# chao1224/GeoSSL

Hardware: AMD Instinct MI355X
Metric: molecules/s/GPU SchNet+DDM fwd+bwd (QM9-sized, bs=1024); % HBM roofline (higher is better)
Workload: dtype f32

## Files before the change

### geossl_amd/Geom3D/models/schnet.py

```python
import ctypes as C
import math
import os

import torch
from ...switches import env as _env
from torch.nn import Embedding, Linear, ModuleList, Sequential

from ... import _lib, ops
from ..._lib import call, ptr, stream
from ...layout import get_layout
from ._atomic_mass import atomic_masses

SUPPORTED_F = (32, 64, 128)


class _Ssp(torch.autograd.Function):
    @staticmethod
    def forward(ctx, x):
        x = x.contiguous()
        y = torch.empty_like(x)
        call("geossl_ssp_fwd", ptr(x), x.numel(), ptr(y), stream())
        ctx.save_for_backward(y)
        return y

    @staticmethod
    def backward(ctx, dy):
        (y,) = ctx.saved_tensors
        dx = torch.empty_like(y)
        call("geossl_ssp_bwd", ptr(y), ptr(dy.contiguous()), y.numel(), ptr(dx), stream())
        return dx


class ShiftedSoftplus(torch.nn.Module):

    def __init__(self):
        super().__init__()
        self.shift = torch.log(torch.tensor(2.0)).item()

    def forward(self, x):
        _lib.require_cuda(x)
        if x.dtype != torch.float32:
            raise TypeError("expected float32, got %s" % x.dtype)
        return _Ssp.apply(x)


class GaussianSmearing(torch.nn.Module):

    def __init__(self, start=0.0, stop=5.0, num_gaussians=50):
        super().__init__()
        offset = torch.linspace(start, stop, num_gaussians)
        self.coeff = -0.5 / (offset[1] - offset[0]).item() ** 2
        self.register_buffer("offset", offset)

    def forward(self, dist):
        return ops.gaussian_smearing(dist, self.offset, self.coeff)


class CFConv(torch.nn.Module):

    def __init__(self, in_channels, out_channels, num_filters, nn, cutoff):
        super().__init__()
        self.lin1 = Linear(in_channels, num_filters, bias=False)
        self.lin2 = Linear(num_filters, out_channels)
        self.nn = nn
        self.cutoff = cutoff
        self.reset_parameters()

    def reset_parameters(self):
        torch.nn.init.xavier_uniform_(self.lin1.weight)
        torch.nn.init.xavier_uniform_(self.lin2.weight)
        self.lin2.bias.data.fill_(0)


class InteractionBlock(torch.nn.Module):
    def __init__(self, hidden_channels, num_gaussians, num_filters, cutoff):
        super().__init__()
        self.mlp = Sequential(Linear(num_gaussians, num_filters), ShiftedSoftplus(), Linear(num_filters, num_filters))
        self.conv = CFConv(hidden_channels, hidden_channels, num_filters, self.mlp, cutoff)
        self.act = ShiftedSoftplus()
        self.lin = Linear(hidden_channels, hidden_channels)
        self.reset_parameters()

    def reset_parameters(self):
        torch.nn.init.xavier_uniform_(self.mlp[0].weight)
        self.mlp[0].bias.data.fill_(0)
        torch.nn.init.xavier_uniform_(self.mlp[2].weight)
        self.conv.reset_parameters()
        torch.nn.init.xavier_uniform_(self.lin.weight)
        self.lin.bias.data.fill_(0)


def _core_params(model):
    ps = [model.embedding.weight]
    for blk in model.interactions:
        ps += [blk.mlp[0].weight, blk.mlp[0].bias, blk.mlp[2].weight, blk.mlp[2].bias, blk.conv.lin1.weight,
               blk.conv.lin2.weight, blk.conv.lin2.bias, blk.lin.weight, blk.lin.bias]
    ps += [model.lin1.weight, model.lin1.bias, model.lin2.weight, model.lin2.bias]
    return ps


class _SchNetCore(torch.autograd.Function):

    @staticmethod
    def forward(ctx, z, pos, lay, cfg, *params):
        L, F, G = cfg["L"], cfg["F"], cfg["G"]
        dev = pos.device
        N = pos.size(0)
        want_params = any(ctx.needs_input_grad[4:])
        training = want_params or ctx.needs_input_grad[1]
        ps = [p.detach().contiguous() for p in params]
        emb_w, head = ps[0], ps[1 + 9 * L:]
        layers = [ps[1 + 9 * l: 1 + 9 * (l + 1)] for l in range(L)]
        st = stream()
        h = torch.empty(N, F, dtype=torch.float32, device=dev)
        status = cfg["status"]
        dyn = getattr(lay, "dyn", None)
        dN2, dP2 = (dyn.n_atoms2, dyn.n_pairs2) if dyn is not None else (None, None)
        if dyn is not None and (ctx.needs_input_grad[1] or F != 128 or not cfg["chain"]):
            raise _lib.GeosslHipError("a capacity-bucket layout serves the F = 128 chain path without position gradients")
        call("geossl_embedding_fwd_dyn", ptr(z), z.stride(0) if z.numel() else 1, ptr(emb_w), emb_w.size(0), N, F, ptr(h),
             ptr(status.word), dN2, st)
        if cfg["debug"]:
            status.check()
        sp = None
        if getattr(lay, "sparse", False):
            if dyn is not None:
                raise _lib.GeosslHipError("capacity buckets hold molecules of at most 255 atoms (bucket.MAX_N)")
            sp = ops.sparse_pair_geometry(pos, lay, cfg["cutoff"])
            pair_d, pair_c, pair_flag, dP2 = sp.pair_d, sp.pair_c, sp.pair_flag, sp.dyn_P
            aggregate = lambda x_, W_, out=None, swap=False, mols=None: ops.aggregate_sparse(x_, W_, sp, swap=swap, out=out)
        else:
            pair_d, pair_c, pair_flag = ops.pair_geometry(pos, lay, cfg["cutoff"])
            aggregate = lambda x_, W_, out=None, swap=False, mols=None: ops.aggregate(x_, W_, pair_flag, lay, swap=swap,
                                                                                      out=out, mols=mols)
        P = lay.P
        fw = _lib.FilterWeights()
        for l, lp in enumerate(layers):
            fw.w1[l], fw.b1[l], fw.w2[l], fw.b2[l] = ptr(lp[0]), ptr(lp[1]), ptr(lp[2]), ptr(lp[3])
        Wf = torch.empty(L, P, F, dtype=torch.float32, device=dev)
        keep_T = training and (ctx.needs_input_grad[1] or not _env("GEOSSL_FILTER_RECOMPUTE_T")
                               or bool(_env("GEOSSL_FILTER_BWD_BF16X3"))
                               or bool(_env("GEOSSL_ARITH_24BIT")))
        T = torch.empty(L, P, F, dtype=torch.float32, device=dev) if keep_T else None
        if P > 0:
            call("geossl_cfconv_filter_fwd_dyn", ptr(pair_d), ptr(pair_c), P, C.byref(fw), L, F, G, ptr(cfg["offset"]),
                 cfg["coeff"], ptr(T), ptr(Wf), dP2, st)
        hs, xs, aggs, ts = [], [], [], []
        heads = None
        if cfg["chain"]:
            chain_w = [lp[k] for lp in layers for k in (4, 5, 7)] + [head[0], head[2]]
            if want_params and 2 * len(chain_w) <= _lib.PREPARE_MAX:
                img, img_bwd = ops.prepare_chain(chain_w, both=True)
            else:
                img, img_bwd = ops.prepare_chain(chain_w, transB=True), None
            i_lin1, i_lin2, i_lin = img[0:3 * L:3], img[1:3 * L:3], img[2:3 * L:3]
            full = lambda: torch.empty(N, F, dtype=torch.float32, device=dev)
            hs, xs, aggs, ts = [h] + [full() for _ in range(L)], [full() for _ in range(L)], [full() for _ in range(L)], \
                [full() for _ in range(L)]
            u, hout = full(), full()

            def run_rows(a0, a1, mols, todo=None):
                rows = lambda t_: t_[a0:a1]

                def chain(x_, stages):
                    if todo is not None:
                        todo.append(("chain", x_, stages))
                    else:
                        ops.linear_chain(x_, stages, dyn_rows=dN2)

                chain(rows(hs[0]), [dict(image=i_lin1[0], out=rows(xs[0]))])
                for l, lp in enumerate(layers):
                    if todo is not None:
                        todo.append(("agg", xs[l], Wf[l], aggs[l], False))
                    else:
                        aggregate(xs[l], Wf[l], out=aggs[l], mols=mols)
                    stages = [dict(image=i_lin2[l], bias=lp[6], flags=_lib.EPI_SSP, out=rows(ts[l])),
                              dict(image=i_lin[l], bias=lp[8], res=rows(hs[l]), out=rows(hs[l + 1]))]
                    if l + 1 < L:
                        stages.append(dict(image=i_lin1[l + 1], out=rows(xs[l + 1])))
                    else:
                        stages.append(dict(image=img[3 * L], bias=head[1], flags=_lib.EPI_SSP, out=rows(u)))
                    chain(rows(aggs[l]), stages)
                chain(rows(u), [dict(image=img[3 * L + 1], bias=head[3], out=rows(hout))])

            todo = [] if (cfg["loop"] and P > 0 and sp is None and 2 * L + 2 <= _lib.LOOP_MAX_OPS) else None
            if todo is not None:
                run_rows(0, N, None, todo)
                if not ops.layer_loop(todo, lay, pair_flag, N, F, stagger=cfg["loop_stagger"]):
                    todo = None
            if todo is None:
                run_rows(0, N, None)
            h = hs[L]
            hs = hs[:L]
            if not training:
                hs, xs, aggs, ts = [], [], [], []
        else:
            pw = ops.prepare_linear([lp[k] for lp in layers for k in (4, 5, 7)], transB=True)
            if pw is not None:
                layers = [lp[:4] + [pw[3 * l], pw[3 * l + 1], lp[6], pw[3 * l + 2], lp[8]] for l, lp in enumerate(layers)]
            for l, lp in enumerate(layers):
                x = ops.linear(h, lp[4])
                agg = aggregate(x, Wf[l])
                t = ops.linear(agg, lp[5], bias=lp[6], flags=_lib.EPI_SSP)
                hn = ops.linear(t, lp[7], bias=lp[8], res=h)
                if training:
                    hs.append(h); xs.append(x); aggs.append(agg); ts.append(t)
                h = hn
            u = ops.linear(h, head[0], bias=head[1], flags=_lib.EPI_SSP)
            hout = ops.linear(u, head[2], bias=head[3])
        if training:
            ctx.lay, ctx.cfg = lay, cfg
            ctx.z = z
            ctx.pos = pos
            ctx.want_params = want_params
            ctx.ps = ps
            ctx.params = params
            ctx.saved = dict(pair_d=pair_d, pair_c=pair_c, pair_flag=pair_flag, Wf=Wf, T=T, hs=hs, xs=xs, aggs=aggs,
                             ts=ts, h_last=h, u=u, img_bwd=img_bwd if cfg["chain"] else None, sparse=sp)
        return hout

    @staticmethod
    def backward(ctx, dhout):
        want_pos, want_params = ctx.needs_input_grad[1], ctx.want_params
        if torch.is_grad_enabled():
            from ...higher_order import SchNetGradNode
            if ctx.saved.get("sparse") is not None:
                raise NotImplementedError("second-order gradients (create_graph=True, training on forces) are limited to "
                                          "dense layouts: structures of at most 255 atoms, GEOSSL_SPARSE_PAIRS unset")
            dpos, grads = SchNetGradNode.run(ctx, dhout, want_pos, want_params)
            return (None, dpos, None, None) + tuple(grads)
        dpos, grads = _SchNetCore.fused_backward(ctx, dhout, want_pos, want_params, allow_direct=True)
        return (None, dpos, None, None) + tuple(grads)

    @staticmethod
    def fused_backward(ctx, dhout, want_pos, want_params, allow_direct):
        cfg, lay, sv, ps = ctx.cfg, ctx.lay, ctx.saved, ctx.ps
        L, F, G = cfg["L"], cfg["F"], cfg["G"]
        dev = dhout.device
        N = dhout.size(0)
        st = stream()
        emb_w, head = ps[0], ps[1 + 9 * L:]
        layers = [ps[1 + 9 * l: 1 + 9 * (l + 1)] for l in range(L)]
        direct = want_params and allow_direct and _lib.direct_grads_enabled(ctx.params)
        grads = [p.grad for p in ctx.params] if direct else [torch.empty_like(p) if want_params else None for p in ps]
        accum = 1 if direct else 0
        g_emb, g_head = grads[0], grads[1 + 9 * L:]
        g_layers = [grads[1 + 9 * l: 1 + 9 * (l + 1)] for l in range(L)]
        dh_out = dhout.contiguous()
        dyn = getattr(lay, "dyn", None)
        dN2, dP2 = (dyn.n_atoms2, dyn.n_pairs2) if dyn is not None else (None, None)
        sp = sv.get("sparse")
        if sp is not None:
            dP2, pair_i, pair_j = sp.dyn_P, sp.pair_i, sp.pair_j
            aggregate = lambda x_, W_, out=None, mols=None: ops.aggregate_sparse(x_, W_, sp, swap=True, out=out)
        else:
            pair_i, pair_j = lay.pair_i, lay.pair_j
            aggregate = lambda x_, W_, out=None, mols=None: ops.aggregate(x_, W_, sv["pair_flag"], lay, swap=True,
                                                                          out=out, mols=mols)
        probs = []
        daggs = [None] * L
        if cfg["chain"]:
            img = sv.get("img_bwd")
            if img is None:
                img = ops.prepare_chain([lp[k] for lp in layers for k in (4, 5, 7)] + [head[0], head[2]], transB=False)
            i_lin1, i_lin2, i_lin = img[0:3 * L:3], img[1:3 * L:3], img[2:3 * L:3]
            full = lambda: torch.empty(N, F, dtype=torch.float32, device=dev)
            du = full()
            dhs = [full() for _ in range(L + 1)]
            dys, dxs = [full() for _ in range(L)], [full() for _ in range(L)]
            daggs = [full() for _ in range(L)]

            def run_rows(a0, a1, mols, todo=None):
                rows = lambda t_: t_[a0:a1]

                def chain(x_, stages):
                    if todo is not None:
                        todo.append(("chain", x_, stages))
                    else:
                        ops.linear_chain(x_, stages, dyn_rows=dN2)

                chain(rows(dh_out), [dict(image=img[3 * L + 1], tprev=rows(sv["u"]), out=rows(du)),
                                     dict(image=img[3 * L], out=rows(dhs[L]))])
                chain(rows(dhs[L]), [dict(image=i_lin[L - 1], tprev=rows(sv["ts"][L - 1]), out=rows(dys[L - 1])),
                                     dict(image=i_lin2[L - 1], out=rows(daggs[L - 1]))])
                for l in reversed(range(L)):
                    if todo is not None:
                        todo.append(("agg", daggs[l], sv["Wf"][l], dxs[l], True))
                    else:
                        aggregate(daggs[l], sv["Wf"][l], out=dxs[l], mols=mols)
                    stages = [dict(image=i_lin1[l], res=rows(dhs[l + 1]), out=rows(dhs[l]))]
                    if l > 0:
                        stages += [dict(image=i_lin[l - 1], tprev=rows(sv["ts"][l - 1]), out=rows(dys[l - 1])),
                                   dict(image=i_lin2[l - 1], out=rows(daggs[l - 1]))]
                    chain(rows(dxs[l]), stages)

            todo = [] if (cfg["loop"] and lay.P > 0 and sp is None and 2 * L + 2 <= _lib.LOOP_MAX_OPS) else None
            if todo is not None:
                run_rows(0, N, None, todo)
                if not ops.layer_loop(todo, lay, sv["pair_flag"], N, F, stagger=cfg["loop_stagger"]):
                    todo = None
            if todo is None:
                run_rows(0, N, None)
            probs.append((dh_out, sv["u"], g_head[2], g_head[3]))
            probs.append((du, sv["h_last"], g_head[0], g_head[1]))
            for l in reversed(range(L)):
                gl = g_layers[l]
                probs.append((dhs[l + 1], sv["ts"][l], gl[7], gl[8]))
                probs.append((dys[l], sv["aggs"][l], gl[5], gl[6]))
                probs.append((dxs[l], sv["hs"][l], gl[4], None))
            dh = dhs[0]
        else:
            du = ops.linear(dh_out, head[2], transB=False, tprev=sv["u"])
            dh = ops.linear(du, head[0], transB=False)
            probs.append((dh_out, sv["u"], g_head[2], g_head[3]))
            probs.append((du, sv["h_last"], g_head[0], g_head[1]))
            pw = ops.prepare_linear([lp[k] for lp in layers for k in (4, 5, 7)], transB=False)
            for l in reversed(range(L)):
                lp, gl = layers[l], g_layers[l]
                w_lin1, w_lin2, w_lin = (pw[3 * l], pw[3 * l + 1], pw[3 * l + 2]) if pw is not None else (lp[4], lp[5], lp[7])
                dy = ops.linear(dh, w_lin, transB=False, tprev=sv["ts"][l])
                dagg = ops.linear(dy, w_lin2, transB=False)
                dx = aggregate(dagg, sv["Wf"][l])
                dh_new = ops.linear(dx, w_lin1, transB=False, res=dh)
                probs.append((dh, sv["ts"][l], gl[7], gl[8]))
                probs.append((dy, sv["aggs"][l], gl[5], gl[6]))
                probs.append((dx, sv["hs"][l], gl[4], None))
                daggs[l] = dagg
                dh = dh_new
        P = lay.P
        fw = _lib.FilterWeights()
        gin = _lib.FilterGradIn()
        for l, lp in enumerate(layers):
            fw.w1[l], fw.b1[l], fw.w2[l], fw.b2[l] = ptr(lp[0]), ptr(lp[1]), ptr(lp[2]), ptr(lp[3])
            gin.x[l], gin.dagg[l] = ptr(sv["xs"][l]), ptr(daggs[l])
        if want_params:
            ops.linear_wgrad(probs, N, F, F, accumulate=bool(accum), dyn_rows=dN2)
            nfl = _lib.load().geossl_embedding_bwd_workspace_floats(emb_w.size(0), F)
            ws = torch.empty(nfl, dtype=torch.float32, device=dev)
            z = ctx.z
            call("geossl_embedding_bwd_dyn", ptr(z), z.stride(0) if z.numel() else 1, ptr(dh), emb_w.size(0), N, F,
                 ptr(g_emb), ptr(ws), accum, dN2, st)
            if P > 0:
                gout = _lib.FilterGradOut()
                for l, gl in enumerate(g_layers):
                    gout.dw1[l], gout.db1[l], gout.dw2[l], gout.db2[l] = ptr(gl[0]), ptr(gl[1]), ptr(gl[2]), ptr(gl[3])
                nfl = _lib.load().geossl_cfconv_filter_bwd_workspace_floats(P, L, F, G)
                ws2 = torch.empty(nfl, dtype=torch.float32, device=dev)
                call("geossl_cfconv_filter_bwd_dyn", ptr(sv["pair_d"]), ptr(sv["pair_c"]), ptr(sv["pair_flag"]),
                     ptr(pair_i), ptr(pair_j), P, N, C.byref(fw), C.byref(gin), L, F, G, ptr(cfg["offset"]),
                     cfg["coeff"], ptr(sv["T"]), C.byref(gout), ptr(ws2), accum, dP2, dN2, st)
            elif not direct:
                for gl in g_layers:
                    for k in range(4):
                        gl[k].zero_()
        dpos = None
        if want_pos:
            dpos = torch.zeros(N, 3, dtype=torch.float32, device=dev)
            if P > 0:
                dd = torch.empty(L, P, dtype=torch.float32, device=dev)
                call("geossl_cfconv_filter_dpos", ptr(sv["pair_d"]), ptr(sv["pair_c"]), ptr(sv["pair_flag"]),
                     ptr(pair_i), ptr(pair_j), P, C.byref(fw), C.byref(gin), L, F, G, ptr(cfg["offset"]),
                     cfg["coeff"], cfg["cutoff"], ptr(sv["T"]), ptr(sv["Wf"]), ptr(dd), st)
                if sp is not None:
                    ops.pair_position_grad_sparse(ctx.pos, sp, dd, out=dpos)
                else:
                    call("geossl_pair_position_grad", ptr(ctx.pos), ptr(sv["pair_d"]), ptr(dd), ptr(lay.mol_ptr),
                         ptr(lay.pair_ptr), lay.B, P, L, ptr(dpos), st)
        if direct:
            return dpos, [None] * len(grads)
        return dpos, list(grads)


class _SchNetTapeCore(torch.autograd.Function):

    @staticmethod
    def forward(ctx, z, pos, lay, cfg, *params):
        from ... import tape as tp
        with torch.no_grad():
            x = tp.leaf(pos, bool(ctx.needs_input_grad[1]))
            ps = [tp.leaf(p, bool(n)) for p, n in zip(params, ctx.needs_input_grad[4:])]
            h = tp.schnet_atom_features(z, x, lay, cfg, ps)
        ctx.tape = (h, x, ps)
        ctx.shapes = [tuple(p.shape) for p in params]
        return h.t

    @staticmethod
    def backward(ctx, dh):
        from ... import tape as tp
        if torch.is_grad_enabled():
            raise NotImplementedError("second-order gradients (training on forces) need the fused widths: "
                                      "hidden_channels == num_filters in %s" % (SUPPORTED_F,))
        h, x, ps = ctx.tape
        wrt = [v for v in [x] + ps if v.req]
        with torch.no_grad():
            got = iter(tp.grad([h], [tp.const(dh.contiguous())], wrt))
        vals = [next(got) if v.req else None for v in [x] + ps]
        dpos = None if vals[0] is None else vals[0].t
        grads = [None if g is None else g.t.reshape(shape) for g, shape in zip(vals[1:], ctx.shapes)]
        return (None, dpos, None, None) + tuple(grads)


class _SegmentReduce(torch.autograd.Function):

    @staticmethod
    def forward(ctx, h, lay, reduce):
        ctx.lay, ctx.reduce = lay, reduce
        return ops.segment_reduce(h.contiguous(), lay, reduce)

    @staticmethod
    def backward(ctx, dout):
        return _SegmentExpand.apply(dout, ctx.lay, ctx.reduce), None, None


class _SegmentExpand(torch.autograd.Function):

    @staticmethod
    def forward(ctx, dout, lay, reduce):
        ctx.lay, ctx.reduce = lay, reduce
        dh = torch.empty(lay.N, dout.size(1), dtype=torch.float32, device=dout.device)
        call("geossl_segment_reduce_bwd", ptr(dout.contiguous()), ptr(lay.mol_ptr), lay.B, dout.size(1),
             1 if reduce == "mean" else 0, ptr(dh), 0, stream())
        return dh

    @staticmethod
    def backward(ctx, g):
        return _SegmentReduce.apply(g, ctx.lay, ctx.reduce), None, None


class SchNet(torch.nn.Module):
    def __init__(self, hidden_channels=128, num_filters=128, num_interactions=6, num_gaussians=50, cutoff=10.0,
                 node_class=None, readout="mean", dipole=False, mean=None, std=None, atomref=None):
        super().__init__()
        assert readout in ["add", "sum", "mean"]
        self.hidden_channels = hidden_channels
        self.num_filters = num_filters
        self.num_interactions = num_interactions
        self.num_gaussians = num_gaussians
        self.cutoff = cutoff
        self.readout = readout
        self.dipole = dipole
        self.readout = "add" if self.dipole else self.readout
        self.mean = mean
        self.std = std
        self.scale = None

        self.register_buffer("atomic_mass", atomic_masses())
        self.embedding = Embedding(node_class, hidden_channels)
        self.distance_expansion = GaussianSmearing(0.0, cutoff, num_gaussians)
        self.interactions = ModuleList()
        for _ in range(num_interactions):
            self.interactions.append(InteractionBlock(hidden_channels, num_gaussians, num_filters, cutoff))
        self.lin1 = Linear(hidden_channels, hidden_channels)
        self.act = ShiftedSoftplus()
        self.lin2 = Linear(hidden_channels, hidden_channels)
        self.register_buffer("initial_atomref", atomref)
        self.atomref = None
        if atomref is not None:
            self.atomref = Embedding(100, 1)
            self.atomref.weight.data.copy_(atomref)
        self.reset_parameters()

    def reset_parameters(self):
        self.embedding.reset_parameters()
        for interaction in self.interactions:
            interaction.reset_parameters()
        torch.nn.init.xavier_uniform_(self.lin1.weight)
        self.lin1.bias.data.fill_(0)
        torch.nn.init.xavier_uniform_(self.lin2.weight)
        self.lin2.bias.data.fill_(0)
        if self.atomref is not None:
            self.atomref.weight.data.copy_(self.initial_atomref)

    def _status_word(self, device):
        return _lib.module_status(self, device, "atom type out of range for the embedding table (node_class=%d)"
                                  % self.embedding.num_embeddings)

    def check_status(self):
        st = self.__dict__.get("_geossl_status")
        if st is not None:
            st.check()

    def _check_supported(self):
        if self.dipole:
            raise NotImplementedError("dipole readout (schnet.py:103-107,117-118) is off the GeoSSL path")
        F = self.hidden_channels
        return (self.num_filters == F and F in SUPPORTED_F and self.num_interactions <= _lib.MAX_L
                and self.num_gaussians <= 64)

    def forward(self, z, pos, batch=None, return_latent=False, layout=None, latent_only=False):
        assert z.dim() == 1 and z.dtype == torch.long
        _lib.require_cuda(z, pos, batch)
        fused = self._check_supported()
        batch = torch.zeros_like(z) if batch is None else batch
        lay = layout if layout is not None else get_layout(batch)
        if lay.N != pos.size(0):
            raise ValueError("layout does not match the number of atoms")
        status = self._status_word(pos.device)
        status.poll()
        cfg = dict(L=self.num_interactions, F=self.hidden_channels, G=self.num_gaussians, cutoff=float(self.cutoff),
                   offset=self.distance_expansion.offset, coeff=float(self.distance_expansion.coeff),
                   debug=bool(_env("GEOSSL_DEBUG")), status=status,
                   chain=(self.num_interactions >= 1 and not _env("GEOSSL_NO_CHAIN")
                          and not _env("GEOSSL_ARITH_24BIT")),
                   loop=(_env("GEOSSL_LAYER_LOOP") == "1" or
                         (_env("GEOSSL_LAYER_LOOP") is None and not _env("GEOSSL_NO_LAYER_LOOP")
                          and torch.cuda.is_current_stream_capturing())),
                   loop_stagger=int(_env("GEOSSL_LAYER_LOOP_STAGGER") or 0))
        if pos.dtype != torch.float32:
            raise TypeError("positions must be float32")
        if fused:
            h = _SchNetCore.apply(z, pos.contiguous(), lay, cfg, *_core_params(self))
        else:
            if getattr(lay, "sparse", False):
                raise NotImplementedError("the general-width path (hidden_channels != num_filters, or widths outside %s) "
                                          "is limited to structures of at most 255 atoms; the fused widths take up to "
                                          "1024" % (SUPPORTED_F,))
            if z.numel() and (int(z.min()) < 0 or int(z.max()) >= self.embedding.num_embeddings):
                raise IndexError("atom type out of range for the embedding table (node_class=%d)"
                                 % self.embedding.num_embeddings)
            h = _SchNetTapeCore.apply(z, pos.contiguous(), lay, cfg, *_core_params(self))
        status.arm()
        if not self.dipole and self.mean is not None and self.std is not None:
            h = h * self.std + self.mean
        if not self.dipole and self.atomref is not None:
            h = h + self.atomref(z)
        if latent_only and return_latent:
            return None, h
        out = _SegmentReduce.apply(h, lay, self.readout)
        if self.scale is not None:
            out = self.scale * out
        if return_latent:
            return out, h
        return out

    def __repr__(self):
        return (f"{self.__class__.__name__}(hidden_channels={self.hidden_channels}, "
                f"num_filters={self.num_filters}, num_interactions={self.num_interactions}, "
                f"num_gaussians={self.num_gaussians}, cutoff={self.cutoff})")
```

### geossl_amd/_lib.py

```python
import ctypes as C
import os

import torch

HERE = os.path.dirname(os.path.abspath(__file__))
LIB_PATH = os.path.join(HERE, "lib", "libgeossl_hip.so")

MAX_L = 12
TN_MAX = 32
EPI_BIAS, EPI_SSP, EPI_RESIDUAL, EPI_MUL_DSSP, CHAIN_SAME_INPUT, CHAIN_NEW_INPUT, CHAIN_ADD_PREV = 1, 2, 4, 8, 16, 32, 64
EPI_SILU, EPI_MUL_DSILU = 128, 256

vp = C.c_void_p
i64 = C.c_int64
i32 = C.c_int
f32 = C.c_float
f64 = C.c_double
u64 = C.c_uint64


class FilterWeights(C.Structure):
    _fields_ = [("w1", vp * MAX_L), ("b1", vp * MAX_L), ("w2", vp * MAX_L), ("b2", vp * MAX_L)]


PREPARE_MAX = 64


class PrepareBatch(C.Structure):
    _fields_ = [("W", vp * PREPARE_MAX), ("image", vp * PREPARE_MAX), ("ldw", i32 * PREPARE_MAX), ("tb", i32 * PREPARE_MAX)]


CHAIN_MAX = 5


class ChainStage(C.Structure):
    _fields_ = [("image", vp), ("bias", vp), ("res", vp), ("tprev", vp), ("out", vp), ("ld", i32), ("flags", i32),
                ("xin", vp), ("ldxin", i32), ("pad_", i32), ("out_act", vp)]


class Chain(C.Structure):
    _fields_ = [("nstage", i32), ("st", ChainStage * CHAIN_MAX)]


LOOP_MAX_OPS = 14


class LoopOp(C.Structure):
    _fields_ = [("kind", i32), ("swap", i32), ("X", vp), ("Wf", vp), ("out", vp), ("chain", Chain)]


class FilterGradIn(C.Structure):
    _fields_ = [("x", vp * MAX_L), ("dagg", vp * MAX_L)]


class FilterGradOut(C.Structure):
    _fields_ = [("dw1", vp * MAX_L), ("db1", vp * MAX_L), ("dw2", vp * MAX_L), ("db2", vp * MAX_L)]


class TnBatch(C.Structure):
    _fields_ = [("A", vp * TN_MAX), ("B", vp * TN_MAX), ("dW", vp * TN_MAX), ("db", vp * TN_MAX)]


class NcsnWeights(C.Structure):
    _fields_ = [(k, vp) for k in ("in_w1", "in_b1", "in_w2", "in_b2", "o1_w", "o1_b", "o2_w", "o2_b", "o3_w", "o3_b",
                                  "sigmas")]


class NcsnGrads(C.Structure):
    _fields_ = [(k, vp) for k in ("in_w1", "in_b1", "in_w2", "in_b2", "o1_w", "o1_b", "o2_w", "o2_b", "o3_w", "o3_b")]


class NcsnSaved(C.Structure):
    _fields_ = [(k, vp) for k in ("a1", "a2", "pd", "emb", "gscale")]


class NcsnHeadFwd(C.Structure):
    _fields_ = [("h", vp), ("distance", vp), ("noise_level", vp), ("distance_noise", vp), ("w", NcsnWeights),
                ("saved", NcsnSaved), ("anneal_power", f32), ("pad_", f32), ("loss_e", vp), ("workspace", vp)]


class NcsnHeadBwd(C.Structure):
    _fields_ = [("h", vp), ("w", NcsnWeights), ("saved", NcsnSaved), ("out_scale", f32), ("pad_", f32), ("dfeat", vp),
                ("demb", vp), ("grow", vp), ("grads", NcsnGrads), ("workspace", vp), ("dh", vp)]


COPY_MAX = 8


class CopyBatch(C.Structure):
    _fields_ = [("dst", vp * COPY_MAX), ("src", vp * COPY_MAX), ("bytes", i64 * COPY_MAX)]


class Gather(C.Structure):
    _fields_ = [(k, vp) for k in ("x_src", "pos_src", "src_off", "mol_ptr", "x_dst", "pos_dst", "batch_dst", "se_ptr", "sei0",
                                  "sei1", "pair_ptr2", "pair_i", "pair_j", "inc_ptr", "inc_idx", "e0_src", "e1_src",
                                  "e_src_off", "e_ptr", "e0_dst", "e1_dst", "zero")] + \
               [("zero_count", i64), ("x_cols", i32), ("option", i32)]


class Mask(C.Structure):
    _fields_ = [(k, vp) for k in ("bond_ptr", "bond_dst", "src_n", "mol_id", "keep_in", "keep_out", "e_src_cnt",
                                  "e_count")] + [("seed", u64), ("max_n", i32), ("pad_", i32)]


P = C.POINTER
PROTOTYPES = {
    "geossl_abi_version": (i32, []),
    "geossl_layout_build": (i32, [vp, i64, i64, vp, vp, vp, vp]),
    "geossl_pair_index_fill": (i32, [vp, vp, i64, vp, vp, vp]),
    "geossl_radius_graph_count": (i32, [vp, vp, i64, i32, f32, i32, vp, vp]),
    "geossl_radius_graph_fill": (i32, [vp, vp, i64, i32, f32, i32, vp, vp, vp, vp, vp]),
    "geossl_pair_geometry": (i32, [vp, vp, vp, i64, i32, f32, i32, f32, vp, vp, vp, vp]),
    "geossl_rbf_fwd": (i32, [vp, i64, vp, i32, f32, vp, vp]),
    "geossl_ssp_fwd": (i32, [vp, i64, vp, vp]),
    "geossl_ssp_bwd": (i32, [vp, vp, i64, vp, vp]),
    "geossl_cfconv_filter_fwd": (i32, [vp, vp, i64, P(FilterWeights), i32, i32, i32, vp, f32, vp, vp, vp]),
    "geossl_cfconv_filter_bwd_workspace_floats": (i64, [i64, i32, i32, i32]),
    "geossl_cfconv_filter_bwd": (i32, [vp, vp, vp, vp, vp, i64, i64, P(FilterWeights), P(FilterGradIn), i32, i32, i32, vp,
                                       f32, vp, P(FilterGradOut), vp, i32, vp]),
    "geossl_cfconv_filter_dpos": (i32, [vp, vp, vp, vp, vp, i64, P(FilterWeights), P(FilterGradIn), i32, i32, i32, vp, f32,
                                        f32, vp, vp, vp, vp]),
    "geossl_pair_position_grad": (i32, [vp, vp, vp, vp, vp, i64, i64, i32, vp, vp]),
    "geossl_cfconv_aggregate": (i32, [vp, vp, vp, vp, vp, vp, i64, i32, i32, i32, vp, vp]),
    "geossl_aggregate_parts": (i32, [i32]),
    "geossl_cfconv_aggregate_work": (i32, [vp, vp, vp, vp, vp, vp, i64, i32, i32, i32, vp, vp]),
    "geossl_pair_product": (i32, [vp, vp, vp, vp, vp, i64, i32, i32, vp, vp]),
    "geossl_linear": (i32, [vp, i32, vp, vp, vp, vp, vp, i32, i64, i32, i32, i32, i32, vp]),
    "geossl_tn_plan": (None, [i64, i32, P(i32), P(i32)]),
    "geossl_tn_workspace_floats": (i64, [i64, i32, i32, i32]),
    "geossl_row_normalize_fwd": (i32, [vp, i64, i32, f32, vp, vp, vp]),
    "geossl_row_normalize_bwd": (i32, [vp, vp, vp, i64, i32, f32, vp, vp]),
    "geossl_atom_tuples": (i32, [vp, vp, i64, i32, vp, vp, vp]),
    "geossl_linear_image_words": (i64, [i32, i32]),
    "geossl_linear_prepare": (i32, [P(PrepareBatch), i32, i32, i32, i32, vp]),
    "geossl_linear_prepared": (i32, [vp, i32, vp, vp, vp, vp, vp, i32, i64, i32, i32, i32, vp]),
    "geossl_chain_image_words": (i64, [i32]),
    "geossl_chain_prepare": (i32, [P(PrepareBatch), i32, i32, i32, vp]),
    "geossl_linear_chain": (i32, [vp, i32, P(Chain), i64, i32, vp]),
    "geossl_linear_wgrad": (i32, [P(TnBatch), i32, i64, i32, i32, i32, i32, i32, vp, i32, vp]),
    "geossl_embedding_fwd": (i32, [vp, i64, vp, i32, i64, i32, vp, vp, vp]),
    "geossl_embedding_bwd_workspace_floats": (i64, [i32, i32]),
    "geossl_embedding_bwd": (i32, [vp, i64, vp, i32, i64, i32, vp, vp, i32, vp]),
    "geossl_segment_reduce_fwd": (i32, [vp, vp, i64, i32, i32, vp, vp]),
    "geossl_segment_reduce_bwd": (i32, [vp, vp, i64, i32, i32, vp, i32, vp]),
    "geossl_axpy": (i32, [vp, vp, f32, i64, vp, vp]),
    "geossl_pair_distance": (i32, [vp, vp, vp, i64, vp, vp]),
    "geossl_super_edge_ptr": (i32, [vp, vp, vp, i64, i64, vp, vp, vp]),
    "geossl_incidence_count": (i32, [vp, vp, vp, vp, i64, i32, vp, vp]),
    "geossl_incidence_fill": (i32, [vp, vp, vp, vp, i64, i32, vp, vp, vp]),
    "geossl_ddm_loss_fwd_workspace_floats": (i64, [i32]),
    "geossl_ddm_loss_fwd": (i32, [vp, vp, vp, vp, i64, vp, vp, vp, P(NcsnWeights), i32, f32, vp, P(NcsnSaved), vp, vp]),
    "geossl_schnet_layer_loop": (i32, [vp, i32, vp, i32, vp, vp, vp, i32, i32, i64, i32, i32, vp]),
    "geossl_schnet_layer_loop_ragged": (i32, [vp, i32, vp, vp, vp, i64, i32, i64, i32, vp]),
    "geossl_copy2": (i32, [vp, vp, i64, vp, vp, i64, vp]),
    "geossl_ddm_noise": (i32, [vp, f32, f32, i64, i64, i64, i32, i32, vp, vp, vp, vp, vp, vp]),
    "geossl_ddm_noise_seeded": (i32, [u64, f32, f32, i64, i64, i64, i32, i32, vp, vp, vp, vp, vp, vp]),
    "geossl_ddm_views": (i32, [vp, vp, vp, vp, i64, i64, vp, vp, vp, vp, i64, vp, vp]),
    "geossl_loss_reduce_partials": (i32, [vp, vp, f32, vp, i32, vp]),
    "geossl_ddm_loss_fwd2": (i32, [vp, vp, vp, vp, i64, i32, vp]),
    "geossl_loss_reduce_partials2": (i32, [vp, vp, vp, f32, f32, vp, vp]),
    "geossl_ddm_loss_bwd_fused2": (i32, [vp, vp, vp, i64, i64, i32, vp, vp, vp, vp, i32, vp]),
    "geossl_loss_reduce_workspace_floats": (i64, [i64]),
    "geossl_loss_reduce": (i32, [vp, i64, vp, f32, vp, vp, i32, vp]),
    "geossl_ddm_loss_bwd_rows": (i32, [P(NcsnWeights), P(NcsnSaved), i64, i32, vp, f32, vp, vp, vp, vp, vp, vp]),
    "geossl_ddm_loss_bwd_workspace_floats": (i64, [i64, i32]),
    "geossl_ddm_loss_bwd_weights": (i32, [vp, vp, vp, i64, i32, P(NcsnWeights), P(NcsnSaved), vp, vp, vp, P(NcsnGrads),
                                          vp, i32, vp]),
    "geossl_ddm_loss_bwd_fused_workspace_floats": (i64, [i64, i32]),
    "geossl_ddm_loss_bwd_fused": (i32, [vp, vp, vp, i64, i64, i32, P(NcsnWeights), P(NcsnSaved), vp, f32, vp, vp, vp, vp,
                                        P(NcsnGrads), vp, i32, vp]),
    "geossl_incidence_gather": (i32, [vp, vp, vp, i64, i32, vp, i32, vp]),
    "geossl_painn_edge_geom": (i32, [vp, vp, vp, i64, f32, vp, vp, i32, vp, vp, vp, vp]),
    "geossl_silu_fwd": (i32, [vp, i64, vp, vp]),
    "geossl_silu_bwd": (i32, [vp, vp, i64, vp, vp]),
    "geossl_painn_interaction_fwd": (i32, [vp, vp, vp, vp, vp, vp, vp, vp, vp, vp, vp, i64, i32, i32, vp, vp, vp]),
    "geossl_painn_interaction_bwd_workspace_floats": (i64, [i64, i32, i32]),
    "geossl_painn_interaction_fwd_mol": (i32, [vp, vp, vp, vp, vp, vp, vp, vp, vp, vp, vp, vp, i64, i32, i64, i32, i32, vp,
                                               vp, vp]),
    "geossl_painn_interaction_fwd_mma": (i32, [vp, vp, vp, vp, vp, vp, vp, vp, vp, vp, vp, vp, vp, i64, i32, i64, i32, i32,
                                               vp, vp, vp]),
    "geossl_painn_interaction_bwd_mol_workspace_floats": (i64, [i64, i64, i32, i32]),
    "geossl_painn_interaction_bwd_mol": (i32, [vp, vp, vp, vp, vp, vp, vp, vp, vp, vp, vp, vp, vp, i64, i32, i64, i32, i32,
                                               vp, vp, vp, vp, vp, i32, vp]),
    "geossl_painn_interaction_bwd": (i32, [vp, vp, vp, vp, vp, vp, vp, vp, vp, vp, vp, vp, i64, i32, i32, vp, vp, vp, vp,
                                           vp, i32, vp]),
    "geossl_painn_mix_pre_fwd": (i32, [vp, vp, i64, i32, f32, vp, vp, vp]),
    "geossl_painn_mix_post_fwd": (i32, [vp, vp, vp, vp, vp, i64, i32, vp, vp, vp]),
    "geossl_painn_mix_post_bwd": (i32, [vp, vp, vp, vp, vp, i64, i32, vp, vp, vp]),
    "geossl_painn_mix_pre_bwd": (i32, [vp, vp, vp, vp, i64, i32, vp, vp, vp]),
    "geossl_add": (i32, [vp, vp, i64, vp, vp]),
    "geossl_painn_edge_grads": (i32, [vp] * 11 + [i64, i32, i32, vp, vp, vp, i32, vp]),
    "geossl_painn_edge_geom_bwd": (i32, [vp, vp, vp, i64, f32, vp, vp, i32, vp, vp, vp, vp, vp]),
    "geossl_painn_position_grad": (i32, [vp, vp, vp, vp, vp, i64, vp, vp]),
    "geossl_adam_step": (i32, [vp, vp, vp, vp, i64, f64, f64, f64, f64, f64, i64, f32, vp]),
    "geossl_copy_n": (i32, [P(CopyBatch), i32, vp]),
    "geossl_ddm_views_dyn": (i32, [vp, vp, vp, vp, i64, i64, vp, vp, vp, vp, i64, vp, vp, vp, vp]),
    "geossl_embedding_fwd_dyn": (i32, [vp, i64, vp, i32, i64, i32, vp, vp, vp, vp]),
    "geossl_embedding_bwd_dyn": (i32, [vp, i64, vp, i32, i64, i32, vp, vp, i32, vp, vp]),
    "geossl_cfconv_filter_fwd_dyn": (i32, [vp, vp, i64, P(FilterWeights), i32, i32, i32, vp, f32, vp, vp, vp, vp]),
    "geossl_cfconv_filter_bwd_dyn": (i32, [vp, vp, vp, vp, vp, i64, i64, P(FilterWeights), P(FilterGradIn), i32, i32, i32,
                                           vp, f32, vp, P(FilterGradOut), vp, i32, vp, vp, vp]),
    "geossl_cfconv_aggregate_work_dyn": (i32, [vp, vp, vp, vp, vp, vp, i64, i32, i32, i32, vp, vp, vp]),
    "geossl_cfconv_aggregate_targets_dyn": (i32, [vp, vp, vp, vp, vp, vp, i64, i32, i32, i32, vp, vp, vp]),
    "geossl_linear_chain_dyn": (i32, [vp, i32, P(Chain), i64, i32, vp, vp]),
    "geossl_linear_wgrad_dyn": (i32, [P(TnBatch), i32, i64, i32, i32, i32, i32, i32, vp, i32, vp, vp]),
    "geossl_ddm_loss_fwd2_dyn": (i32, [vp, vp, vp, vp, i64, i32, vp, vp, vp]),
    "geossl_ddm_loss_bwd_fused2_dyn": (i32, [vp, vp, vp, i64, i64, i32, vp, vp, vp, vp, i32, vp, vp, vp]),
    "geossl_painn_group_capacity": (i64, [i64, i64]),
    "geossl_painn_edge_layout": (i32, [vp, vp, i64, vp, i64, i64, i64] + [vp] * 12),
    "geossl_painn_edge_geom_dyn": (i32, [vp, vp, vp, i64, f32, vp, vp, i32, vp, vp, vp, vp, vp]),
    "geossl_painn_interaction_fwd_mma_dyn": (i32, [vp, vp, vp, vp, vp, vp, vp, vp, vp, vp, vp, vp, vp, i64, i32, i64, i32,
                                                   i32, vp, vp, vp, vp]),
    "geossl_tape_unary": (i32, [i32, vp, i64, f32, f32, vp, vp]),
    "geossl_tape_binary": (i32, [i32, vp, i32, vp, i32, i64, i32, f32, vp, vp]),
    "geossl_tape_colsum_workspace_floats": (i64, [i64, i32]),
    "geossl_tape_reduce": (i32, [i32, vp, i64, i32, vp, vp, vp]),
    "geossl_tape_gather_rows": (i32, [vp, vp, i32, i64, i32, vp, vp]),
    "geossl_tape_scatter_rows": (i32, [vp, vp, i32, vp, i64, i32, vp, vp]),
    "geossl_tape_copy2d": (i32, [vp, i64, vp, i64, i64, i32, vp]),
    "geossl_tape_fill": (i32, [vp, i64, f32, vp]),
    "geossl_painn_stage_cap": (i32, [i32, i32, i32]),
    "geossl_painn_interaction_fwd_atoms": (i32, [vp] * 12 + [i64, vp, i32, i32, vp, vp, vp]),
    "geossl_painn_interaction_bwd_atoms": (i32, [vp] * 13 + [i64, vp, i32, i32, vp, vp, vp, vp, vp, i32, vp]),
    "geossl_painn_interaction_bwd_mol_skip": (i32, [vp, vp, vp, vp, vp, vp, vp, vp, vp, vp, vp, vp, vp, i64, i32, i64, i32,
                                                    i32, vp, vp, vp, vp, vp, i32, vp]),
    "geossl_painn_mix_pre_fwd_dyn": (i32, [vp, vp, i64, i32, f32, vp, vp, vp, vp]),
    "geossl_painn_mix_post_fwd_dyn": (i32, [vp, vp, vp, vp, vp, i64, i32, vp, vp, vp, vp]),
    "geossl_painn_mix_post_bwd_dyn": (i32, [vp, vp, vp, vp, vp, i64, i32, vp, vp, vp, vp]),
    "geossl_painn_mix_pre_bwd_dyn": (i32, [vp, vp, vp, vp, i64, i32, vp, vp, vp, vp]),
    "geossl_gather_molecules": (i32, [P(Gather), i64, vp]),
    "geossl_gather_masked_molecules": (i32, [P(Gather), P(Mask), i64, vp]),
    "geossl_infonce_fwd": (i32, [vp, vp, i64, i32, f32, vp, vp, vp, vp, vp]),
    "geossl_infonce_bwd": (i32, [vp, vp, vp, vp, i64, i32, f32, vp, vp, vp, vp]),
    "geossl_ebm_nce_fwd": (i32, [vp, vp, i64, i32, i32, vp, vp, vp, vp, vp, vp]),
    "geossl_ebm_nce_bwd": (i32, [vp, vp, vp, i64, i32, i32, vp, vp, vp, vp]),
    "geossl_distance_head_width_ok": (i32, [i32]),
    "geossl_distance_head_fwd_workspace_floats": (i64, [i64]),
    "geossl_distance_head_bwd_workspace_floats": (i64, [i64, i32]),
    "geossl_distance_head_fwd": (i32, [vp, i64, i32, vp, vp, vp, vp, vp, i64, vp, vp, vp, vp, vp, vp]),
    "geossl_distance_head_fwd_dyn": (i32, [vp, i64, i32, vp, vp, vp, vp, vp, i64, vp, vp, vp, vp, vp, vp, vp, vp]),
    "geossl_distance_head_bwd": (i32, [vp, i64, i32, vp, vp, i64, vp, vp, vp, vp, vp, vp, vp, vp, i32, vp]),
    "geossl_distance_head_bwd_dyn": (i32, [vp, i64, i32, vp, vp, i64, vp, vp, vp, vp, vp, vp, vp, vp, i32, vp, vp, vp]),
    "geossl_charge_mask_count": (i64, [i64, f64]),
    "geossl_charge_mask": (i32, [vp, i32, i64, f64, i32, vp, vp, vp, vp, vp, vp]),
    "geossl_charge_mask_dyn": (i32, [vp, i32, i64, f64, i32, vp, vp, vp, vp, vp, vp, vp]),
    "geossl_charge_head_width_ok": (i32, [i32, i32]),
    "geossl_charge_head_fwd_workspace_floats": (i64, [i64]),
    "geossl_charge_head_bwd_workspace_floats": (i64, [i64, i32, i32]),
    "geossl_charge_head_fwd": (i32, [vp, i64, i32, vp, vp, i32, vp, vp, i64, vp, vp, vp, vp, vp, vp]),
    "geossl_charge_head_fwd_dyn": (i32, [vp, i64, i32, vp, vp, i32, vp, vp, i64, vp, vp, vp, vp, vp, vp, vp]),
    "geossl_charge_head_bwd": (i32, [vp, i64, i32, vp, i32, vp, vp, i64, vp, vp, vp, vp, vp, vp, vp, i32, vp]),
    "geossl_charge_head_bwd_dyn": (i32, [vp, i64, i32, vp, i32, vp, vp, i64, vp, vp, vp, vp, vp, vp, vp, i32, vp, vp]),
    "geossl_infograph_width_ok": (i32, [i32]),
    "geossl_infograph_fwd_workspace_floats": (i64, [i64]),
    "geossl_infograph_fwd": (i32, [vp, i64, i32, vp, vp, i64, i32, vp, vp, vp, vp, vp, vp, vp, vp]),
    "geossl_infograph_fwd_dyn": (i32, [vp, i64, i32, vp, vp, i64, i32, vp, vp, vp, vp, vp, vp, vp, vp, vp]),
    "geossl_infograph_bwd": (i32, [vp, i64, i32, vp, vp, i64, i32, vp, vp, vp, vp, vp, vp, vp, vp]),
    "geossl_infograph_bwd_dyn": (i32, [vp, i64, i32, vp, vp, i64, i32, vp, vp, vp, vp, vp, vp, vp, vp, vp]),
    "geossl_property_width_ok": (i32, [i32]),
    "geossl_property_workspace_floats": (i64, [i64]),
    "geossl_property_fwd": (i32, [vp, i64, i32, vp, i64, i32, i32, vp, vp, vp, vp, vp, i64, vp, i32, vp, vp, vp, vp, vp,
                                  vp]),
    "geossl_property_fwd_dyn": (i32, [vp, i64, i32, vp, i64, i32, i32, vp, vp, vp, vp, vp, i64, vp, i32, vp, vp, vp, vp,
                                      vp, vp, vp]),
    "geossl_property_predict": (i32, [vp, i64, i32, vp, i64, i32, i32, vp, vp, vp, vp, vp, vp, vp]),
    "geossl_property_predict_dyn": (i32, [vp, i64, i32, vp, i64, i32, i32, vp, vp, vp, vp, vp, vp, vp, vp]),
    "geossl_property_bwd": (i32, [i64, i32, vp, i64, i32, i32, vp, vp, vp, vp, vp, vp, i64, vp, i32, vp, vp, vp, vp, vp,
                                  vp, i32, vp]),
    "geossl_property_bwd_dyn": (i32, [i64, i32, vp, i64, i32, i32, vp, vp, vp, vp, vp, vp, i64, vp, i32, vp, vp, vp, vp,
                                      vp, vp, i32, vp, vp]),
    "geossl_property_targets": (i32, [vp, i64, i32, i32, vp, vp, i64, vp, vp]),
    "geossl_torsion_head_width_ok": (i32, [i32]),
    "geossl_torsion_head_fwd_workspace_floats": (i64, [i64]),
    "geossl_torsion_head_bwd_workspace_floats": (i64, [i64, i32]),
    "geossl_torsion_head_fwd": (i32, [vp, i64, i32, vp, vp, vp, vp, vp, vp, i64, vp, vp, vp, vp, vp, vp]),
    "geossl_torsion_head_fwd_dyn": (i32, [vp, i64, i32, vp, vp, vp, vp, vp, vp, i64, vp, vp, vp, vp, vp, vp, vp, vp]),
    "geossl_torsion_head_bwd": (i32, [vp, i64, i32, vp, vp, vp, vp, i64, vp, vp, i64, vp, vp, vp, vp, vp, i32, vp]),
    "geossl_torsion_head_bwd_dyn": (i32, [vp, i64, i32, vp, vp, vp, vp, i64, vp, vp, i64, vp, vp, vp, vp, vp, i32, vp, vp,
                                          vp]),
    "geossl_triple_angles": (i32, [vp, i64, vp, vp, vp, i64, vp, vp]),
    "geossl_gather_triples": (i32, [vp, i64, vp, vp, vp, vp, i64, vp, vp, vp, vp, vp]),
    "geossl_sparse_pairs_build": (i32, [vp, vp, i64, i64, i32, f32, i32, f32, i64] + [vp] * 13),
    "geossl_cfconv_aggregate_sparse": (i32, [vp, vp, vp, vp, vp, i64, i32, i32, vp, vp]),
    "geossl_pair_position_grad_sparse": (i32, [vp, vp, vp, vp, vp, vp, i64, i64, i32, vp, vp]),
}

_lib = None


class GeosslHipError(RuntimeError):
    pass


def load():
    global _lib
    if _lib is not None:
        return _lib
    path = os.environ.get("GEOSSL_HIP_LIB", LIB_PATH)
    if not os.path.exists(path):
        raise GeosslHipError(
            "libgeossl_hip.so is not built (%s). Run `python -m geossl_amd.build` (needs hipcc); "
            "there is no CPU fallback." % path)
    lib = C.CDLL(path)
    for name, (res, args) in PROTOTYPES.items():
        fn = getattr(lib, name)
        fn.restype = res
        fn.argtypes = args
    if lib.geossl_abi_version() != 1:
        raise GeosslHipError("ABI version mismatch")
    _lib = lib
    return lib


def check(rc, what):
    if rc != 0:
        raise GeosslHipError("%s failed with hipError %d" % (what, rc))


def ptr(t):
    if t is None:
        return None
    return t.data_ptr()


def stream():
    return torch._C._cuda_getCurrentRawStream(torch._C._cuda_getDevice())


def require_cuda(*tensors):
    for t in tensors:
        if t is not None and not t.is_cuda:
            raise GeosslHipError(
                "geossl_amd runs on MI355X only: got a %s tensor. The HIP path has no CPU fallback." % t.device.type)



_DIRECT = {"depth": 0}


class direct_grads:
    def __enter__(self):
        _DIRECT["depth"] += 1
        return self

    def __exit__(self, *exc):
        _DIRECT["depth"] -= 1
        return False


def direct_grads_enabled(params):
    return _DIRECT["depth"] > 0 and all(
        p.grad is not None and p.grad.is_contiguous() and p.grad.dtype == torch.float32 and p.grad.is_cuda
        for p in params)


class StatusWord:

    def __init__(self, device, message):
        self.word = torch.zeros(1, dtype=torch.int32, device=device)
        self.host = torch.zeros(1, dtype=torch.int32).pin_memory()
        self.event = None
        self.message = message

    def __deepcopy__(self, memo):
        return None

    def __reduce__(self):
        return (type(None), ())

    def poll(self):
        if self.event is None or torch.cuda.is_current_stream_capturing():
            return
        if self.event.query():
            self.event = None
            if int(self.host[0]):
                raise IndexError(self.message)

    def arm(self, every=1):
        self.calls = getattr(self, "calls", 0) + 1
        if every > 1 and self.calls % every != 1:
            return
        if self.event is None and not torch.cuda.is_current_stream_capturing():
            self.host.copy_(self.word, non_blocking=True)
            self.event = torch.cuda.Event()
            self.event.record()

    def check(self):
        if int(self.word.item()):
            raise IndexError(self.message)


def module_status(module, device, message):
    st = module.__dict__.get("_geossl_status")
    if st is None or st.word.device != device:
        st = StatusWord(device, message)
        module.__dict__["_geossl_status"] = st
    return st


TIMERS = None
CALLS = None


def call(name, *args):
    global CALLS
    lib = load()
    if CALLS is not None:
        CALLS += 1
    timers = TIMERS
    key = name[:-4] if name.endswith("_dyn") else name
    if timers is not None and key in timers:
        e0, e1 = torch.cuda.Event(enable_timing=True), torch.cuda.Event(enable_timing=True)
        e0.record()
        rc = getattr(lib, name)(*args)
        e1.record()
        timers[key].append((e0, e1))
    else:
        rc = getattr(lib, name)(*args)
    check(rc, name)


def fill_ptrs(arr, tensors):
    for i, t in enumerate(tensors):
        arr[i] = ptr(t)
```

### geossl_amd/csrc/filter_fwd.hip

```cpp
#include "common.h"
#include "geossl_hip.h"
#include "split.h"

using namespace geossl;

namespace {

#ifdef FF_TIMING
__device__ long long ff_dbg[2 * 64 * 8 + 2 * 64];
#define FF_MARK(slot)                                                                                     \
  do {                                                                                                    \
    __builtin_amdgcn_sched_barrier(0);                                                                    \
    if (blockIdx.x == 3 && blockIdx.y == 0 && lane == 0 && (wave == 0 || wave == 4) && ff_t < 64)        \
      ff_dbg[((wave == 0 ? 0 : 1) * 64 + ff_t) * 8 + (slot)] = clock64();                                 \
    __builtin_amdgcn_sched_barrier(0);                                                                    \
  } while (0)
#else
#define FF_MARK(slot) do {} while (0)
#endif

template <int NMB, int K1S>
__global__ __launch_bounds__(512) void k_filter_fwd(const float* __restrict__ pair_d,
                                                    const float* __restrict__ pair_c, int P,
                                                    GeosslFilterWeights w, int G,
                                                    const float* __restrict__ offset, float coeff,
                                                    float* __restrict__ Tout, float* __restrict__ Wf,
                                                    const int32_t* __restrict__ dyn_P) {
  constexpr int F = 32 * NMB, K2S = F / 16;
  extern __shared__ __attribute__((aligned(16))) uint8_t smem_raw[];
  u32x4* W2f = reinterpret_cast<u32x4*>(smem_raw);
  u32x4* W1f = W2f + NMB * K2S * 3 * 64;
  float* b1s = reinterpret_cast<float*>(W1f + NMB * K1S * 3 * 64);
  float* b2s = b1s + F;
  float* offs = b2s + F;
  const int tid = threadIdx.x, lane = tid & 63, wave = tid >> 6, j = lane & 31, kh = lane >> 5;
  const int l = blockIdx.y;
  {
    const float* __restrict__ w2 = w.w2[l];
    for (int i = tid; i < NMB * K2S * 64; i += 512) {
      const int ln = i & 63, ks = (i >> 6) % K2S, mb = i / (64 * K2S);
      const float* row = w2 + (size_t)(32 * mb + (ln & 31)) * F + 16 * ks + 4 * (ln >> 5);
      const float4 lo = *reinterpret_cast<const float4*>(row), hi = *reinterpret_cast<const float4*>(row + 8);
      const float v[8] = {lo.x, lo.y, lo.z, lo.w, hi.x, hi.y, hi.z, hi.w};
      const Frag3 f = split8(v);
      u32x4* dst = W2f + ((size_t)(mb * K2S + ks) * 3) * 64 + ln;
      dst[0] = f.h;
      dst[64] = f.m;
      dst[128] = f.l;
    }
    const float* __restrict__ w1 = w.w1[l];
    for (int i = tid; i < NMB * K1S * 64; i += 512) {
      const int ln = i & 63, ks = (i >> 6) % K1S, mb = i / (64 * K1S);
      const float* row = w1 + (size_t)(32 * mb + (ln & 31)) * G;
      float v[8];
#pragma unroll
      for (int e = 0; e < 8; ++e) {
        const int g = 16 * ks + 8 * (ln >> 5) + e;
        v[e] = g < G ? row[g] : 0.0f;
      }
      const Frag3 f = split8(v);
      u32x4* dst = W1f + ((size_t)(mb * K1S + ks) * 3) * 64 + ln;
      dst[0] = f.h;
      dst[64] = f.m;
      dst[128] = f.l;
    }
    for (int i = tid; i < F; i += 512) {
      b1s[i] = w.b1[l][i];
      b2s[i] = w.b2[l][i];
    }
    for (int i = tid; i < 16 * K1S; i += 512) offs[i] = i < G ? offset[i] : 0.0f;
  }
  __syncthreads();
  const size_t lbase = (size_t)l * P;
  P = dyn_count(P, dyn_P);
  if (P <= 0) return;
  const int nrb = (P + 31) / 32;
#ifdef FF_TIMING
  int ff_t = -1;
#endif
  for (int rb = blockIdx.x + gridDim.x * wave; rb < nrb; rb += gridDim.x * 8) {
#ifdef FF_TIMING
    ++ff_t;
#endif
    FF_MARK(0);
#ifdef FF_TIMING
    if (blockIdx.x == 3 && blockIdx.y == 0 && lane == 0 && (wave == 0 || wave == 4) && ff_t < 64)
      ff_dbg[2 * 64 * 8 + (wave == 0 ? 0 : 64) + ff_t] = wall_clock64();
#endif
    const int row = 32 * rb + j;
    const bool live = row < P;
    const float d = live ? pair_d[row] : 0.0f;
    const float cw = live ? pair_c[row] : 0.0f;
    f32x16 acc1[NMB];
#pragma unroll
    for (int mb = 0; mb < NMB; ++mb)
#pragma unroll
      for (int q = 0; q < 4; ++q) {
        const float4 b = *reinterpret_cast<const float4*>(b1s + 32 * mb + 8 * q + 4 * kh);
        acc1[mb][4 * q] = b.x;
        acc1[mb][4 * q + 1] = b.y;
        acc1[mb][4 * q + 2] = b.z;
        acc1[mb][4 * q + 3] = b.w;
      }
    Frag3 bfr[K1S];
#pragma unroll
    for (int ks = 0; ks < K1S; ++ks) {
      float v[8];
      const float4 o0 = *reinterpret_cast<const float4*>(offs + 16 * ks + 8 * kh);
      const float4 o1 = *reinterpret_cast<const float4*>(offs + 16 * ks + 8 * kh + 4);
      const float o[8] = {o0.x, o0.y, o0.z, o0.w, o1.x, o1.y, o1.z, o1.w};
#pragma unroll
      for (int e = 0; e < 8; ++e) {
        const float diff = d - o[e];
        v[e] = exp_neg(coeff * (diff * diff));
      }
      bfr[ks] = split8(v);
    }
    FF_MARK(1);
    Frag3 tb[K2S];
    float* trow = Tout != nullptr ? Tout + (lbase + row) * F + 4 * kh : nullptr;
    auto finish_block = [&](int mb) {
#pragma unroll
      for (int half = 0; half < 2; ++half) {
        float v[8];
#pragma unroll
        for (int e = 0; e < 8; ++e) v[e] = ssp(acc1[mb][8 * half + e]);
        if (trow != nullptr && live) {
          *reinterpret_cast<float4*>(trow + 32 * mb + 16 * half) = make_float4(v[0], v[1], v[2], v[3]);
          *reinterpret_cast<float4*>(trow + 32 * mb + 16 * half + 8) = make_float4(v[4], v[5], v[6], v[7]);
        }
        tb[2 * mb + half] = split8(v);
      }
    };
#pragma unroll
    for (int mb = 0; mb < NMB; ++mb) {
#pragma unroll
      for (int ks = 0; ks < K1S; ++ks) {
        Frag3 af;
        const u32x4* src = W1f + ((size_t)(mb * K1S + ks) * 3) * 64 + lane;
        af.h = src[0];
        af.m = src[64];
        af.l = src[128];
        mma6(acc1[mb], af, bfr[ks]);
      }
      if (mb > 0) {
        finish_block(mb - 1);
#pragma unroll
        for (int i = 0; i < 6 * K1S; ++i) {
          __builtin_amdgcn_sched_group_barrier(0x008, 1, 0);
          __builtin_amdgcn_sched_group_barrier(0x002, 16, 0);
        }
      }
      __builtin_amdgcn_sched_barrier(0);
    }
    FF_MARK(2);
    finish_block(NMB - 1);
    __builtin_amdgcn_sched_barrier(0);
    FF_MARK(3);
    constexpr int MP = NMB >= 2 ? 2 : 1;
    float* orow = Wf + (lbase + row) * F + 4 * kh;
#pragma unroll
    for (int mb0 = 0; mb0 < NMB; mb0 += MP) {
      f32x16 acc2[MP];
#pragma unroll
      for (int u = 0; u < MP; ++u)
#pragma unroll
        for (int q = 0; q < 4; ++q) {
          const float4 b = *reinterpret_cast<const float4*>(b2s + 32 * (mb0 + u) + 8 * q + 4 * kh);
          acc2[u][4 * q] = b.x;
          acc2[u][4 * q + 1] = b.y;
          acc2[u][4 * q + 2] = b.z;
          acc2[u][4 * q + 3] = b.w;
        }
      Frag3 af[MP], an[MP];
#pragma unroll
      for (int u = 0; u < MP; ++u) {
        const u32x4* src = W2f + ((size_t)((mb0 + u) * K2S) * 3) * 64 + lane;
        af[u].h = src[0];
        af[u].m = src[64];
        af[u].l = src[128];
      }
#pragma unroll
      for (int ks = 0; ks < K2S; ++ks) {
        if (ks + 1 < K2S) {
#pragma unroll
          for (int u = 0; u < MP; ++u) {
            const u32x4* src = W2f + ((size_t)((mb0 + u) * K2S + ks + 1) * 3) * 64 + lane;
            an[u].h = src[0];
            an[u].m = src[64];
            an[u].l = src[128];
          }
        }
        __builtin_amdgcn_sched_barrier(0);
#pragma unroll
        for (int u = 0; u < MP; ++u) acc2[u] = mfma_bf16(af[u].l, tb[ks].h, acc2[u]);
#pragma unroll
        for (int u = 0; u < MP; ++u) acc2[u] = mfma_bf16(af[u].h, tb[ks].l, acc2[u]);
#pragma unroll
        for (int u = 0; u < MP; ++u) acc2[u] = mfma_bf16(af[u].m, tb[ks].m, acc2[u]);
#pragma unroll
        for (int u = 0; u < MP; ++u) acc2[u] = mfma_bf16(af[u].m, tb[ks].h, acc2[u]);
#pragma unroll
        for (int u = 0; u < MP; ++u) acc2[u] = mfma_bf16(af[u].h, tb[ks].m, acc2[u]);
#pragma unroll
        for (int u = 0; u < MP; ++u) acc2[u] = mfma_bf16(af[u].h, tb[ks].h, acc2[u]);
        __builtin_amdgcn_sched_barrier(0);
        if (ks + 1 < K2S) {
#pragma unroll
          for (int u = 0; u < MP; ++u) af[u] = an[u];
        }
      }
      if (mb0 == 0) FF_MARK(4);
      else FF_MARK(6);
      if (live) {
#pragma unroll
        for (int u = 0; u < MP; ++u)
#pragma unroll
          for (int q = 0; q < 4; ++q)
            *reinterpret_cast<float4*>(orow + 32 * (mb0 + u) + 8 * q) =
                make_float4(acc2[u][4 * q] * cw, acc2[u][4 * q + 1] * cw, acc2[u][4 * q + 2] * cw,
                            acc2[u][4 * q + 3] * cw);
      }
      if (mb0 == 0) FF_MARK(5);
      else FF_MARK(7);
    }
  }
}



#ifndef FFH_THREADS
#define FFH_THREADS 512
#endif
template <int NMB, int K1S>
__global__ __launch_bounds__(FFH_THREADS) void k_filter_fwd_h(const float* __restrict__ pair_d,
                                                      const float* __restrict__ pair_c, int P,
                                                      GeosslFilterWeights w, int G,
                                                      const float* __restrict__ offset, float coeff,
                                                      float* __restrict__ Tout, float* __restrict__ Wf,
                                                    const int32_t* __restrict__ dyn_P) {
  constexpr int F = 32 * NMB, K2S = F / 16;
  extern __shared__ __attribute__((aligned(16))) uint8_t smem_raw[];
  u32x4* W2f = reinterpret_cast<u32x4*>(smem_raw);
  u32x4* W1f = W2f + NMB * K2S * 2 * 64;
  float* b1s = reinterpret_cast<float*>(W1f + NMB * K1S * 2 * 64);
  float* b2s = b1s + F;
  float* offs = b2s + F;
  float* red = offs + 16 * K1S;
  const int tid = threadIdx.x, lane = tid & 63, wave = tid >> 6, j = lane & 31, kh = lane >> 5;
  const int l = blockIdx.y;
  float s1, s2;
  {
    const float* __restrict__ w2 = w.w2[l];
    const float* __restrict__ w1 = w.w1[l];
    float m1 = 0.0f, m2 = 0.0f;
    for (int i = tid; i < F * G; i += FFH_THREADS) m1 = fmaxf(m1, fabsf(w1[i]));
    for (int i = tid; i < F * F; i += FFH_THREADS) m2 = fmaxf(m2, fabsf(w2[i]));
#pragma unroll
    for (int o = 32; o >= 1; o >>= 1) {
      m1 = fmaxf(m1, __shfl_xor(m1, o));
      m2 = fmaxf(m2, __shfl_xor(m2, o));
    }
    if (lane == 0) {
      red[wave] = m1;
      red[16 + wave] = m2;
    }
    __syncthreads();
#pragma unroll
    for (int i = 0; i < FFH_THREADS / 64; ++i) {
      m1 = fmaxf(m1, red[i]);
      m2 = fmaxf(m2, red[16 + i]);
    }
    int e1, e2;
    s1 = pow2_scale_to_2p14(m1, e1);
    s2 = pow2_scale_to_2p14(m2, e2);
    for (int i = tid; i < NMB * K2S * 64; i += FFH_THREADS) {
      const int ln = i & 63, ks = (i >> 6) % K2S, mb = i / (64 * K2S);
      const float* row = w2 + (size_t)(32 * mb + (ln & 31)) * F + 16 * ks + 4 * (ln >> 5);
      const float4 lo = *reinterpret_cast<const float4*>(row), hi = *reinterpret_cast<const float4*>(row + 8);
      const float v[8] = {lo.x * s2, lo.y * s2, lo.z * s2, lo.w * s2, hi.x * s2, hi.y * s2, hi.z * s2, hi.w * s2};
      const Frag2 f = split8h(v);
      u32x4* dst = W2f + ((size_t)(mb * K2S + ks) * 2) * 64 + ln;
      dst[0] = f.h;
      dst[64] = f.l;
    }
    for (int i = tid; i < NMB * K1S * 64; i += FFH_THREADS) {
      const int ln = i & 63, ks = (i >> 6) % K1S, mb = i / (64 * K1S);
      const float* row = w1 + (size_t)(32 * mb + (ln & 31)) * G;
      float v[8];
#pragma unroll
      for (int e = 0; e < 8; ++e) {
        const int g = 16 * ks + 8 * (ln >> 5) + e;
        v[e] = g < G ? row[g] * s1 : 0.0f;
      }
      const Frag2 f = split8h(v);
      u32x4* dst = W1f + ((size_t)(mb * K1S + ks) * 2) * 64 + ln;
      dst[0] = f.h;
      dst[64] = f.l;
    }
    for (int i = tid; i < F; i += FFH_THREADS) {
      b1s[i] = w.b1[l][i];
      b2s[i] = w.b2[l][i];
    }
    for (int i = tid; i < 16 * K1S; i += FFH_THREADS) offs[i] = i < G ? offset[i] : 0.0f;
  }
  int* next_rb = reinterpret_cast<int*>(red + 32);
  if (tid == 0) *next_rb = 0;
  __syncthreads();
  const float inv1 = 1.0f / (s1 * 16384.0f), inv2 = 1.0f / s2;
  const size_t lbase = (size_t)l * P;
  P = dyn_count(P, dyn_P);
  if (P <= 0) return;
  const int nrb = (P + 31) / 32;
  auto take = [&]() {
    int t = 0;
    if (lane == 0) t = atomicAdd(next_rb, 1);
    return (int)blockIdx.x + (int)gridDim.x * __builtin_amdgcn_readfirstlane(t);
  };
  int rb = take();
  float d_n = pair_d[min(32 * rb + j, P - 1)], cw_n = pair_c[min(32 * rb + j, P - 1)];
  while (rb < nrb) {
    const int row = 32 * rb + j;
    const bool live = row < P;
    const float d = d_n;
    const float cw = live ? cw_n : 0.0f;
    const int rb_next = take();
    d_n = pair_d[min(32 * rb_next + j, P - 1)];
    cw_n = pair_c[min(32 * rb_next + j, P - 1)];
    int z = 0;
    asm volatile("" : "+v"(z));
    const int lz = lane + z, khz = 4 * kh + z;
    Frag2 bfr[K1S];
#pragma unroll
    for (int ks = 0; ks < K1S; ++ks) {
      float v[8];
      const float4 o0 = *reinterpret_cast<const float4*>(offs + 16 * ks + 2 * khz);
      const float4 o1 = *reinterpret_cast<const float4*>(offs + 16 * ks + 2 * khz + 4);
      const float o[8] = {o0.x, o0.y, o0.z, o0.w, o1.x, o1.y, o1.z, o1.w};
#pragma unroll
      for (int e = 0; e < 8; ++e) {
        const float diff = d - o[e];
        v[e] = exp_neg(coeff * (diff * diff));
      }
      bfr[ks] = split8h_scaled(v, 16384.0f);
    }
    f32x16 acc1[NMB];
#pragma unroll
    for (int mb = 0; mb < NMB; ++mb) {
#pragma unroll
      for (int e = 0; e < 16; ++e) acc1[mb][e] = 0.0f;
#pragma unroll
      for (int ks = 0; ks < K1S; ++ks) {
        const u32x4* src = W1f + ((size_t)(mb * K1S + ks) * 2) * 64 + lz;
        const u32x4 ah = src[0], al = src[64];
        acc1[mb] = mfma_f16(al, bfr[ks].h, acc1[mb]);
        acc1[mb] = mfma_f16(ah, bfr[ks].l, acc1[mb]);
        acc1[mb] = mfma_f16(ah, bfr[ks].h, acc1[mb]);
      }
    }
    float* trow = Tout != nullptr ? Tout + (lbase + row) * F + 4 * kh : nullptr;
    float tmax = 0.0f;
#pragma unroll
    for (int mb = 0; mb < NMB; ++mb)
#pragma unroll
      for (int q = 0; q < 4; ++q) {
        const float4 b = *reinterpret_cast<const float4*>(b1s + 32 * mb + 8 * q + khz);
        const float bb[4] = {b.x, b.y, b.z, b.w};
#pragma unroll
        for (int e = 0; e < 4; ++e) {
          const float t = ssp(fmaf(acc1[mb][4 * q + e], inv1, bb[e]));
          acc1[mb][4 * q + e] = t;
          tmax = fmaxf(tmax, fabsf(t));
        }
        if (trow != nullptr && live)
          *reinterpret_cast<float4*>(trow + 32 * mb + 8 * q) =
              make_float4(acc1[mb][4 * q], acc1[mb][4 * q + 1], acc1[mb][4 * q + 2], acc1[mb][4 * q + 3]);
      }
    tmax = fmaxf(tmax, __shfl_xor(tmax, 32));
    int et;
    const float st = pow2_scale_to_2p14(tmax, et);
    const float k2 = inv2 * __builtin_amdgcn_ldexpf(1.0f, et - 14);
    Frag2 tb[K2S];
#pragma unroll
    for (int ks = 0; ks < K2S; ++ks) {
      float v[8];
#pragma unroll
      for (int e = 0; e < 8; ++e) v[e] = acc1[ks >> 1][8 * (ks & 1) + e];
      tb[ks] = split8h_scaled(v, st);
    }
    constexpr int MP = NMB >= 2 ? 2 : 1;
    float* orow = Wf + (lbase + row) * F + 4 * kh;
#pragma unroll
    for (int mb0 = 0; mb0 < NMB; mb0 += MP) {
      f32x16 acc2[MP];
#pragma unroll
      for (int u = 0; u < MP; ++u)
#pragma unroll
        for (int e = 0; e < 16; ++e) acc2[u][e] = 0.0f;
#pragma unroll
      for (int ks = 0; ks < K2S; ++ks) {
        u32x4 ah[MP], al[MP];
#pragma unroll
        for (int u = 0; u < MP; ++u) {
          const u32x4* src = W2f + ((size_t)((mb0 + u) * K2S + ks) * 2) * 64 + lz;
          ah[u] = src[0];
          al[u] = src[64];
        }
#pragma unroll
        for (int u = 0; u < MP; ++u) acc2[u] = mfma_f16(al[u], tb[ks].h, acc2[u]);
#pragma unroll
        for (int u = 0; u < MP; ++u) acc2[u] = mfma_f16(ah[u], tb[ks].l, acc2[u]);
#pragma unroll
        for (int u = 0; u < MP; ++u) acc2[u] = mfma_f16(ah[u], tb[ks].h, acc2[u]);
      }
#pragma unroll
      for (int u = 0; u < MP; ++u)
#pragma unroll
        for (int q = 0; q < 4; ++q) {
          const float4 b = *reinterpret_cast<const float4*>(b2s + 32 * (mb0 + u) + 8 * q + khz);
          const float4 o = make_float4(fmaf(acc2[u][4 * q], k2, b.x) * cw, fmaf(acc2[u][4 * q + 1], k2, b.y) * cw,
                                       fmaf(acc2[u][4 * q + 2], k2, b.z) * cw, fmaf(acc2[u][4 * q + 3], k2, b.w) * cw);
          if (live) *reinterpret_cast<float4*>(orow + 32 * (mb0 + u) + 8 * q) = o;
        }
    }
    rb = rb_next;
  }
}

#ifdef FF_TIMING
}
extern "C" int geossl_filter_fwd_debug_read(long long* host) {
  return (int)hipMemcpyFromSymbol(host, HIP_SYMBOL(ff_dbg), sizeof(long long) * (2 * 64 * 8 + 2 * 64));
}
namespace {
#endif

}

extern "C" int geossl_cfconv_filter_fwd(const float* pair_d, const float* pair_c, int64_t P,
                                        const GeosslFilterWeights* w, int L, int F, int G, const float* offset,
                                        float coeff, float* T, float* Wf, hipStream_t stream) {
  return geossl_cfconv_filter_fwd_dyn(pair_d, pair_c, P, w, L, F, G, offset, coeff, T, Wf, nullptr, stream);
}

extern "C" int geossl_cfconv_filter_fwd_dyn(const float* pair_d, const float* pair_c, int64_t P,
                                            const GeosslFilterWeights* w, int L, int F, int G, const float* offset,
                                            float coeff, float* T, float* Wf, const int32_t* dyn_P,
                                            hipStream_t stream) {
  if (P <= 0 || L <= 0) return 0;
  if (L > GEOSSL_MAX_L || (F != 32 && F != 64 && F != 128) || G > 64 || G < 1) return (int)hipErrorInvalidValue;
  const int nrb = (int)((P + 31) / 32);
  int per_layer = 256 / L;
  if (per_layer < 1) per_layer = 1;
  if (per_layer > (nrb + 7) / 8) per_layer = (nrb + 7) / 8;
  dim3 grid(per_layer, L);
#define LAUNCH(NMB, K1S)                                                                                        \
  do {                                                                                                          \
    const size_t lds = (size_t)(NMB * (2 * NMB) + NMB * K1S) * 3 * 1024 + (2 * 32 * NMB + 16 * K1S) * 4;        \
    allow_big_lds(&k_filter_fwd<NMB, K1S>);                                                                     \
    hipLaunchKernelGGL((k_filter_fwd<NMB, K1S>), grid, dim3(512), lds, stream, pair_d, pair_c, (int)P, *w, G,   \
                       offset, coeff, T, Wf, dyn_P);                                                            \
  } while (0)
#define LAUNCH_F(NMB)                   \
  do {                                  \
    if (G <= 16) LAUNCH(NMB, 1);        \
    else if (G <= 32) LAUNCH(NMB, 2);   \
    else if (G <= 48) LAUNCH(NMB, 3);   \
    else LAUNCH(NMB, 4);                \
  } while (0)
  const bool bf16x3 = getenv("GEOSSL_FILTER_FWD_BF16X3") != nullptr || getenv("GEOSSL_ARITH_24BIT") != nullptr;
#define LAUNCH_H(NMB, K1S)                                                                                      \
  do {                                                                                                          \
    const size_t lds = (size_t)(NMB * (2 * NMB) + NMB * K1S) * 2 * 1024 + (2 * 32 * NMB + 16 * K1S + 36) * 4;   \
    allow_big_lds(&k_filter_fwd_h<NMB, K1S>);                                                                   \
    hipLaunchKernelGGL((k_filter_fwd_h<NMB, K1S>), grid, dim3(FFH_THREADS), lds, stream, pair_d, pair_c, (int)P, *w, G, \
                       offset, coeff, T, Wf, dyn_P);                                                            \
  } while (0)
#define LAUNCH_HF(NMB)                    \
  do {                                    \
    if (G <= 16) LAUNCH_H(NMB, 1);        \
    else if (G <= 32) LAUNCH_H(NMB, 2);   \
    else if (G <= 48) LAUNCH_H(NMB, 3);   \
    else LAUNCH_H(NMB, 4);                \
  } while (0)
  if (!bf16x3) {
    if (F == 128) LAUNCH_HF(4); else if (F == 64) LAUNCH_HF(2); else LAUNCH_HF(1);
  } else {
    if (F == 128) LAUNCH_F(4); else if (F == 64) LAUNCH_F(2); else LAUNCH_F(1);
  }
#undef LAUNCH_HF
#undef LAUNCH_H
#undef LAUNCH_F
#undef LAUNCH
  GEOSSL_CHECK_LAUNCH();
  return 0;
}
```

### geossl_amd/csrc/graph.hip

```cpp
#include "common.h"
#include "radius_adj.h"
#include "geossl_hip.h"

using namespace geossl;

namespace {

__global__ __launch_bounds__(1024) void k_layout_build(const int64_t* __restrict__ batch, int N, int B,
                                                       int32_t* __restrict__ mol_ptr, int32_t* __restrict__ pair_ptr,
                                                       int64_t* __restrict__ stats) {
  __shared__ int s_scan[1024];
  __shared__ int s_carry, s_bad, s_maxn;
  const int tid = threadIdx.x;
  if (tid == 0) {
    s_carry = 0;
    s_bad = 0;
    s_maxn = 0;
  }
  __syncthreads();
  int bad = 0;
  for (int a = tid; a < N; a += 1024) {
    const int64_t g = batch[a];
    if (g < 0 || g >= B || (a > 0 && batch[a - 1] > g)) bad = 1;
  }
  if (bad) atomicOr(&s_bad, 1);
  for (int g = tid; g <= B; g += 1024) {
    int lo = 0, hi = N;
    while (lo < hi) {
      const int mid = (lo + hi) >> 1;
      if (batch[mid] < g) lo = mid + 1; else hi = mid;
    }
    mol_ptr[g] = lo;
  }
  __syncthreads();
  __threadfence_block();
  int maxn = 0;
  for (int base = 0; base < B; base += 1024) {
    const int g = base + tid;
    int n = 0;
    if (g < B) n = mol_ptr[g + 1] - mol_ptr[g];
    maxn = max(maxn, n);
    const int v = n * (n - 1) / 2;
    s_scan[tid] = v;
    __syncthreads();
    for (int o = 1; o < 1024; o <<= 1) {
      const int add = tid >= o ? s_scan[tid - o] : 0;
      __syncthreads();
      s_scan[tid] += add;
      __syncthreads();
    }
    const int carry = s_carry;
    if (g < B) pair_ptr[g] = carry + s_scan[tid] - v;
    __syncthreads();
    if (tid == 1023) s_carry = carry + s_scan[1023];
    __syncthreads();
  }
  atomicMax(&s_maxn, maxn);
  __syncthreads();
  if (tid == 0) {
    pair_ptr[B] = s_carry;
    stats[0] = s_maxn;
    stats[1] = s_carry;
    stats[2] = s_bad;
    stats[3] = 0;
  }
}

__global__ void k_pair_index_fill(const int32_t* __restrict__ mol_ptr, const int32_t* __restrict__ pair_ptr, int B,
                                  int32_t* __restrict__ pair_i, int32_t* __restrict__ pair_j) {
  const int m = blockIdx.x;
  if (m >= B) return;
  const int a0 = mol_ptr[m], n = mol_ptr[m + 1] - a0, base = pair_ptr[m];
  for (int a = 0; a + 1 < n; ++a) {
    const int row = base + a * n - a * (a + 1) / 2 - a - 1;
    for (int b = a + 1 + threadIdx.x; b < n; b += blockDim.x) {
      pair_i[row + b] = a0 + a;
      pair_j[row + b] = a0 + b;
    }
  }
}

__global__ void k_atom_tuples(const int32_t* __restrict__ mol_ptr, const int64_t* __restrict__ tuple_ptr, int B,
                              int option, int64_t* __restrict__ out0, int64_t* __restrict__ out1) {
  const int m = blockIdx.x;
  if (m >= B) return;
  const int a0 = mol_ptr[m], n = mol_ptr[m + 1] - a0;
  const int64_t base = tuple_ptr[m];
  if (option == 0) {
    for (int a = 0; a + 1 < n; ++a) {
      const int64_t row = base + a * n - a * (a + 1) / 2 - a - 1;
      for (int b = a + 1 + threadIdx.x; b < n; b += blockDim.x) {
        out0[row + b] = a0 + a;
        out1[row + b] = a0 + b;
      }
    }
  } else {
    for (int a = 0; a < n; ++a) {
      const int64_t row = base + (int64_t)a * (n - 1);
      for (int b = threadIdx.x; b < n; b += blockDim.x) {
        if (b == a) continue;
        const int64_t c = row + (b < a ? b : b - 1);
        out0[c] = a0 + a;
        out1[c] = a0 + b;
      }
    }
  }
}

template <int MODE>
__global__ __launch_bounds__(64) void k_radius(const float* __restrict__ pos, const int32_t* __restrict__ mol_ptr,
                                               const int32_t* __restrict__ pair_ptr, int B, int max_n, float r2, int cap,
                                               int32_t* __restrict__ deg, const int64_t* __restrict__ edge_ptr,
                                               int64_t* __restrict__ edge_src, int64_t* __restrict__ edge_dst,
                                               float* __restrict__ edge_weight, float* __restrict__ pair_d,
                                               uint8_t* __restrict__ pair_flag, float cutoff,
                                               float* __restrict__ pair_c) {
  extern __shared__ __attribute__((aligned(16))) unsigned char smem_raw[];
  const int m = blockIdx.x;
  if (m >= B) return;
  const int lane = threadIdx.x;
  const int a0 = mol_ptr[m], n = mol_ptr[m + 1] - a0;
  const int words = (max_n + 63) / 64;
  unsigned long long* adj = reinterpret_cast<unsigned long long*>(smem_raw);
  float* sp = reinterpret_cast<float*>(adj + (size_t)max_n * words);
  for (int i = lane; i < 3 * n; i += 64) sp[i] = pos[(size_t)a0 * 3 + i];
  __syncthreads();
  const unsigned long long lt = (lane == 0) ? 0ull : (~0ull >> (64 - lane));
  for (int i = 0; i < n; ++i) {
    int64_t ebase = 0;
    if (MODE == 1) ebase = edge_ptr[a0 + i];
    const int d_all = radius_scan_target(sp, n, i, lane, r2, cap,
                                         [&](int c, int jn, float d2, bool keep, unsigned long long kept, int d_in) {
      if (MODE == 2 && lane == 0) adj[(size_t)i * words + c] = kept;
      if (MODE == 1 && keep) {
        const int64_t e = ebase + d_in + __popcll(kept & lt);
        edge_src[e] = a0 + jn;
        edge_dst[e] = a0 + i;
        edge_weight[e] = sqrtf(d2);
      }
    });
    if (MODE == 0 && lane == 0) deg[a0 + i] = d_all;
  }
  if (MODE == 2) {
    __syncthreads();
    const int base = pair_ptr[m];
    for (int a = 0; a + 1 < n; ++a) {
      const int row = base + a * n - a * (a + 1) / 2 - a - 1;
      for (int b = a + 1 + lane; b < n; b += 64) {
        const float d2 = dist2_nofma(sp + 3 * a, sp + 3 * b);
        const unsigned f0 = (adj[(size_t)a * words + (b >> 6)] >> (b & 63)) & 1ull;
        const unsigned f1 = (adj[(size_t)b * words + (a >> 6)] >> (a & 63)) & 1ull;
        const float d = sqrtf(d2);
        pair_d[row + b] = d;
        pair_c[row + b] = pair_envelope(d, cutoff);
        pair_flag[row + b] = (uint8_t)(f0 | (f1 << 1));
      }
    }
  }
}

__global__ __launch_bounds__(64) void k_pair_geometry_flat(const float* __restrict__ pos, const int32_t* __restrict__ mol_ptr,
                                                           const int32_t* __restrict__ pair_ptr, int B, float r2,
                                                           float cutoff, float* __restrict__ pair_d,
                                                           float* __restrict__ pair_c, uint8_t* __restrict__ pair_flag) {
  __shared__ float sp[3 * 64];
  const int m = blockIdx.x, lane = threadIdx.x;
  if (m >= B) return;
  const int a0 = mol_ptr[m], n = mol_ptr[m + 1] - a0;
  const int base = pair_ptr[m], np = n * (n - 1) / 2;
  for (int i = lane; i < 3 * n; i += 64) sp[i] = pos[(size_t)a0 * 3 + i];
  __syncthreads();
  const float tn = (float)(2 * n - 1);
  for (int q = lane; q < np; q += 64) {
    int a = (int)((tn - sqrtf(fmaxf(tn * tn - 8.0f * (float)q, 0.0f))) * 0.5f);
    a = min(max(a, 0), n - 2);
    if (a * n - a * (a + 1) / 2 > q) --a;
    else if ((a + 1) * n - (a + 1) * (a + 2) / 2 <= q) ++a;
    const int b = q - (a * n - a * (a + 1) / 2) + a + 1;
    const float d2 = dist2_nofma(sp + 3 * a, sp + 3 * b);
    const float d = sqrtf(d2);
    pair_d[base + q] = d;
    pair_c[base + q] = pair_envelope(d, cutoff);
    pair_flag[base + q] = d2 < r2 ? (uint8_t)3 : (uint8_t)0;
  }
}

__global__ void k_super_edge_ptr(const int64_t* __restrict__ batch, const int64_t* __restrict__ sei0,
                                 const int64_t* __restrict__ sei1, int S, int B, int32_t* __restrict__ se_ptr,
                                 int64_t* __restrict__ stats) {
  const int tid = blockIdx.x * blockDim.x + threadIdx.x, nth = gridDim.x * blockDim.x;
  if (tid == 0) stats[0] = S > 0 ? batch[sei0[S - 1]] + 1 : 0;
  for (int s = tid; s < S; s += nth) {
    const int64_t g = batch[sei0[s]];
    if (batch[sei1[s]] != g || (s > 0 && batch[sei0[s - 1]] > g)) stats[1] = 1;
  }
  for (int g = tid; g <= B; g += nth) {
    int lo = 0, hi = S;
    while (lo < hi) {
      const int mid = (lo + hi) >> 1;
      if (batch[sei0[mid]] < g) lo = mid + 1; else hi = mid;
    }
    se_ptr[g] = lo;
  }
}

template <int FILL>
__global__ __launch_bounds__(256) void k_incidence(const int64_t* __restrict__ batch, const int64_t* __restrict__ sei0,
                                                   const int64_t* __restrict__ sei1, const int32_t* __restrict__ se_ptr,
                                                   int N, int sides, int32_t* __restrict__ inc_cnt,
                                                   const int64_t* __restrict__ inc_ptr, int32_t* __restrict__ inc_idx) {
  const int a = blockIdx.x * 4 + (threadIdx.x >> 6), lane = threadIdx.x & 63;
  if (a >= N) return;
  const int g = (int)batch[a];
  const int s0 = se_ptr[g], s1 = se_ptr[g + 1];
  const unsigned long long lt = (lane == 0) ? 0ull : (~0ull >> (64 - lane));
  int count = 0;
  const int64_t base = FILL ? inc_ptr[a] : 0;
  for (int s = s0 + lane; s - lane < s1; s += 64) {
    bool mu = false, mv = false;
    if (s < s1) {
      mu = (sides & 1) && sei0[s] == a;
      mv = (sides & 2) && sei1[s] == a;
    }
    const unsigned long long bu = __ballot(mu), bv = __ballot(mv);
    if (FILL) {
      const int before = count + __popcll(bu & lt) + __popcll(bv & lt);
      if (mu) inc_idx[base + before] = s;
      if (mv) inc_idx[base + before + (mu ? 1 : 0)] = s;
    }
    count += __popcll(bu) + __popcll(bv);
  }
  if (!FILL && lane == 0) inc_cnt[a] = count;
}

__global__ void k_pair_distance(const float* __restrict__ pos, const int64_t* __restrict__ sei0,
                                const int64_t* __restrict__ sei1, int S, float* __restrict__ out) {
  for (int s = blockIdx.x * blockDim.x + threadIdx.x; s < S; s += gridDim.x * blockDim.x) {
    const int64_t u = sei0[s], v = sei1[s];
    out[s] = sqrtf(norm2_rn(pos[3 * u] - pos[3 * v], pos[3 * u + 1] - pos[3 * v + 1], pos[3 * u + 2] - pos[3 * v + 2]));
  }
}

__global__ void k_ddm_views(const float* __restrict__ pos, const float* __restrict__ noise,
                            const int64_t* __restrict__ sei0, const int64_t* __restrict__ sei1, int64_t n3, int S,
                            float* __restrict__ pos2, float* __restrict__ d01, float* __restrict__ d02,
                            const int64_t* __restrict__ z, int64_t zs, int64_t* __restrict__ z2,
                            const int32_t* __restrict__ dyn_N, const int32_t* __restrict__ dyn_S) {
  n3 = 3 * (int64_t)dyn_count((int)(n3 / 3), dyn_N);
  S = dyn_count(S, dyn_S);
  const int64_t t = (int64_t)blockIdx.x * blockDim.x + threadIdx.x, nt = (int64_t)gridDim.x * blockDim.x;
  if (z2 != nullptr)
    for (int64_t i = t; i < n3 / 3; i += nt) {
      const int64_t v = z[i * zs];
      z2[i] = v;
      z2[n3 / 3 + i] = v;
    }
  for (int64_t i = t; i < n3; i += nt) {
    const float a = pos[i];
    pos2[i] = a;
    pos2[n3 + i] = add_rn(a, noise[i]);
  }
  for (int64_t s = t; s < S; s += nt) {
    const int64_t u = sei0[s], v = sei1[s];
    const float ux = pos[3 * u], uy = pos[3 * u + 1], uz = pos[3 * u + 2];
    const float vx = pos[3 * v], vy = pos[3 * v + 1], vz = pos[3 * v + 2];
    d01[s] = sqrtf(norm2_rn(ux - vx, uy - vy, uz - vz));
    const float px = add_rn(ux, noise[3 * u]), py = add_rn(uy, noise[3 * u + 1]), pz = add_rn(uz, noise[3 * u + 2]);
    const float qx = add_rn(vx, noise[3 * v]), qy = add_rn(vy, noise[3 * v + 1]), qz = add_rn(vz, noise[3 * v + 2]);
    d02[s] = sqrtf(norm2_rn(px - qx, py - qy, pz - qz));
  }
}

__global__ void k_copy2(uint32_t* __restrict__ d0, const uint32_t* __restrict__ s0, int64_t n0,
                        uint32_t* __restrict__ d1, const uint32_t* __restrict__ s1, int64_t n1) {
  const int64_t t = (int64_t)blockIdx.x * blockDim.x + threadIdx.x, nt = (int64_t)gridDim.x * blockDim.x;
  for (int64_t i = t; i < n0; i += nt) d0[i] = s0[i];
  for (int64_t i = t; i < n1; i += nt) d1[i] = s1[i];
}

__device__ __forceinline__ uint4 philox4x32_10(uint4 c, uint2 k) {
#pragma unroll
  for (int r = 0; r < 10; ++r) {
    const uint32_t hi0 = __umulhi(0xD2511F53u, c.x), lo0 = 0xD2511F53u * c.x;
    const uint32_t hi1 = __umulhi(0xCD9E8D57u, c.z), lo1 = 0xCD9E8D57u * c.z;
    c = make_uint4(hi1 ^ c.y ^ k.x, lo1, hi0 ^ c.w ^ k.y, lo0);
    k.x += 0x9E3779B9u;
    k.y += 0xBB67AE85u;
  }
  return c;
}
__device__ __forceinline__ void normal4(uint4 r, float (&z)[4]) {
  const float u0 = ((float)(r.x >> 8) + 1.0f) * (1.0f / 16777216.0f), u1 = (float)(r.y >> 8) * (1.0f / 16777216.0f);
  const float u2 = ((float)(r.z >> 8) + 1.0f) * (1.0f / 16777216.0f), u3 = (float)(r.w >> 8) * (1.0f / 16777216.0f);
  const float ra = sqrtf(-2.0f * logf(u0)), rb = sqrtf(-2.0f * logf(u2));
  float sa, ca, sb, cb;
  sincosf(6.283185307179586f * u1, &sa, &ca);
  sincosf(6.283185307179586f * u3, &sb, &cb);
  z[0] = ra * ca; z[1] = ra * sa; z[2] = rb * cb; z[3] = rb * sb;
}
__global__ void k_ddm_noise(const int64_t* __restrict__ seed, uint64_t seed_value, float mu, float sigma, int64_t n_pos,
                            int64_t S, int64_t B, int K1, int K2, float* __restrict__ pos_noise,
                            int64_t* __restrict__ nl1, float* __restrict__ dn1, int64_t* __restrict__ nl2,
                            float* __restrict__ dn2) {
  const uint64_t sd = seed != nullptr ? (uint64_t)seed[0] : seed_value;
  const uint2 key = make_uint2((uint32_t)sd, (uint32_t)(sd >> 32));
  const int64_t g_pos = (n_pos + 3) / 4, g_s = (S + 3) / 4, g_b = (B + 3) / 4;
  const int64_t total = g_pos + 2 * g_s + 2 * g_b;
  for (int64_t t = (int64_t)blockIdx.x * blockDim.x + threadIdx.x; t < total; t += (int64_t)gridDim.x * blockDim.x) {
    int seg;
    int64_t g = t;
    if (g < g_pos) seg = 0;
    else if ((g -= g_pos) < g_s) seg = 1;
    else if ((g -= g_s) < g_s) seg = 2;
    else if ((g -= g_s) < g_b) seg = 3;
    else { g -= g_b; seg = 4; }
    const uint4 r = philox4x32_10(make_uint4((uint32_t)g, (uint32_t)(g >> 32), (uint32_t)seg, 0u), key);
    if (seg <= 2) {
      float z[4];
      normal4(r, z);
      float* dst = seg == 0 ? pos_noise : (seg == 1 ? dn1 : dn2);
      const int64_t n = seg == 0 ? n_pos : S;
      const float m = seg == 0 ? mu : 0.0f, sg = seg == 0 ? sigma : 1.0f;
#pragma unroll
      for (int e = 0; e < 4; ++e)
        if (4 * g + e < n) dst[4 * g + e] = add_rn(mul_rn(z[e], sg), m);
    } else {
      int64_t* dst = seg == 3 ? nl1 : nl2;
      const uint32_t K = (uint32_t)(seg == 3 ? K1 : K2);
      const uint32_t v[4] = {r.x, r.y, r.z, r.w};
#pragma unroll
      for (int e = 0; e < 4; ++e)
        if (4 * g + e < B) dst[4 * g + e] = (int64_t)(v[e] % K);
    }
  }
}

__global__ void k_axpy(const float* __restrict__ a, const float* __restrict__ b, float alpha, int64_t n,
                       float* __restrict__ out) {
  for (int64_t i = (int64_t)blockIdx.x * blockDim.x + threadIdx.x; i < n; i += (int64_t)gridDim.x * blockDim.x)
    out[i] = a[i] + alpha * b[i];
}

inline int grid1d(int64_t n, int block, int cap = 2048) {
  int64_t g = (n + block - 1) / block;
  return (int)(g < 1 ? 1 : (g > cap ? cap : g));
}

}

extern "C" int geossl_layout_build(const int64_t* batch, int64_t N, int64_t B, int32_t* mol_ptr, int32_t* pair_ptr,
                                   int64_t* stats, hipStream_t stream) {
  hipLaunchKernelGGL(k_layout_build, dim3(1), dim3(1024), 0, stream, batch, (int)N, (int)B, mol_ptr, pair_ptr, stats);
  GEOSSL_CHECK_LAUNCH();
  return 0;
}

extern "C" int geossl_pair_index_fill(const int32_t* mol_ptr, const int32_t* pair_ptr, int64_t B, int32_t* pair_i,
                                      int32_t* pair_j, hipStream_t stream) {
  if (B <= 0) return 0;
  hipLaunchKernelGGL(k_pair_index_fill, dim3((unsigned)B), dim3(64), 0, stream, mol_ptr, pair_ptr, (int)B, pair_i,
                     pair_j);
  GEOSSL_CHECK_LAUNCH();
  return 0;
}

extern "C" int geossl_atom_tuples(const int32_t* mol_ptr, const int64_t* tuple_ptr, int64_t B, int option,
                                  int64_t* out0, int64_t* out1, hipStream_t stream) {
  if (B <= 0) return 0;
  if (option != 0 && option != 1) return (int)hipErrorInvalidValue;
  hipLaunchKernelGGL(k_atom_tuples, dim3((unsigned)B), dim3(64), 0, stream, mol_ptr, tuple_ptr, (int)B, option, out0,
                     out1);
  GEOSSL_CHECK_LAUNCH();
  return 0;
}

extern "C" int geossl_radius_graph_count(const float* pos, const int32_t* mol_ptr, int64_t B, int max_n, float r2,
                                         int cap, int32_t* deg, hipStream_t stream) {
  if (B <= 0) return 0;
  if (max_n < 1 || max_n > GEOSSL_RADIUS_MAX_N) return (int)hipErrorInvalidValue;
  allow_big_lds(&k_radius<0>);
  hipLaunchKernelGGL((k_radius<0>), dim3((unsigned)B), dim3(64), radius_lds(max_n), stream, pos, mol_ptr, nullptr,
                     (int)B, max_n, r2, cap, deg, nullptr, nullptr, nullptr, nullptr, nullptr, nullptr, 1.0f, nullptr);
  GEOSSL_CHECK_LAUNCH();
  return 0;
}

extern "C" int geossl_radius_graph_fill(const float* pos, const int32_t* mol_ptr, int64_t B, int max_n, float r2,
                                        int cap, const int64_t* edge_ptr, int64_t* edge_src, int64_t* edge_dst,
                                        float* edge_weight, hipStream_t stream) {
  if (B <= 0) return 0;
  if (max_n < 1 || max_n > GEOSSL_RADIUS_MAX_N) return (int)hipErrorInvalidValue;
  allow_big_lds(&k_radius<1>);
  hipLaunchKernelGGL((k_radius<1>), dim3((unsigned)B), dim3(64), radius_lds(max_n), stream, pos, mol_ptr, nullptr,
                     (int)B, max_n, r2, cap, nullptr, edge_ptr, edge_src, edge_dst, edge_weight, nullptr, nullptr, 1.0f,
                     nullptr);
  GEOSSL_CHECK_LAUNCH();
  return 0;
}

extern "C" int geossl_pair_geometry(const float* pos, const int32_t* mol_ptr, const int32_t* pair_ptr, int64_t B,
                                    int max_n, float r2, int cap, float cutoff, float* pair_d, float* pair_c,
                                    uint8_t* pair_flag, hipStream_t stream) {
  if (B <= 0) return 0;
  if (max_n <= cap && max_n <= 64) {
    hipLaunchKernelGGL(k_pair_geometry_flat, dim3((unsigned)B), dim3(64), 0, stream, pos, mol_ptr, pair_ptr, (int)B, r2,
                       cutoff, pair_d, pair_c, pair_flag);
    GEOSSL_CHECK_LAUNCH();
    return 0;
  }
  if (max_n < 1 || max_n > GEOSSL_RADIUS_MAX_N) return (int)hipErrorInvalidValue;
  allow_big_lds(&k_radius<2>);
  hipLaunchKernelGGL((k_radius<2>), dim3((unsigned)B), dim3(64), radius_lds(max_n), stream, pos, mol_ptr, pair_ptr,
                     (int)B, max_n, r2, cap, nullptr, nullptr, nullptr, nullptr, nullptr, pair_d, pair_flag, cutoff, pair_c);
  GEOSSL_CHECK_LAUNCH();
  return 0;
}

extern "C" int geossl_super_edge_ptr(const int64_t* batch, const int64_t* sei0, const int64_t* sei1, int64_t S,
                                     int64_t B, int32_t* se_ptr, int64_t* stats, hipStream_t stream) {
  hipLaunchKernelGGL(k_super_edge_ptr, dim3(grid1d(S > B ? S : B + 1, 256)), dim3(256), 0, stream, batch, sei0, sei1,
                     (int)S, (int)B, se_ptr, stats);
  GEOSSL_CHECK_LAUNCH();
  return 0;
}

extern "C" int geossl_incidence_count(const int64_t* batch, const int64_t* sei0, const int64_t* sei1,
                                      const int32_t* se_ptr, int64_t N, int sides, int32_t* inc_cnt,
                                      hipStream_t stream) {
  if (N <= 0) return 0;
  hipLaunchKernelGGL((k_incidence<0>), dim3((unsigned)((N + 3) / 4)), dim3(256), 0, stream, batch, sei0, sei1, se_ptr,
                     (int)N, sides, inc_cnt, nullptr, nullptr);
  GEOSSL_CHECK_LAUNCH();
  return 0;
}

extern "C" int geossl_incidence_fill(const int64_t* batch, const int64_t* sei0, const int64_t* sei1,
                                     const int32_t* se_ptr, int64_t N, int sides, const int64_t* inc_ptr,
                                     int32_t* inc_idx, hipStream_t stream) {
  if (N <= 0) return 0;
  hipLaunchKernelGGL((k_incidence<1>), dim3((unsigned)((N + 3) / 4)), dim3(256), 0, stream, batch, sei0, sei1, se_ptr,
                     (int)N, sides, nullptr, inc_ptr, inc_idx);
  GEOSSL_CHECK_LAUNCH();
  return 0;
}

extern "C" int geossl_pair_distance(const float* pos, const int64_t* sei0, const int64_t* sei1, int64_t S, float* out,
                                    hipStream_t stream) {
  if (S <= 0) return 0;
  hipLaunchKernelGGL(k_pair_distance, dim3(grid1d(S, 256)), dim3(256), 0, stream, pos, sei0, sei1, (int)S, out);
  GEOSSL_CHECK_LAUNCH();
  return 0;
}

extern "C" int geossl_ddm_views_dyn(const float* pos, const float* noise, const int64_t* sei0, const int64_t* sei1,
                                    int64_t N, int64_t S, float* pos2, float* d01, float* d02, const int64_t* z,
                                    int64_t z_stride, int64_t* z2, const int32_t* dyn_N, const int32_t* dyn_S,
                                    hipStream_t stream) {
  if (N <= 0) return 0;
  const int64_t work = 3 * N > S ? 3 * N : S;
  hipLaunchKernelGGL(k_ddm_views, dim3(grid1d(work, 256)), dim3(256), 0, stream, pos, noise, sei0, sei1, 3 * N, (int)S,
                     pos2, d01, d02, z, z_stride, z2, dyn_N, dyn_S);
  GEOSSL_CHECK_LAUNCH();
  return 0;
}

extern "C" int geossl_ddm_views(const float* pos, const float* noise, const int64_t* sei0, const int64_t* sei1, int64_t N,
                                int64_t S, float* pos2, float* d01, float* d02, const int64_t* z, int64_t z_stride,
                                int64_t* z2, hipStream_t stream) {
  return geossl_ddm_views_dyn(pos, noise, sei0, sei1, N, S, pos2, d01, d02, z, z_stride, z2, nullptr, nullptr, stream);
}

extern "C" int geossl_copy2(void* dst0, const void* src0, int64_t bytes0, void* dst1, const void* src1, int64_t bytes1,
                            hipStream_t stream) {
  if ((bytes0 | bytes1) & 3) return (int)hipErrorInvalidValue;
  if (((uintptr_t)dst0 | (uintptr_t)src0 | (uintptr_t)dst1 | (uintptr_t)src1) & 3) return (int)hipErrorInvalidValue;
  const int64_t n0 = bytes0 / 4, n1 = bytes1 / 4, work = n0 > n1 ? n0 : n1;
  if (work <= 0) return 0;
  hipLaunchKernelGGL(k_copy2, dim3(grid1d(work, 256)), dim3(256), 0, stream, (uint32_t*)dst0, (const uint32_t*)src0, n0,
                     (uint32_t*)dst1, (const uint32_t*)src1, n1);
  GEOSSL_CHECK_LAUNCH();
  return 0;
}

namespace {
__global__ void k_copy_n(GeosslCopyBatch b) {
  const uint32_t* __restrict__ s = reinterpret_cast<const uint32_t*>(b.src[blockIdx.y]);
  uint32_t* __restrict__ d = reinterpret_cast<uint32_t*>(b.dst[blockIdx.y]);
  const int64_t n = b.bytes[blockIdx.y] / 4;
  const int64_t t0 = (int64_t)blockIdx.x * blockDim.x + threadIdx.x, nt = (int64_t)gridDim.x * blockDim.x;
  if (s == nullptr) {
    for (int64_t i = t0; i < n; i += nt) d[i] = 0u;
    return;
  }
  for (int64_t i = t0; i < n; i += nt) d[i] = s[i];
}
}

extern "C" int geossl_copy_n(const GeosslCopyBatch* batch, int n, hipStream_t stream) {
  if (batch == nullptr || n < 0 || n > GEOSSL_COPY_MAX) return (int)hipErrorInvalidValue;
  int64_t work = 0;
  for (int i = 0; i < n; ++i) {
    if ((batch->bytes[i] & 3) || (((uintptr_t)batch->dst[i] | (uintptr_t)batch->src[i]) & 3) || batch->bytes[i] < 0 ||
        (batch->dst[i] == nullptr && batch->bytes[i] > 0))
      return (int)hipErrorInvalidValue;
    if (batch->bytes[i] / 4 > work) work = batch->bytes[i] / 4;
  }
  if (n == 0 || work <= 0) return 0;
  hipLaunchKernelGGL(k_copy_n, dim3(grid1d(work, 256, 512), n), dim3(256), 0, stream, *batch);
  GEOSSL_CHECK_LAUNCH();
  return 0;
}

static int ddm_noise_launch(const int64_t* seed, uint64_t seed_value, float mu, float sigma, int64_t n_pos, int64_t S,
                            int64_t B, int K1, int K2, float* pos_noise, int64_t* noise_level_1,
                            float* distance_noise_1, int64_t* noise_level_2, float* distance_noise_2,
                            hipStream_t stream) {
  if (K1 < 1 || K2 < 1) return (int)hipErrorInvalidValue;
  const int64_t total = (n_pos + 3) / 4 + 2 * ((S + 3) / 4) + 2 * ((B + 3) / 4);
  if (total <= 0) return 0;
  hipLaunchKernelGGL(k_ddm_noise, dim3(grid1d(total, 256)), dim3(256), 0, stream, seed, seed_value, mu, sigma, n_pos, S, B,
                     K1, K2, pos_noise, noise_level_1, distance_noise_1, noise_level_2, distance_noise_2);
  GEOSSL_CHECK_LAUNCH();
  return 0;
}

extern "C" int geossl_ddm_noise(const int64_t* seed, float mu, float sigma, int64_t n_pos, int64_t S, int64_t B, int K1,
                                int K2, float* pos_noise, int64_t* noise_level_1, float* distance_noise_1,
                                int64_t* noise_level_2, float* distance_noise_2, hipStream_t stream) {
  if (seed == nullptr) return (int)hipErrorInvalidValue;
  return ddm_noise_launch(seed, 0, mu, sigma, n_pos, S, B, K1, K2, pos_noise, noise_level_1, distance_noise_1,
                          noise_level_2, distance_noise_2, stream);
}

extern "C" int geossl_ddm_noise_seeded(uint64_t seed, float mu, float sigma, int64_t n_pos, int64_t S, int64_t B, int K1,
                                       int K2, float* pos_noise, int64_t* noise_level_1, float* distance_noise_1,
                                       int64_t* noise_level_2, float* distance_noise_2, hipStream_t stream) {
  return ddm_noise_launch(nullptr, seed, mu, sigma, n_pos, S, B, K1, K2, pos_noise, noise_level_1, distance_noise_1,
                          noise_level_2, distance_noise_2, stream);
}

extern "C" int geossl_axpy(const float* a, const float* b, float alpha, int64_t n, float* out, hipStream_t stream) {
  if (n <= 0) return 0;
  hipLaunchKernelGGL(k_axpy, dim3(grid1d(n, 256)), dim3(256), 0, stream, a, b, alpha, n, out);
  GEOSSL_CHECK_LAUNCH();
  return 0;
}
```

### geossl_amd/csrc/sparse_pairs.hip

```cpp
#include "common.h"
#include "radius_adj.h"
#include "geossl_hip.h"

using namespace geossl;

namespace {

constexpr int SP_THREADS = 256, SP_WAVES = SP_THREADS / 64;
constexpr unsigned SP_FWD = 1u << 30, SP_BWD = 1u << 31, SP_ATOM = SP_FWD - 1u;

__host__ __device__ inline int sp_stride(int max_n) { return ((max_n + 63) / 64) | 1; }

struct SpLds {
  unsigned long long* adj;
  float* sp;
  int* up;
  int* inc;
  int* s_a;
  int* s_b;
  int* s_wcnt;
};
inline size_t sp_lds_bytes(int max_n) {
  return (size_t)max_n * sp_stride(max_n) * 8 + (size_t)max_n * 12 + 2 * (size_t)(max_n + 1) * 4 +
         (2 * SP_THREADS + 2 * 4 * SP_WAVES) * 4;
}
__device__ __forceinline__ SpLds sp_carve(unsigned char* raw, int max_n) {
  SpLds L;
  L.adj = reinterpret_cast<unsigned long long*>(raw);
  L.sp = reinterpret_cast<float*>(L.adj + (size_t)max_n * sp_stride(max_n));
  L.up = reinterpret_cast<int*>(L.sp + 3 * (size_t)max_n);
  L.inc = L.up + max_n + 1;
  L.s_a = L.inc + max_n + 1;
  L.s_b = L.s_a + SP_THREADS;
  L.s_wcnt = L.s_b + SP_THREADS;
  return L;
}

__device__ __forceinline__ void sp_adjacency(const float* __restrict__ pos, int a0, int n, int ws, float r2, int cap,
                                             const SpLds& L) {
  const int tid = threadIdx.x, lane = tid & 63, wave = tid >> 6;
  for (int i = tid; i < 3 * n; i += SP_THREADS) L.sp[i] = pos[(size_t)a0 * 3 + i];
  __syncthreads();
  for (int i = wave; i < n; i += SP_WAVES)
    radius_scan_target(L.sp, n, i, lane, r2, cap, [&](int c, int, float, bool, unsigned long long kept, int) {
      if (lane == 0) L.adj[(size_t)i * ws + c] = kept;
    });
  __syncthreads();
}

__global__ __launch_bounds__(SP_THREADS) void k_sparse_count(const float* __restrict__ pos,
                                                             const int32_t* __restrict__ mol_ptr, int B, int max_n,
                                                             float r2, int cap, int32_t* __restrict__ mol_cnt,
                                                             int32_t* __restrict__ up_cnt, int32_t* __restrict__ lo_cnt) {
  extern __shared__ __attribute__((aligned(16))) unsigned char smem_raw[];
  const int m = blockIdx.x;
  if (m >= B) return;
  const int tid = threadIdx.x, lane = tid & 63, wave = tid >> 6;
  const int a0 = mol_ptr[m], n = mol_ptr[m + 1] - a0, ws = sp_stride(max_n);
  const SpLds L = sp_carve(smem_raw, max_n);
  int* s_tot = L.s_a;
  sp_adjacency(pos, a0, n, ws, r2, cap, L);
  int tot = 0;
  for (int a = wave; a < n; a += SP_WAVES) {
    const int wa = a >> 6, ba = a & 63;
    int up = 0, lo = 0;
    for (int c = 0; c * 64 < n; ++c) {
      const int b = c * 64 + lane;
      const unsigned long long row = L.adj[(size_t)a * ws + c];
      bool on = false;
      if (b < n && b != a) on = (((row >> lane) | (L.adj[(size_t)b * ws + wa] >> ba)) & 1ull) != 0ull;
      const unsigned long long mk = __ballot(on);
      if (c < wa) lo += __popcll(mk);
      else if (c > wa) up += __popcll(mk);
      else {
        lo += __popcll(mk & ((1ull << ba) - 1ull));
        up += __popcll((mk >> ba) >> 1);
      }
    }
    if (lane == 0) {
      up_cnt[a0 + a] = up;
      lo_cnt[a0 + a] = lo;
    }
    tot += up;
  }
  if (lane == 0) s_tot[wave] = tot;
  __syncthreads();
  if (tid == 0) {
    int t = 0;
    for (int w = 0; w < SP_WAVES; ++w) t += s_tot[w];
    mol_cnt[m] = t;
  }
}

__global__ __launch_bounds__(SP_THREADS) void k_sparse_fill(
    const float* __restrict__ pos, const int32_t* __restrict__ mol_ptr, int B, int N, int max_n, float r2, int cap,
    float cutoff, const int32_t* __restrict__ mol_cnt, const int32_t* __restrict__ up_cnt,
    const int32_t* __restrict__ lo_cnt, int Pcap, int32_t* __restrict__ pair_i, int32_t* __restrict__ pair_j,
    float* __restrict__ pair_d, float* __restrict__ pair_c, uint8_t* __restrict__ pair_flag,
    int32_t* __restrict__ inc_ptr, int32_t* __restrict__ inc_pair, uint32_t* __restrict__ inc_src,
    int32_t* __restrict__ n_pairs) {
  extern __shared__ __attribute__((aligned(16))) unsigned char smem_raw[];
  const int m = blockIdx.x;
  if (m >= B) return;
  const int tid = threadIdx.x, lane = tid & 63, wave = tid >> 6;
  const int a0 = mol_ptr[m], n = mol_ptr[m + 1] - a0, ws = sp_stride(max_n);
  const SpLds L = sp_carve(smem_raw, max_n);
  int* s_a = L.s_a;
  int* s_b = L.s_b;
  int(*s_wcnt)[4][SP_WAVES] = reinterpret_cast<int(*)[4][SP_WAVES]>(L.s_wcnt);
  {
    int before = 0, all = 0;
    for (int k = tid; k < B; k += SP_THREADS) {
      const int v = mol_cnt[k];
      all += v;
      if (k < m) before += v;
    }
    s_a[tid] = before;
    s_b[tid] = all;
    __syncthreads();
    for (int o = SP_THREADS / 2; o > 0; o >>= 1) {
      if (tid < o) {
        s_a[tid] += s_a[tid + o];
        s_b[tid] += s_b[tid + o];
      }
      __syncthreads();
    }
  }
  const int base = s_a[0], total = min(s_b[0], Pcap);
  __syncthreads();
  if (m == 0 && tid == 0) n_pairs[0] = total;
  if (m == B - 1 && tid == 0) inc_ptr[N] = 2 * total;
  for (int p = total + m * SP_THREADS + tid; p < Pcap; p += B * SP_THREADS) {
    pair_i[p] = 0;
    pair_j[p] = 0;
    pair_d[p] = cutoff;
    pair_c[p] = 0.0f;
    pair_flag[p] = 0;
  }
  sp_adjacency(pos, a0, n, ws, r2, cap, L);
  {
    int va[4], vb[4], ta = 0, tb = 0;
#pragma unroll
    for (int q = 0; q < 4; ++q) {
      const int a = 4 * tid + q;
      va[q] = a < n ? up_cnt[a0 + a] : 0;
      vb[q] = a < n ? va[q] + lo_cnt[a0 + a] : 0;
      ta += va[q];
      tb += vb[q];
    }
    s_a[tid] = ta;
    s_b[tid] = tb;
    __syncthreads();
    for (int o = 1; o < SP_THREADS; o <<= 1) {
      const int xa = tid >= o ? s_a[tid - o] : 0, xb = tid >= o ? s_b[tid - o] : 0;
      __syncthreads();
      s_a[tid] += xa;
      s_b[tid] += xb;
      __syncthreads();
    }
    int ea = s_a[tid] - ta, eb = s_b[tid] - tb;
#pragma unroll
    for (int q = 0; q < 4; ++q) {
      const int a = 4 * tid + q;
      if (a < n) {
        L.up[a] = ea;
        L.inc[a] = eb;
        inc_ptr[a0 + a] = 2 * base + eb;
      }
      ea += va[q];
      eb += vb[q];
    }
    if (tid == 0) {
      L.up[n] = s_a[SP_THREADS - 1];
      L.inc[n] = s_b[SP_THREADS - 1];
    }
    __syncthreads();
  }
  const unsigned long long lt = (lane == 0) ? 0ull : (~0ull >> (64 - lane));
  const int nS = (n + SP_THREADS - 1) / SP_THREADS;
  int colcnt[4] = {0, 0, 0, 0};
  for (int a = 0; a + 1 < n; ++a) {
    const int par = a & 1, wa = a >> 6, ba = a & 63;
    unsigned fl[4];
    unsigned long long msk[4];
#pragma unroll
    for (int s = 0; s < 4; ++s) {
      fl[s] = 0u;
      msk[s] = 0ull;
      if (s < nS && SP_THREADS * s + SP_THREADS - 1 > a) {
        const int b = SP_THREADS * s + tid;
        if (b < n && b > a) {
          const unsigned f0 = (unsigned)((L.adj[(size_t)a * ws + (b >> 6)] >> lane) & 1ull);
          const unsigned f1 = (unsigned)((L.adj[(size_t)b * ws + wa] >> ba) & 1ull);
          fl[s] = f0 | (f1 << 1);
        }
        msk[s] = __ballot(fl[s] != 0u);
      }
      if (lane == 0) s_wcnt[par][s][wave] = __popcll(msk[s]);
    }
    __syncthreads();
    const int up0 = L.up[a];
    const int lo_a = (L.inc[a + 1] - L.inc[a]) - (L.up[a + 1] - up0);
    const int inc_a = 2 * base + L.inc[a] + lo_a;
    int run = 0;
#pragma unroll
    for (int s = 0; s < 4; ++s) {
      int mine = 0;
#pragma unroll
      for (int w = 0; w < SP_WAVES; ++w) {
        if (w == wave) mine = run;
        run += s_wcnt[par][s][w];
      }
      if (fl[s] != 0u) {
        const int b = SP_THREADS * s + tid;
        const int rank = mine + __popcll(msk[s] & lt);
        const int p = base + up0 + rank;
        if (p < Pcap) {
          const unsigned f0 = fl[s] & 1u, f1 = fl[s] >> 1;
          const float d = sqrtf(dist2_nofma(L.sp + 3 * a, L.sp + 3 * b));
          pair_i[p] = a0 + a;
          pair_j[p] = a0 + b;
          pair_d[p] = d;
          pair_c[p] = pair_envelope(d, cutoff);
          pair_flag[p] = (uint8_t)fl[s];
          const int ku = min(inc_a + rank, 2 * Pcap - 1), kl = min(2 * base + L.inc[b] + colcnt[s], 2 * Pcap - 1);
          inc_pair[ku] = p;
          inc_src[ku] = (unsigned)(a0 + b) | (f0 ? SP_FWD : 0u) | (f1 ? SP_BWD : 0u);
          inc_pair[kl] = p;
          inc_src[kl] = (unsigned)(a0 + a) | (f1 ? SP_FWD : 0u) | (f0 ? SP_BWD : 0u);
        }
        colcnt[s] += 1;
      }
    }
  }
}

template <int VW>
__global__ __launch_bounds__(SP_THREADS) void k_aggregate_sparse(const float* __restrict__ x,
                                                                 const float* __restrict__ Wf,
                                                                 const int32_t* __restrict__ inc_ptr,
                                                                 const int32_t* __restrict__ inc_pair,
                                                                 const uint32_t* __restrict__ inc_src, int N, int F,
                                                                 int swap, float* __restrict__ out) {
#pragma clang fp contract(off)
  typedef float V __attribute__((ext_vector_type(VW)));
  const int per = gridDim.x / 8;
  const int blk = (blockIdx.x & 7) * per + (blockIdx.x >> 3);
  const int t = blk * SP_WAVES + (threadIdx.x >> 6), lane = threadIdx.x & 63;
  if (t >= N) return;
  const bool col = VW * lane < F;
  const int f = col ? VW * lane : 0;
  const int k0 = inc_ptr[t], k1 = inc_ptr[t + 1];
  const unsigned dir = swap ? SP_BWD : SP_FWD;
  V acc = V(0.0f);
  for (int kb = k0; kb < k1; kb += 64) {
    const int k = min(kb + lane, k1 - 1);
    const unsigned src = inc_src[k];
    const int row = inc_pair[k];
    unsigned long long mk = __ballot(kb + lane < k1 && (src & dir) != 0u);
    while (mk != 0ull) {
      V xv[4], wv[4];
      bool live[4];
#pragma unroll
      for (int q = 0; q < 4; ++q) {
        live[q] = mk != 0ull;
        const int u = live[q] ? __builtin_ctzll(mk) : 0;
        mk &= mk - 1ull;
        const unsigned s_u = (unsigned)__builtin_amdgcn_readlane((int)src, u) & SP_ATOM;
        const int r_u = __builtin_amdgcn_readlane(row, u);
        xv[q] = *reinterpret_cast<const V*>(x + (size_t)s_u * F + f);
        wv[q] = *reinterpret_cast<const V*>(Wf + (size_t)r_u * F + f);
      }
#pragma unroll
      for (int q = 0; q < 4; ++q) {
        const V tq = xv[q] * wv[q];
        const V sq = acc + tq;
        acc = live[q] ? sq : acc;
      }
    }
  }
  if (col) *reinterpret_cast<V*>(out + (size_t)t * F + f) = acc;
}

__global__ __launch_bounds__(64) void k_pair_position_grad_sparse(const float* __restrict__ pos,
                                                                  const float* __restrict__ pair_d,
                                                                  const float* __restrict__ dd,
                                                                  const int32_t* __restrict__ inc_ptr,
                                                                  const int32_t* __restrict__ inc_pair,
                                                                  const uint32_t* __restrict__ inc_src, int N, int64_t P,
                                                                  int L, float* __restrict__ dpos) {
  const int t = blockIdx.x * 64 + threadIdx.x;
  if (t >= N) return;
  const float px = pos[3 * (size_t)t], py = pos[3 * (size_t)t + 1], pz = pos[3 * (size_t)t + 2];
  float gx = 0.0f, gy = 0.0f, gz = 0.0f;
  const int k1 = inc_ptr[t + 1];
  for (int k = inc_ptr[t]; k < k1; ++k) {
    const int row = inc_pair[k];
    const size_t b = inc_src[k] & SP_ATOM;
    float s = 0.0f;
    for (int l = 0; l < L; ++l) s += dd[(size_t)l * P + row];
    const float dist = pair_d[row];
    if (s != 0.0f && dist > 0.0f) {
      const float k_ = s / dist;
      gx += k_ * (px - pos[3 * b]);
      gy += k_ * (py - pos[3 * b + 1]);
      gz += k_ * (pz - pos[3 * b + 2]);
    }
  }
  dpos[3 * (size_t)t] = gx;
  dpos[3 * (size_t)t + 1] = gy;
  dpos[3 * (size_t)t + 2] = gz;
}

}

extern "C" int geossl_sparse_pairs_build(const float* pos, const int32_t* mol_ptr, int64_t B, int64_t N, int max_n,
                                         float r2, int cap, float cutoff, int64_t capacity, int32_t* mol_cnt,
                                         int32_t* up_cnt, int32_t* lo_cnt, int32_t* pair_i, int32_t* pair_j,
                                         float* pair_d, float* pair_c, uint8_t* pair_flag, int32_t* inc_ptr,
                                         int32_t* inc_pair, uint32_t* inc_src, int32_t* n_pairs, hipStream_t stream) {
  if (max_n < 1 || max_n > GEOSSL_RADIUS_MAX_N || B <= 0 || N <= 0 || capacity < 0 || capacity > (1ll << 29))
    return (int)hipErrorInvalidValue;
  const size_t lds = sp_lds_bytes(max_n);
  allow_big_lds(&k_sparse_count);
  allow_big_lds(&k_sparse_fill);
  hipLaunchKernelGGL(k_sparse_count, dim3((unsigned)B), dim3(SP_THREADS), lds, stream, pos, mol_ptr, (int)B, max_n, r2, cap,
                     mol_cnt, up_cnt, lo_cnt);
  GEOSSL_CHECK_LAUNCH();
  hipLaunchKernelGGL(k_sparse_fill, dim3((unsigned)B), dim3(SP_THREADS), lds, stream, pos, mol_ptr, (int)B, (int)N, max_n,
                     r2, cap, cutoff, mol_cnt, up_cnt, lo_cnt, (int)capacity, pair_i, pair_j, pair_d, pair_c, pair_flag,
                     inc_ptr, inc_pair, inc_src, n_pairs);
  GEOSSL_CHECK_LAUNCH();
  return 0;
}

extern "C" int geossl_cfconv_aggregate_sparse(const float* x, const float* Wf, const int32_t* inc_ptr,
                                              const int32_t* inc_pair, const uint32_t* inc_src, int64_t N, int F,
                                              int swap, float* out, hipStream_t stream) {
  if (N <= 0) return 0;
  if (F != 32 && F != 64 && F != 128) return (int)hipErrorInvalidValue;
  const unsigned blocks = (unsigned)((N + SP_WAVES - 1) / SP_WAVES), grid = 8 * ((blocks + 7) / 8);
  if (F == 128)
    hipLaunchKernelGGL(k_aggregate_sparse<2>, dim3(grid), dim3(SP_THREADS), 0, stream, x, Wf, inc_ptr, inc_pair, inc_src,
                       (int)N, F, swap, out);
  else
    hipLaunchKernelGGL(k_aggregate_sparse<1>, dim3(grid), dim3(SP_THREADS), 0, stream, x, Wf, inc_ptr, inc_pair, inc_src,
                       (int)N, F, swap, out);
  GEOSSL_CHECK_LAUNCH();
  return 0;
}

extern "C" int geossl_pair_position_grad_sparse(const float* pos, const float* pair_d, const float* dd,
                                                const int32_t* inc_ptr, const int32_t* inc_pair,
                                                const uint32_t* inc_src, int64_t N, int64_t P, int L, float* dpos,
                                                hipStream_t stream) {
  if (N <= 0) return 0;
  hipLaunchKernelGGL(k_pair_position_grad_sparse, dim3((unsigned)((N + 63) / 64)), dim3(64), 0, stream, pos, pair_d, dd,
                     inc_ptr, inc_pair, inc_src, (int)N, P, L, dpos);
  GEOSSL_CHECK_LAUNCH();
  return 0;
}
```

### geossl_amd/ops.py

```python
import ctypes as C
import math
import os

import numpy as np
import torch
from .switches import env as _env

from . import _lib
from ._lib import call, ptr, stream
from .layout import MolLayout, SPARSE_MAX_N, get_layout

PI_F32 = float(torch.tensor(math.pi, dtype=torch.float32))
RAGGED_LOOP_MAX_MOLS = int(_env("GEOSSL_RAGGED_LOOP_MAX", 256))


def _f32(t):
    if t.dtype != torch.float32:
        raise TypeError("expected float32, got %s" % t.dtype)
    return t.contiguous()


def radius_cap(max_num_neighbors, loop=False):
    return max_num_neighbors if loop else max_num_neighbors + 1


def _check_graph_size(layout):
    if layout.max_n > SPARSE_MAX_N:
        raise ValueError("the radius graph takes structures of at most %d atoms (the largest here has %d)"
                         % (SPARSE_MAX_N, layout.max_n))


def radius_graph(pos, r, batch=None, loop=False, max_num_neighbors=32, layout=None, return_weight=False):
    _lib.require_cuda(pos)
    if loop:
        raise NotImplementedError("loop=True is not on the GeoSSL path")
    pos = _f32(pos)
    N = pos.size(0)
    if batch is None:
        batch = torch.zeros(N, dtype=torch.long, device=pos.device)
    lay = layout or get_layout(batch)
    _check_graph_size(lay)
    r2 = float(torch.tensor(float(r) * float(r), dtype=torch.float32))
    cap = radius_cap(max_num_neighbors)
    deg = torch.zeros(N, dtype=torch.int32, device=pos.device)
    call("geossl_radius_graph_count", ptr(pos), ptr(lay.mol_ptr), lay.B, lay.max_n, r2, cap, ptr(deg), stream())
    edge_ptr = torch.zeros(N + 1, dtype=torch.int64, device=pos.device)
    edge_ptr[1:] = torch.cumsum(deg, 0, dtype=torch.int64)
    E = int(edge_ptr[-1].item())
    edge_index = torch.empty(2, E, dtype=torch.int64, device=pos.device)
    weight = torch.empty(E, dtype=torch.float32, device=pos.device)
    if E > 0:
        call("geossl_radius_graph_fill", ptr(pos), ptr(lay.mol_ptr), lay.B, lay.max_n, r2, cap, ptr(edge_ptr),
             ptr(edge_index[0]), ptr(edge_index[1]), ptr(weight), stream())
    return (edge_index, weight) if return_weight else edge_index


def pair_geometry(pos, layout, cutoff, max_num_neighbors=32):
    if getattr(layout, "sparse", False):
        raise _lib.GeosslHipError("a sparse layout (a structure above 255 atoms, or GEOSSL_SPARSE_PAIRS=1) has no dense "
                                  "pair slots: ops.sparse_pair_geometry builds its pair list")
    _check_graph_size(layout)
    pos = _f32(pos)
    dev = pos.device
    P = layout.P
    pair_d = torch.empty(P, dtype=torch.float32, device=dev)
    pair_c = torch.empty(P, dtype=torch.float32, device=dev)
    pair_flag = torch.empty(P, dtype=torch.uint8, device=dev)
    r2 = float(torch.tensor(float(cutoff) * float(cutoff), dtype=torch.float32))
    if P > 0:
        call("geossl_pair_geometry", ptr(pos), ptr(layout.mol_ptr), ptr(layout.pair_ptr), layout.B, layout.max_n, r2,
             radius_cap(max_num_neighbors), float(cutoff), ptr(pair_d), ptr(pair_c), ptr(pair_flag), stream())
    return pair_d, pair_c, pair_flag


class SparsePairs:

    __slots__ = ("P", "N", "pair_i", "pair_j", "pair_d", "pair_c", "pair_flag", "inc_ptr", "inc_pair", "inc_src",
                 "n_pairs")

    @property
    def dyn_P(self):
        return self.n_pairs.data_ptr()


def sparse_pair_geometry(pos, layout, cutoff, max_num_neighbors=32):
    if not getattr(layout, "sparse", False):
        raise _lib.GeosslHipError("sparse_pair_geometry needs a sparse layout (GEOSSL_SPARSE_PAIRS=1 makes any layout one)")
    _check_graph_size(layout)
    if radius_cap(max_num_neighbors) > 33:
        raise ValueError("the capacity of the sparse pair list is sized for max_num_neighbors <= 32")
    pos = _f32(pos)
    dev, N, P = pos.device, layout.N, layout.P
    i32 = dict(dtype=torch.int32, device=dev)
    sp = SparsePairs()
    sp.P, sp.N = P, N
    sp.pair_i, sp.pair_j = torch.empty(max(P, 1), **i32), torch.empty(max(P, 1), **i32)
    sp.pair_d = torch.empty(max(P, 1), dtype=torch.float32, device=dev)
    sp.pair_c = torch.empty(max(P, 1), dtype=torch.float32, device=dev)
    sp.pair_flag = torch.empty(max(P, 1), dtype=torch.uint8, device=dev)
    sp.inc_ptr = torch.empty(N + 1, **i32)
    sp.inc_pair, sp.inc_src = torch.empty(max(2 * P, 1), **i32), torch.empty(max(2 * P, 1), **i32)
    sp.n_pairs = torch.empty(1, **i32)
    work = torch.empty(layout.B + 2 * N, **i32)
    r2 = float(torch.tensor(float(cutoff) * float(cutoff), dtype=torch.float32))
    call("geossl_sparse_pairs_build", ptr(pos), ptr(layout.mol_ptr), layout.B, N, layout.max_n, r2,
         radius_cap(max_num_neighbors), float(cutoff), P, ptr(work), ptr(work[layout.B:]), ptr(work[layout.B + N:]),
         ptr(sp.pair_i), ptr(sp.pair_j), ptr(sp.pair_d), ptr(sp.pair_c), ptr(sp.pair_flag), ptr(sp.inc_ptr),
         ptr(sp.inc_pair), ptr(sp.inc_src), ptr(sp.n_pairs), stream())
    return sp


def aggregate_sparse(x, Wf_l, pairs, swap=False, out=None):
    N, F = x.shape
    if out is None:
        out = torch.empty_like(x)
    call("geossl_cfconv_aggregate_sparse", ptr(x), ptr(Wf_l), ptr(pairs.inc_ptr), ptr(pairs.inc_pair), ptr(pairs.inc_src),
         N, F, 1 if swap else 0, ptr(out), stream())
    return out


def pair_position_grad_sparse(pos, pairs, dd, out=None):
    N = pos.size(0)
    if out is None:
        out = torch.empty(N, 3, dtype=torch.float32, device=pos.device)
    call("geossl_pair_position_grad_sparse", ptr(pos), ptr(pairs.pair_d), ptr(dd), ptr(pairs.inc_ptr), ptr(pairs.inc_pair),
         ptr(pairs.inc_src), N, pairs.P, dd.size(0), ptr(out), stream())
    return out


def gaussian_smearing(dist, offset, coeff):
    _lib.require_cuda(dist)
    d = _f32(dist).view(-1)
    out = torch.empty(d.numel(), offset.numel(), dtype=torch.float32, device=d.device)
    call("geossl_rbf_fwd", ptr(d), d.numel(), ptr(offset), offset.numel(), float(coeff), ptr(out), stream())
    return out


class PreparedWeight:
    __slots__ = ("image", "K", "NO")

    def __init__(self, image, K, NO):
        self.image, self.K, self.NO = image, K, NO


def prepare_linear(weights, transB=True):
    w0 = weights[0]
    NO, K = (w0.size(0), w0.size(1)) if transB else (w0.size(1), w0.size(0))
    words = int(_lib.load().geossl_linear_image_words(K, NO))
    if words == 0:
        return None
    out = []
    for lo in range(0, len(weights), _lib.TN_MAX):
        chunk = weights[lo:lo + _lib.TN_MAX]
        images = torch.empty(len(chunk), words, dtype=torch.int32, device=w0.device)
        pb = _lib.PrepareBatch()
        for i, w in enumerate(chunk):
            assert w.shape == w0.shape and w.stride(1) == 1
            pb.W[i], pb.image[i] = ptr(w), ptr(images[i])
            pb.ldw[i] = 0 if w.is_contiguous() else w.stride(0)
        call("geossl_linear_prepare", C.byref(pb), len(chunk), K, NO, 1 if transB else 0, stream())
        out += [PreparedWeight(images[i], K, NO) for i in range(len(chunk))]
    return out


def linear(x, w, bias=None, res=None, tprev=None, transB=True, flags=0, out=None, K=None, NO=None):
    R = x.size(0)
    prepared = isinstance(w, PreparedWeight)
    if prepared:
        K, NO = w.K, w.NO
    K = x.size(1) if K is None else K
    NO = (w.size(0) if transB else w.size(1)) if NO is None else NO
    if out is None:
        out = torch.empty(R, NO, dtype=torch.float32, device=x.device)
    if bias is not None:
        flags |= _lib.EPI_BIAS
    if res is not None:
        flags |= _lib.EPI_RESIDUAL
    if tprev is not None:
        flags |= _lib.EPI_MUL_DSSP
    assert x.stride(1) == 1 and out.stride(1) == 1
    for aux in (res, tprev):
        assert aux is None or (aux.stride(0) == out.stride(0) and aux.stride(1) == 1)
    if prepared:
        call("geossl_linear_prepared", ptr(x), x.stride(0), ptr(w.image), ptr(bias), ptr(res), ptr(tprev), ptr(out),
             out.stride(0), R, K, NO, flags, stream())
    else:
        call("geossl_linear", ptr(x), x.stride(0), ptr(w), ptr(bias), ptr(res), ptr(tprev), ptr(out), out.stride(0), R,
             K, NO, 1 if transB else 0, flags, stream())
    return out


def prepare_chain(weights, transB=True, both=False):
    w0 = weights[0]
    F = w0.size(0)
    words = int(_lib.load().geossl_chain_image_words(F)) if w0.size(1) == F else 0
    if words == 0:
        return (None, None) if both else None
    jobs = [(w, 1) for w in weights] + [(w, 2) for w in weights] if both else [(w, 0) for w in weights]
    out = []
    for lo in range(0, len(jobs), _lib.PREPARE_MAX):
        chunk = jobs[lo:lo + _lib.PREPARE_MAX]
        images = torch.empty(len(chunk), words, dtype=torch.int32, device=w0.device)
        pb = _lib.PrepareBatch()
        for i, (w, tb) in enumerate(chunk):
            assert w.shape == w0.shape and w.stride(1) == 1
            pb.W[i], pb.image[i] = ptr(w), ptr(images[i])
            pb.ldw[i] = 0 if w.is_contiguous() else w.stride(0)
            pb.tb[i] = tb
        call("geossl_chain_prepare", C.byref(pb), len(chunk), F, 1 if transB else 0, stream())
        out += [images[i] for i in range(len(chunk))]
    return (out[:len(weights)], out[len(weights):]) if both else out


def _dyn(layout_or_dyn, field):
    d = getattr(layout_or_dyn, "dyn", layout_or_dyn)
    return None if d is None else getattr(d, field)


def linear_chain(x, stages, dyn_rows=None):
    R, F = x.shape
    assert x.stride(1) == 1 and 1 <= len(stages) <= _lib.CHAIN_MAX
    ch = _lib.Chain()
    ch.nstage = len(stages)
    outs = []
    for s, sd in enumerate(stages):
        st = ch.st[s]
        o = sd.get("out")
        if o is None and sd.get("store", True):
            o = torch.empty(R, F, dtype=torch.float32, device=x.device)
        rows_ = [a for a in (o, sd.get("res"), sd.get("tprev"), sd.get("out_act")) if a is not None]
        ld = rows_[0].stride(0) if rows_ else F
        for a in rows_:
            assert a.stride(0) == ld and a.stride(1) == 1 and a.size(0) == R and a.size(1) == F
        st.image, st.bias, st.res, st.tprev, st.out = (ptr(sd["image"]), ptr(sd.get("bias")), ptr(sd.get("res")),
                                                       ptr(sd.get("tprev")), ptr(o))
        st.out_act = ptr(sd.get("out_act"))
        st.ld, st.flags = ld, int(sd.get("flags", 0)) | (_lib.CHAIN_SAME_INPUT if sd.get("same_input") else 0)
        xin = sd.get("x")
        if xin is not None:
            assert s > 0 and xin.stride(1) == 1 and xin.size(0) == R and xin.size(1) == F
            st.xin, st.ldxin = ptr(xin), xin.stride(0)
            st.flags |= _lib.CHAIN_NEW_INPUT | (_lib.CHAIN_ADD_PREV if sd.get("add_prev") else 0)
        else:
            st.xin, st.ldxin = None, 0
        outs.append(o)
    call("geossl_linear_chain_dyn", ptr(x), x.stride(0), C.byref(ch), R, F, dyn_rows, stream())
    return outs


_LOOP_WORDS, _LOOP_STAGE0, _LOOP_STAGE_WORDS = 50, 5, 9
assert C.sizeof(_lib.LoopOp) == 8 * _LOOP_WORDS and _lib.LoopOp.chain.offset == 32 and _lib.Chain.st.offset == 8 \
    and C.sizeof(_lib.ChainStage) == 8 * _LOOP_STAGE_WORDS and _lib.ChainStage.ld.offset == 40 \
    and _lib.ChainStage.out_act.offset == 64


def layer_loop(ops_list, layout, pair_flag, N, F, stagger=0):
    plan, nblk = layout.loop_plan()
    ragged = (plan is None and F == 128 and 1 < layout.max_n <= 33 and layout.B <= RAGGED_LOOP_MAX_MOLS
              and not _env("GEOSSL_NO_RAGGED_LOOP") and len(ops_list) <= _lib.LOOP_MAX_OPS)
    if not ragged and (plan is None or F != 128 or not layout.uniform or layout.max_n > 20
                       or len(ops_list) > _lib.LOOP_MAX_OPS):
        return False
    words = [0] * (_LOOP_WORDS * len(ops_list))
    dp = lambda t_: 0 if t_ is None else t_.data_ptr()
    for i, op in enumerate(ops_list):
        b = _LOOP_WORDS * i
        if op[0] == "chain":
            _, x, stages = op
            assert x.shape == (N, F) and x.is_contiguous() and len(stages) <= 3
            words[b + 1], words[b + 4] = x.data_ptr(), len(stages)
            for s, sd in enumerate(stages):
                w = b + _LOOP_STAGE0 + _LOOP_STAGE_WORDS * s
                o, r, tp = sd.get("out"), sd.get("res"), sd.get("tprev")
                for a in (o, r, tp):
                    assert a is None or (a.shape == (N, F) and a.is_contiguous())
                words[w], words[w + 1], words[w + 2], words[w + 3], words[w + 4] = (
                    sd["image"].data_ptr(), dp(sd.get("bias")), dp(r), dp(tp), dp(o))
                words[w + 5] = F | (int(sd.get("flags", 0)) << 32)
        else:
            _, x, Wf_l, out, swap = op
            words[b], words[b + 1], words[b + 2], words[b + 3] = 1 | ((1 if swap else 0) << 32), x.data_ptr(), \
                Wf_l.data_ptr(), out.data_ptr()
    arr = np.array(words, dtype=np.uint64)
    if ragged:
        call("geossl_schnet_layer_loop_ragged", arr.ctypes.data, len(ops_list), ptr(layout.mol_ptr), ptr(layout.pair_ptr),
             ptr(pair_flag), layout.B, 1 if layout.B <= 512 else 2, N, F, stream())
        return True
    call("geossl_schnet_layer_loop", arr.ctypes.data, len(ops_list), ptr(plan), nblk, ptr(layout.mol_ptr),
         ptr(layout.pair_ptr), ptr(pair_flag), layout.max_n, 1 if layout.uniform else 0, N, F, int(stagger), stream())
    return True


def linear_wgrad(problems, R, M, N, accumulate=False, lda=None, ldb=None, ldw=None, dyn_rows=None):
    dev = problems[0][0].device
    lda, ldb, ldw = lda or M, ldb or N, ldw or N
    for lo in range(0, len(problems), _lib.TN_MAX):
        chunk = problems[lo:lo + _lib.TN_MAX]
        tb = _lib.TnBatch()
        for i, (A, Bm, dW, db) in enumerate(chunk):
            tb.A[i], tb.B[i], tb.dW[i], tb.db[i] = ptr(A), ptr(Bm), ptr(dW), ptr(db)
        nfl = _lib.load().geossl_tn_workspace_floats(R, M, N, len(chunk))
        ws = torch.empty(nfl, dtype=torch.float32, device=dev)
        call("geossl_linear_wgrad_dyn", C.byref(tb), len(chunk), R, M, N, lda, ldb, ldw, ptr(ws), 1 if accumulate else 0,
             dyn_rows, stream())


def aggregate(x, Wf_l, pair_flag, layout, swap=False, out=None, mols=None):
    N, F = x.shape
    if out is None:
        out = torch.empty_like(x)
    work = getattr(layout, "agg_work", None)
    if mols is None and work is not None and 32 < F <= 128:
        call("geossl_cfconv_aggregate_targets_dyn" if getattr(layout, "agg_targets", False)
             else "geossl_cfconv_aggregate_work_dyn", ptr(x), ptr(Wf_l), ptr(pair_flag), ptr(layout.mol_ptr),
             ptr(layout.pair_ptr), ptr(work), work.numel(), layout.max_n, F, 1 if swap else 0, ptr(out),
             _dyn(layout, "n_work"), stream())
        return out
    if getattr(layout, "dyn", None) is not None:
        raise _lib.GeosslHipError("a capacity-bucket layout needs the work-list aggregation (64 or 128 features)")
    if mols is None:
        mp, pp, order, B = ptr(layout.mol_ptr), ptr(layout.pair_ptr), layout.order, layout.B
    else:
        m0, m1, order = mols
        B = m1 - m0
        if order is not None:
            mp, pp = ptr(layout.mol_ptr), ptr(layout.pair_ptr)
        else:
            mp, pp = ptr(layout.mol_ptr) + 4 * m0, ptr(layout.pair_ptr) + 4 * m0
    call("geossl_cfconv_aggregate", ptr(x), ptr(Wf_l), ptr(pair_flag), mp, pp, ptr(order), B, layout.max_n, F,
         1 if swap else 0, ptr(out), stream())
    return out


def pair_product(a, b, layout, pair_flag, swap=False):
    N, F = a.shape
    out = torch.empty(layout.P, F, dtype=torch.float32, device=a.device)
    call("geossl_pair_product", ptr(a), ptr(b), ptr(layout.pair_i), ptr(layout.pair_j), ptr(pair_flag), layout.P, F,
         1 if swap else 0, ptr(out), stream())
    return out


def segment_reduce(h, layout, reduce):
    out = torch.empty(layout.B, h.size(1), dtype=torch.float32, device=h.device)
    call("geossl_segment_reduce_fwd", ptr(h), ptr(layout.mol_ptr), layout.B, h.size(1), 1 if reduce == "mean" else 0,
         ptr(out), stream())
    return out


def pair_distance(pos, sei0, sei1):
    pos = _f32(pos)
    S = sei0.numel()
    out = torch.empty(S, 1, dtype=torch.float32, device=pos.device)
    call("geossl_pair_distance", ptr(pos), ptr(sei0), ptr(sei1), S, ptr(out), stream())
    return out


def ddm_views(pos, noise, sei0, sei1, z=None, dyn=None):
    pos, noise = _f32(pos), _f32(noise)
    N, S = pos.size(0), sei0.numel()
    pos2 = torch.empty(2 * N, 3, dtype=torch.float32, device=pos.device)
    d01 = torch.empty(S, 1, dtype=torch.float32, device=pos.device)
    d02 = torch.empty(S, 1, dtype=torch.float32, device=pos.device)
    z2 = None
    if z is not None:
        assert z.dim() == 1 and z.dtype == torch.long and z.numel() == N
        z2 = torch.empty(2 * N, dtype=torch.long, device=pos.device)
    call("geossl_ddm_views_dyn", ptr(pos), ptr(noise), ptr(sei0), ptr(sei1), N, S, ptr(pos2), ptr(d01), ptr(d02), ptr(z),
         z.stride(0) if z is not None and N > 0 else 1, ptr(z2), _dyn(dyn, "n_atoms"), _dyn(dyn, "n_super"), stream())
    return (pos2, d01, d02) if z is None else (pos2, d01, d02, z2)


def add_scaled(a, b, alpha=1.0):
    a, b = _f32(a), _f32(b)
    out = torch.empty_like(a)
    call("geossl_axpy", ptr(a), ptr(b), float(alpha), a.numel(), ptr(out), stream())
# ... 615 lines not shown
```

### include/geossl_hip.h

```cpp
#ifndef GEOSSL_HIP_H
#define GEOSSL_HIP_H
#include <stdint.h>
#ifdef __HIPCC__
#include <hip/hip_runtime.h>
#else
typedef struct ihipStream_t* hipStream_t;
#endif

#ifdef __cplusplus
extern "C" {
#endif

#define GEOSSL_ABI_VERSION 1
#define GEOSSL_MAX_L 12
#define GEOSSL_TN_MAX 32
#define GEOSSL_LOSS_PARTIALS 256

#define GEOSSL_EPI_BIAS 1
#define GEOSSL_EPI_SSP 2
#define GEOSSL_EPI_RESIDUAL 4
#define GEOSSL_EPI_MUL_DSSP 8
#define GEOSSL_CHAIN_NEW_INPUT 32
#define GEOSSL_CHAIN_ADD_PREV 64
#define GEOSSL_EPI_SILU 128
// ... 270 lines not shown
int geossl_painn_interaction_fwd_mma(const float* q, const float* mu, const float* xc, const int64_t* idx_j,
                                     const int32_t* row_edge, const int32_t* grp_atom, const int32_t* mol_grp,
                                     const float* phi, const float* fcut, const float* dir, const float* Wf,
                                     const float* bf, const int32_t* mol_ptr, int64_t B, int max_n, int64_t N, int F, int R,
                                     float* q_out, float* mu_out, hipStream_t stream);
int geossl_painn_interaction_fwd_mol(const float* q, const float* mu, const float* xc, const int64_t* idx_j,
                                     const int64_t* inc_ptr, const int32_t* inc_idx, const float* phi, const float* fcut,
                                     const float* dir, const float* Wf, const float* bf, const int32_t* mol_ptr,
                                     int64_t B, int max_n, int64_t N, int F, int R, float* q_out, float* mu_out,
                                     hipStream_t stream);
int64_t geossl_painn_interaction_bwd_mol_workspace_floats(int64_t N, int64_t B, int F, int R);
int geossl_painn_interaction_bwd_mol(const float* dq_out, const float* dmu_out, const float* mu, const float* xc,
                                     const int64_t* idx_i, const int64_t* inc_ptr, const int32_t* inc_idx,
                                     const float* phi, const float* fcut, const float* dir, const float* Wf,
                                     const float* bf, const int32_t* mol_ptr, int64_t B, int max_n, int64_t N, int F,
                                     int R, float* dxc, float* dmu_in, float* dWf, float* dbf, float* workspace,
                                     int accumulate, hipStream_t stream);
int geossl_painn_mix_pre_fwd(const float* q, const float* mm, int64_t N, int F, float eps, float* ctx, float* dot,
                             hipStream_t stream);
int geossl_painn_mix_post_fwd(const float* q, const float* mu, const float* mm, const float* xx, const float* dot,
                              int64_t N, int F, float* q_out, float* mu_out, hipStream_t stream);
int geossl_painn_mix_post_bwd(const float* dq_new, const float* dmu_new, const float* mm, const float* xx,
                              const float* dot, int64_t N, int F, float* dxx, float* dmm, hipStream_t stream);
int geossl_painn_mix_pre_bwd(const float* dq_new, const float* dctx, const float* ctx, const float* mm, int64_t N, int F,
                             float* dq_in, float* dmm, hipStream_t stream);
int geossl_add(const float* a, const float* b, int64_t n, float* out, hipStream_t stream);

int geossl_painn_edge_grads(const float* dq_out, const float* dmu_out, const float* mu, const float* xc,
                            const int64_t* idx_i, const int64_t* idx_j, const float* phi, const float* fcut,
                            const float* dir, const float* Wf, const float* bf, int64_t E, int F, int R, float* dphi,
                            float* dfcut, float* ddir, int accumulate, hipStream_t stream);
int geossl_painn_edge_geom_bwd(const float* pos, const int64_t* idx_i, const int64_t* idx_j, int64_t E, float cutoff,
                               const float* offsets, const float* widths, int R, const float* dphi, const float* dfcut,
                               const float* ddir, float* dr, hipStream_t stream);
int geossl_painn_position_grad(const float* dr, const int64_t* inc_i_ptr, const int32_t* inc_i_idx,
                               const int64_t* inc_j_ptr, const int32_t* inc_j_idx, int64_t N, float* dpos,
                               hipStream_t stream);

int geossl_adam_step(float* param, const float* grad, float* exp_avg, float* exp_avg_sq, int64_t n, double lr,
                     double beta1, double beta2, double eps, double weight_decay, int64_t step_count, float grad_scale,
                     hipStream_t stream);

#define GEOSSL_COPY_MAX 8
typedef struct GeosslCopyBatch {
  void* dst[GEOSSL_COPY_MAX];
  const void* src[GEOSSL_COPY_MAX];
  int64_t bytes[GEOSSL_COPY_MAX];
} GeosslCopyBatch;
int geossl_copy_n(const GeosslCopyBatch* batch, int n, hipStream_t stream);
int geossl_ddm_views_dyn(const float* pos, const float* noise, const int64_t* sei0, const int64_t* sei1, int64_t N,
                         int64_t S, float* pos2, float* d01, float* d02, const int64_t* z, int64_t z_stride, int64_t* z2,
                         const int32_t* dyn_N, const int32_t* dyn_S, hipStream_t stream);
int geossl_embedding_fwd_dyn(const int64_t* z, int64_t z_stride, const float* table, int num_classes, int64_t N, int F,
                             float* out, int32_t* status, const int32_t* dyn_N, hipStream_t stream);
int geossl_embedding_bwd_dyn(const int64_t* z, int64_t z_stride, const float* dh, int num_classes, int64_t N, int F,
                             float* dtable, float* workspace, int accumulate, const int32_t* dyn_N, hipStream_t stream);
int geossl_cfconv_filter_fwd_dyn(const float* pair_d, const float* pair_c, int64_t P, const GeosslFilterWeights* w, int L,
                                 int F, int G, const float* offset, float coeff, float* T, float* Wf,
                                 const int32_t* dyn_P, hipStream_t stream);
int geossl_cfconv_filter_bwd_dyn(const float* pair_d, const float* pair_c, const uint8_t* pair_flag,
                                 const int32_t* pair_i, const int32_t* pair_j, int64_t P, int64_t N,
                                 const GeosslFilterWeights* w, const GeosslFilterGradIn* g, int L, int F, int G,
                                 const float* offset, float coeff, const float* T, const GeosslFilterGradOut* out,
                                 float* workspace, int accumulate, const int32_t* dyn_P, const int32_t* dyn_N,
                                 hipStream_t stream);
int geossl_cfconv_aggregate_work_dyn(const float* x, const float* Wf, const uint8_t* pair_flag, const int32_t* mol_ptr,
                                     const int32_t* pair_ptr, const int32_t* work, int64_t nwork, int max_n, int F,
                                     int swap, float* out, const int32_t* dyn_nwork, hipStream_t stream);
int geossl_linear_chain_dyn(const float* X, int ldx, const GeosslChain* chain, int64_t R, int F, const int32_t* dyn_R,
                            hipStream_t stream);
int geossl_linear_wgrad_dyn(const GeosslTnBatch* batch, int nprob, int64_t R, int M, int N, int lda, int ldb, int ldw,
                            float* workspace, int accumulate, const int32_t* dyn_R, hipStream_t stream);
int geossl_ddm_loss_fwd2_dyn(const GeosslNcsnHeadFwd* heads, const int64_t* batch, const int64_t* sei0,
                             const int64_t* sei1, int64_t S, int F, const int32_t* dyn_S, const int32_t* dyn_view,
                             hipStream_t stream);
int geossl_ddm_loss_bwd_fused2_dyn(const GeosslNcsnHeadBwd* heads, const int64_t* sei0, const int64_t* sei1, int64_t S,
                                   int64_t N, int F, const int64_t* stats_divisor, const float* gout,
                                   const int64_t* inc_ptr, const int32_t* inc_idx, int accumulate, const int32_t* dyn_S,
                                   const int32_t* dyn_view, hipStream_t stream);

int64_t geossl_painn_group_capacity(int64_t E2, int64_t N2);
int geossl_painn_edge_layout(const int64_t* src_i, const int64_t* src_j, int64_t E, const int32_t* mol_ptr, int64_t N,
                             int64_t B, int64_t N2cap, int64_t* idx_i2, int64_t* idx_j2, int64_t* iptr_i,
                             int32_t* ilist_i, int64_t* iptr_j, int32_t* ilist_j, int32_t* row_edge, int32_t* grp_atom,
                             int32_t* mol_grp, int32_t* mol_grp_end, int32_t* status, hipStream_t stream);
int geossl_painn_edge_geom_dyn(const float* pos, const int64_t* idx_i, const int64_t* idx_j, int64_t E, float cutoff,
                               const float* offsets, const float* widths, int R, float* dir, float* fcut, float* phi,
                               const int32_t* dyn_E, hipStream_t stream);
int geossl_painn_interaction_fwd_mma_dyn(const float* q, const float* mu, const float* xc, const int64_t* idx_j,
                                         const int32_t* row_edge, const int32_t* grp_atom, const int32_t* mol_grp,
                                         const float* phi, const float* fcut, const float* dir, const float* Wf,
                                         const float* bf, const int32_t* mol_ptr, int64_t B, int max_n, int64_t N, int F,
                                         int R, float* q_out, float* mu_out, const int32_t* mol_grp_end,
                                         hipStream_t stream);
int geossl_painn_stage_cap(int kind, int F, int R);
int geossl_painn_interaction_fwd_atoms(const float* q, const float* mu, const float* xc, const int64_t* idx_j,
                                       const int64_t* inc_ptr, const int32_t* inc_idx, const float* phi,
                                       const float* fcut, const float* dir, const float* Wf, const float* bf,
                                       const int32_t* atom_list, int64_t nlist, const int32_t* dyn_nlist, int F, int R,
                                       float* q_out, float* mu_out, hipStream_t stream);
int geossl_painn_interaction_bwd_atoms(const float* dq_out, const float* dmu_out, const float* mu, const float* xc,
                                       const int64_t* idx_i, const int64_t* inc_ptr, const int32_t* inc_idx,
                                       const float* phi, const float* fcut, const float* dir, const float* Wf,
                                       const float* bf, const int32_t* atom_list, int64_t nlist,
                                       const int32_t* dyn_nlist, int F, int R, float* dxc, float* dmu_in, float* dWf,
                                       float* dbf, float* workspace, int accumulate, hipStream_t stream);
int geossl_painn_interaction_bwd_mol_skip(const float* dq_out, const float* dmu_out, const float* mu, const float* xc,
                                          const int64_t* idx_i, const int64_t* inc_ptr, const int32_t* inc_idx,
                                          const float* phi, const float* fcut, const float* dir, const float* Wf,
                                          const float* bf, const int32_t* mol_ptr, int64_t B, int max_n, int64_t N, int F,
                                          int R, float* dxc, float* dmu_in, float* dWf, float* dbf, float* workspace,
                                          int accumulate, hipStream_t stream);
int geossl_painn_mix_pre_fwd_dyn(const float* q, const float* mm, int64_t N, int F, float eps, float* ctx, float* dot,
                                 const int32_t* dyn_N, hipStream_t stream);
int geossl_painn_mix_post_fwd_dyn(const float* q, const float* mu, const float* mm, const float* xx, const float* dot,
                                  int64_t N, int F, float* q_out, float* mu_out, const int32_t* dyn_N,
                                  hipStream_t stream);
int geossl_painn_mix_post_bwd_dyn(const float* dq_new, const float* dmu_new, const float* mm, const float* xx,
                                  const float* dot, int64_t N, int F, float* dxx, float* dmm, const int32_t* dyn_N,
                                  hipStream_t stream);
int geossl_painn_mix_pre_bwd_dyn(const float* dq_new, const float* dctx, const float* ctx, const float* mm, int64_t N,
                                 int F, float* dq_in, float* dmm, const int32_t* dyn_N, hipStream_t stream);

int geossl_tape_unary(int kind, const float* x, int64_t n, float alpha, float beta, float* y, hipStream_t stream);
int geossl_tape_binary(int op, const float* a, int amode, const float* b, int bmode, int64_t R, int D, float scale,
                       float* y, hipStream_t stream);
int64_t geossl_tape_colsum_workspace_floats(int64_t R, int D);
int geossl_tape_reduce(int kind, const float* x, int64_t R, int D, float* y, float* workspace, hipStream_t stream);
int geossl_tape_gather_rows(const float* src, const void* idx, int idx64, int64_t E, int D, float* out,
                            hipStream_t stream);
int geossl_tape_scatter_rows(const float* src, const void* ptr, int ptr64, const int32_t* perm, int64_t N, int D,
                             float* out, hipStream_t stream);
int geossl_tape_copy2d(const float* src, int64_t ld_src, float* dst, int64_t ld_dst, int64_t R, int C,
                       hipStream_t stream);
int geossl_tape_fill(float* dst, int64_t n, float value, hipStream_t stream);

typedef struct GeosslGather {
  const int64_t* x_src;
  const float* pos_src;
  const int32_t* src_off;
  const int32_t* mol_ptr;
  int64_t* x_dst;
  float* pos_dst;
  int64_t* batch_dst;
  const int32_t* se_ptr;
  int64_t* sei0;
  int64_t* sei1;
  const int32_t* pair_ptr2;
  int32_t* pair_i;
  int32_t* pair_j;
  const int64_t* inc_ptr;
  int32_t* inc_idx;
  const int64_t* e0_src;
  const int64_t* e1_src;
  const int32_t* e_src_off;
  const int32_t* e_ptr;
  int64_t* e0_dst;
  int64_t* e1_dst;
  float* zero;
  int64_t zero_count;
  int32_t x_cols;
  int32_t option;
} GeosslGather;
int geossl_gather_molecules(const GeosslGather* g, int64_t B, hipStream_t stream);

typedef struct GeosslMask {
  const int32_t* bond_ptr;
  const int32_t* bond_dst;
  const int32_t* src_n;
  const int64_t* mol_id;
  const int32_t* keep_in;
  int32_t* keep_out;
  const int32_t* e_src_cnt;
  int32_t* e_count;
  uint64_t seed;
  int32_t max_n;
  int32_t pad_;
} GeosslMask;
int geossl_gather_masked_molecules(const GeosslGather* g, const GeosslMask* mask, int64_t B, hipStream_t stream);

int geossl_infonce_fwd(const float* X, const float* Y, int64_t B, int F, float inv_t, float* stats, int32_t* amax,
                       float* loss, int32_t* counts, hipStream_t stream);
int geossl_infonce_bwd(const float* X, const float* Y, const float* stats, const int32_t* amax, int64_t B, int F,
                       float inv_t, const float* gout, float* dX, float* dY, hipStream_t stream);
int geossl_ebm_nce_fwd(const float* X, const float* Y, int64_t B, int F, int num_neg, float* pred, double* terms,
                       int32_t* hits, double* loss, int32_t* counts, hipStream_t stream);
int geossl_ebm_nce_bwd(const float* X, const float* Y, const float* pred, int64_t B, int F, int num_neg,
                       const double* gout, float* dX, float* dY, hipStream_t stream);

int geossl_distance_head_width_ok(int F);
int64_t geossl_distance_head_fwd_workspace_floats(int64_t S);
int64_t geossl_distance_head_bwd_workspace_floats(int64_t N, int F);
int geossl_distance_head_fwd(const float* h, int64_t N, int F, const float* W, const float* bias, const float* pos,
                             const int64_t* sei0, const int64_t* sei1, int64_t S, float* proj, float* pred, float* sgn,
                             float* workspace, float* loss, hipStream_t stream);
int geossl_distance_head_fwd_dyn(const float* h, int64_t N, int F, const float* W, const float* bias, const float* pos,
                                 const int64_t* sei0, const int64_t* sei1, int64_t S, float* proj, float* pred,
                                 float* sgn, float* workspace, float* loss, const int32_t* dyn_N, const int32_t* dyn_S,
                                 hipStream_t stream);
int geossl_distance_head_bwd(const float* h, int64_t N, int F, const float* W, const int64_t* sei0, int64_t S,
                             const float* sgn, const int64_t* inc_ptr, const int32_t* inc_idx, const float* gout,
                             float* dh, float* dW, float* db, float* workspace, int accumulate, hipStream_t stream);
int geossl_distance_head_bwd_dyn(const float* h, int64_t N, int F, const float* W, const int64_t* sei0, int64_t S,
                                 const float* sgn, const int64_t* inc_ptr, const int32_t* inc_idx, const float* gout,
                                 float* dh, float* dW, float* db, float* workspace, int accumulate,
                                 const int32_t* dyn_N, const int32_t* dyn_S, hipStream_t stream);

int64_t geossl_charge_mask_count(int64_t N, double ratio);
int geossl_charge_mask(int64_t* x, int x_cols, int64_t N, double ratio, int C, int64_t* seed, const int64_t* given,
                       int64_t* idx, int64_t* labels, int32_t* k, hipStream_t stream);
int geossl_charge_mask_dyn(int64_t* x, int x_cols, int64_t N, double ratio, int C, int64_t* seed, const int64_t* given,
                           int64_t* idx, int64_t* labels, int32_t* k, const int32_t* dyn_N, hipStream_t stream);
int geossl_charge_head_width_ok(int F, int C);
int64_t geossl_charge_head_fwd_workspace_floats(int64_t K);
int64_t geossl_charge_head_bwd_workspace_floats(int64_t K, int F, int C);
int geossl_charge_head_fwd(const float* h, int64_t N, int F, const float* W, const float* bias, int C,
                           const int64_t* idx, const int64_t* labels, int64_t K, const int32_t* k_dev, float* prob,
                           float* workspace, float* loss, int32_t* status, hipStream_t stream);
int geossl_charge_head_fwd_dyn(const float* h, int64_t N, int F, const float* W, const float* bias, int C,
                               const int64_t* idx, const int64_t* labels, int64_t K, const int32_t* k_dev, float* prob,
                               float* workspace, float* loss, int32_t* status, const int32_t* dyn_N,
                               hipStream_t stream);
int geossl_charge_head_bwd(const float* h, int64_t N, int F, const float* W, int C, const int64_t* idx,
                           const int64_t* labels, int64_t K, const int32_t* k_dev, const float* prob, const float* gout,
                           float* dh, float* dW, float* db, float* workspace, int accumulate, hipStream_t stream);
int geossl_charge_head_bwd_dyn(const float* h, int64_t N, int F, const float* W, int C, const int64_t* idx,
                               const int64_t* labels, int64_t K, const int32_t* k_dev, const float* prob,
                               const float* gout, float* dh, float* dW, float* db, float* workspace, int accumulate,
                               const int32_t* dyn_N, hipStream_t stream);

int geossl_infograph_width_ok(int F);
int64_t geossl_infograph_fwd_workspace_floats(int64_t B);
int geossl_infograph_fwd(const float* x, int64_t N, int F, const float* W, const int32_t* mol_ptr, int64_t B,
                         int readout, const float* m_in, float* s, float* h, float* scores, float* workspace,
                         float* loss, int32_t* counts, hipStream_t stream);
int geossl_infograph_fwd_dyn(const float* x, int64_t N, int F, const float* W, const int32_t* mol_ptr, int64_t B,
                             int readout, const float* m_in, float* s, float* h, float* scores, float* workspace,
                             float* loss, int32_t* counts, const int32_t* dyn_N, hipStream_t stream);
int geossl_infograph_bwd(const float* x, int64_t N, int F, const float* W, const int32_t* mol_ptr, int64_t B,
                         int readout, const float* s, const float* h, const float* scores, const float* gout,
                         float* dx, float* dm, float* dh, hipStream_t stream);
int geossl_infograph_bwd_dyn(const float* x, int64_t N, int F, const float* W, const int32_t* mol_ptr, int64_t B,
                             int readout, const float* s, const float* h, const float* scores, const float* gout,
                             float* dx, float* dm, float* dh, const int32_t* dyn_N, hipStream_t stream);

int geossl_property_width_ok(int F);
int64_t geossl_property_workspace_floats(int64_t B);
int geossl_property_fwd(const float* h, int64_t N, int F, const int32_t* mol_ptr, int64_t B, int readout, int head,
                        const float* W1, const float* b1, const float* W2, const float* b2, const float* y,
                        int64_t y_stride, const float* stats, int loss_kind, float* m, float* z, float* pred,
                        float* workspace, float* loss, hipStream_t stream);
int geossl_property_fwd_dyn(const float* h, int64_t N, int F, const int32_t* mol_ptr, int64_t B, int readout, int head,
                            const float* W1, const float* b1, const float* W2, const float* b2, const float* y,
                            int64_t y_stride, const float* stats, int loss_kind, float* m, float* z, float* pred,
                            float* workspace, float* loss, const int32_t* dyn_N, hipStream_t stream);
int geossl_property_predict(const float* h, int64_t N, int F, const int32_t* mol_ptr, int64_t B, int readout, int head,
                            const float* W1, const float* b1, const float* W2, const float* b2, const float* stats,
                            float* pred, hipStream_t stream);
int geossl_property_predict_dyn(const float* h, int64_t N, int F, const int32_t* mol_ptr, int64_t B, int readout,
                                int head, const float* W1, const float* b1, const float* W2, const float* b2,
                                const float* stats, float* pred, const int32_t* dyn_N, hipStream_t stream);
int geossl_property_bwd(int64_t N, int F, const int32_t* mol_ptr, int64_t B, int readout, int head, const float* W1,
                        const float* W2, const float* m, const float* z, const float* pred, const float* y,
                        int64_t y_stride, const float* stats, int loss_kind, const float* gout, float* dh, float* dz,
                        float* dw, float* db, float* workspace, int accumulate, hipStream_t stream);
int geossl_property_bwd_dyn(int64_t N, int F, const int32_t* mol_ptr, int64_t B, int readout, int head, const float* W1,
                            const float* W2, const float* m, const float* z, const float* pred, const float* y,
                            int64_t y_stride, const float* stats, int loss_kind, const float* gout, float* dh, float* dz,
                            float* dw, float* db, float* workspace, int accumulate, const int32_t* dyn_N,
                            hipStream_t stream);
int geossl_property_targets(const float* y, int64_t M, int T, int task_id, const int64_t* mol_off,
                            const int32_t* src_off, int64_t B, float* out, hipStream_t stream);

int geossl_torsion_head_width_ok(int F);
int64_t geossl_torsion_head_fwd_workspace_floats(int64_t T);
int64_t geossl_torsion_head_bwd_workspace_floats(int64_t N, int F);
int geossl_torsion_head_fwd(const float* h, int64_t N, int F, const float* W, const float* bias, const int64_t* tri0,
                            const int64_t* tri1, const int64_t* tri2, const float* angle, int64_t T, float* proj,
                            float* pred, float* res, float* workspace, float* loss, hipStream_t stream);
int geossl_torsion_head_fwd_dyn(const float* h, int64_t N, int F, const float* W, const float* bias, const int64_t* tri0,
                                const int64_t* tri1, const int64_t* tri2, const float* angle, int64_t T, float* proj,
                                float* pred, float* res, float* workspace, float* loss, const int32_t* dyn_N,
                                const int32_t* dyn_T, hipStream_t stream);
int geossl_torsion_head_bwd(const float* h, int64_t N, int F, const float* W, const int64_t* tri0, const int64_t* tri1,
                            const int64_t* tri2, int64_t T, const float* res, const int32_t* mol_ptr, int64_t B,
                            const float* gout, float* dh, float* dW, float* db, float* workspace, int accumulate,
                            hipStream_t stream);
int geossl_torsion_head_bwd_dyn(const float* h, int64_t N, int F, const float* W, const int64_t* tri0,
                                const int64_t* tri1, const int64_t* tri2, int64_t T, const float* res,
                                const int32_t* mol_ptr, int64_t B, const float* gout, float* dh, float* dW, float* db,
                                float* workspace, int accumulate, const int32_t* dyn_N, const int32_t* dyn_T,
                                hipStream_t stream);
int geossl_triple_angles(const float* pos, int64_t N, const int64_t* tri0, const int64_t* tri1, const int64_t* tri2,
                         int64_t T, float* angle, hipStream_t stream);
int geossl_gather_triples(const int32_t* tri_src, int64_t stride, const float* angle_src, const int32_t* t_src_off,
                          const int32_t* t_ptr, const int32_t* mol_ptr, int64_t B, int64_t* tri0, int64_t* tri1,
                          int64_t* tri2, float* angle_dst, hipStream_t stream);

int geossl_sparse_pairs_build(const float* pos, const int32_t* mol_ptr, int64_t B, int64_t N, int max_n, float r2,
                              int cap, float cutoff, int64_t capacity, int32_t* mol_cnt, int32_t* up_cnt,
                              int32_t* lo_cnt, int32_t* pair_i, int32_t* pair_j, float* pair_d, float* pair_c,
                              uint8_t* pair_flag, int32_t* inc_ptr, int32_t* inc_pair, uint32_t* inc_src,
                              int32_t* n_pairs, hipStream_t stream);
int geossl_cfconv_aggregate_sparse(const float* x, const float* Wf, const int32_t* inc_ptr, const int32_t* inc_pair,
                                   const uint32_t* inc_src, int64_t N, int F, int swap, float* out,
                                   hipStream_t stream);
int geossl_pair_position_grad_sparse(const float* pos, const float* pair_d, const float* dd, const int32_t* inc_ptr,
                                     const int32_t* inc_pair, const uint32_t* inc_src, int64_t N, int64_t P, int L,
                                     float* dpos, hipStream_t stream);

#ifdef __cplusplus
}
#endif
#endif
```

Before: 391,900.

## Compact live pairs so filter MLP runs only on in-cutoff pairs

Adds a live-pair compaction pass in the dense layout. The pair geometry kernel now counts live pairs per molecule, and a build kernel packs the pairs inside the cutoff (distance, cosine, flag, indices, original slot) into a dense list with a device-side count. The filter forward runs over this compacted list and scatters Wf back to the original slots through row_slot, and the filter backward also iterates only over live pairs, gathering saved T rows when needed. This is meant to skip the filter MLP work on padded or out-of-cutoff pair slots, at the cost of extra compaction and gather kernels and additional buffers.

```diff
diff --git a/geossl_amd/Geom3D/models/schnet.py b/geossl_amd/Geom3D/models/schnet.py
--- a/geossl_amd/Geom3D/models/schnet.py
+++ b/geossl_amd/Geom3D/models/schnet.py
@@ -122,7 +122,7 @@
              ptr(status.word), dN2, st)
         if cfg["debug"]:
             status.check()
-        sp = None
+        sp = live = None
         if getattr(lay, "sparse", False):
             if dyn is not None:
                 raise _lib.GeosslHipError("capacity buckets hold molecules of at most 255 atoms (bucket.MAX_N)")
@@ -130,7 +130,12 @@
             pair_d, pair_c, pair_flag, dP2 = sp.pair_d, sp.pair_c, sp.pair_flag, sp.dyn_P
             aggregate = lambda x_, W_, out=None, swap=False, mols=None: ops.aggregate_sparse(x_, W_, sp, swap=swap, out=out)
         else:
-            pair_d, pair_c, pair_flag = ops.pair_geometry(pos, lay, cfg["cutoff"])
+            use_live = (lay.P > 0 and ops.live_pairs_enabled() and (want_params or not ctx.needs_input_grad[1]))
+            live_fwd = use_live and not ctx.needs_input_grad[1]
+            mol_live = torch.empty(lay.B, dtype=torch.int32, device=dev) if use_live else None
+            pair_d, pair_c, pair_flag = ops.pair_geometry(pos, lay, cfg["cutoff"], mol_live=mol_live)
+            if use_live:
+                live = ops.live_pairs(pair_d, pair_c, pair_flag, lay, mol_live, cfg["cutoff"])
             aggregate = lambda x_, W_, out=None, swap=False, mols=None: ops.aggregate(x_, W_, pair_flag, lay, swap=swap,
                                                                                       out=out, mols=mols)
         P = lay.P
@@ -142,7 +147,10 @@
                                or bool(_env("GEOSSL_FILTER_BWD_BF16X3"))
                                or bool(_env("GEOSSL_ARITH_24BIT")))
         T = torch.empty(L, P, F, dtype=torch.float32, device=dev) if keep_T else None
-        if P > 0:
+        if live is not None and live_fwd:
+            call("geossl_cfconv_filter_fwd_rows", ptr(live.pair_d), ptr(live.pair_c), P, C.byref(fw), L, F, G,
+                 ptr(cfg["offset"]), cfg["coeff"], ptr(T), ptr(Wf), live.dyn_P, ptr(live.row_slot), st)
+        elif P > 0:
             call("geossl_cfconv_filter_fwd_dyn", ptr(pair_d), ptr(pair_c), P, C.byref(fw), L, F, G, ptr(cfg["offset"]),
                  cfg["coeff"], ptr(T), ptr(Wf), dP2, st)
         hs, xs, aggs, ts = [], [], [], []
@@ -216,7 +224,8 @@
             ctx.ps = ps
             ctx.params = params
             ctx.saved = dict(pair_d=pair_d, pair_c=pair_c, pair_flag=pair_flag, Wf=Wf, T=T, hs=hs, xs=xs, aggs=aggs,
-                             ts=ts, h_last=h, u=u, img_bwd=img_bwd if cfg["chain"] else None, sparse=sp)
+                             ts=ts, h_last=h, u=u, img_bwd=img_bwd if cfg["chain"] else None, sparse=sp, live=live,
+                             live_T=live is not None and live_fwd)
         return hout
 
     @staticmethod
@@ -346,9 +355,21 @@
                     gout.dw1[l], gout.db1[l], gout.dw2[l], gout.db2[l] = ptr(gl[0]), ptr(gl[1]), ptr(gl[2]), ptr(gl[3])
                 nfl = _lib.load().geossl_cfconv_filter_bwd_workspace_floats(P, L, F, G)
                 ws2 = torch.empty(nfl, dtype=torch.float32, device=dev)
-                call("geossl_cfconv_filter_bwd_dyn", ptr(sv["pair_d"]), ptr(sv["pair_c"]), ptr(sv["pair_flag"]),
-                     ptr(pair_i), ptr(pair_j), P, N, C.byref(fw), C.byref(gin), L, F, G, ptr(cfg["offset"]),
-                     cfg["coeff"], ptr(sv["T"]), C.byref(gout), ptr(ws2), accum, dP2, dN2, st)
+                live = sv.get("live")
+                if live is not None:
+                    T_rows = sv["T"]
+                    if T_rows is not None and not sv["live_T"]:
+                        T_rows = torch.empty_like(T_rows)
+                        call("geossl_gather_live_rows", ptr(sv["T"]), ptr(live.row_slot), ptr(live.n_live), P, L, F,
+                             ptr(T_rows), st)
+                    call("geossl_cfconv_filter_bwd_dyn", ptr(live.pair_d), ptr(live.pair_c), ptr(live.pair_flag),
+                         ptr(live.pair_i), ptr(live.pair_j), P, N, C.byref(fw), C.byref(gin), L, F, G,
+                         ptr(cfg["offset"]), cfg["coeff"], ptr(T_rows), C.byref(gout), ptr(ws2), accum, live.dyn_P,
+                         dN2, st)
+                else:
+                    call("geossl_cfconv_filter_bwd_dyn", ptr(sv["pair_d"]), ptr(sv["pair_c"]), ptr(sv["pair_flag"]),
+                         ptr(pair_i), ptr(pair_j), P, N, C.byref(fw), C.byref(gin), L, F, G, ptr(cfg["offset"]),
+                         cfg["coeff"], ptr(sv["T"]), C.byref(gout), ptr(ws2), accum, dP2, dN2, st)
             elif not direct:
                 for gl in g_layers:
                     for k in range(4):
diff --git a/geossl_amd/_lib.py b/geossl_amd/_lib.py
--- a/geossl_amd/_lib.py
+++ b/geossl_amd/_lib.py
@@ -283,6 +283,10 @@
     "geossl_sparse_pairs_build": (i32, [vp, vp, i64, i64, i32, f32, i32, f32, i64] + [vp] * 13),
     "geossl_cfconv_aggregate_sparse": (i32, [vp, vp, vp, vp, vp, i64, i32, i32, vp, vp]),
     "geossl_pair_position_grad_sparse": (i32, [vp, vp, vp, vp, vp, vp, i64, i64, i32, vp, vp]),
+    "geossl_pair_geometry_live": (i32, [vp, vp, vp, i64, i32, f32, i32, f32, vp, vp, vp, vp, vp]),
+    "geossl_gather_live_rows": (i32, [vp, vp, vp, i64, i32, i32, vp, vp]),
+    "geossl_live_pairs_build": (i32, [vp] * 8 + [i64, i64, f32] + [vp] * 9),
+    "geossl_cfconv_filter_fwd_rows": (i32, [vp, vp, i64, P(FilterWeights), i32, i32, i32, vp, f32, vp, vp, vp, vp, vp]),
 }
 
 _lib = None
@@ -409,6 +413,8 @@
         CALLS += 1
     timers = TIMERS
     key = name[:-4] if name.endswith("_dyn") else name
+    if key == "geossl_cfconv_filter_fwd_rows":
+        key = "geossl_cfconv_filter_fwd"
     if timers is not None and key in timers:
         e0, e1 = torch.cuda.Event(enable_timing=True), torch.cuda.Event(enable_timing=True)
         e0.record()
diff --git a/geossl_amd/csrc/filter_fwd.hip b/geossl_amd/csrc/filter_fwd.hip
--- a/geossl_amd/csrc/filter_fwd.hip
+++ b/geossl_amd/csrc/filter_fwd.hip
@@ -19,13 +19,14 @@
 #define FF_MARK(slot) do {} while (0)
 #endif
 
-template <int NMB, int K1S>
-__global__ __launch_bounds__(512) void k_filter_fwd(const float* __restrict__ pair_d,
+template <int NMB, int K1S, bool MAP>
+__device__ __forceinline__ void filter_fwd_body(const float* __restrict__ pair_d,
                                                     const float* __restrict__ pair_c, int P,
-                                                    GeosslFilterWeights w, int G,
+                                                    const GeosslFilterWeights& w, int G,
                                                     const float* __restrict__ offset, float coeff,
                                                     float* __restrict__ Tout, float* __restrict__ Wf,
-                                                    const int32_t* __restrict__ dyn_P) {
+                                                    const int32_t* __restrict__ dyn_P,
+                                                    const int32_t* __restrict__ row_slot) {
   constexpr int F = 32 * NMB, K2S = F / 16;
   extern __shared__ __attribute__((aligned(16))) uint8_t smem_raw[];
   u32x4* W2f = reinterpret_cast<u32x4*>(smem_raw);
@@ -91,6 +92,7 @@
     const bool live = row < P;
     const float d = live ? pair_d[row] : 0.0f;
     const float cw = live ? pair_c[row] : 0.0f;
+    const int slot = MAP ? (live ? row_slot[row] : 0) : row;
     f32x16 acc1[NMB];
 #pragma unroll
     for (int mb = 0; mb < NMB; ++mb)
@@ -158,7 +160,7 @@
     __builtin_amdgcn_sched_barrier(0);
     FF_MARK(3);
     constexpr int MP = NMB >= 2 ? 2 : 1;
-    float* orow = Wf + (lbase + row) * F + 4 * kh;
+    float* orow = Wf + (lbase + slot) * F + 4 * kh;
 #pragma unroll
     for (int mb0 = 0; mb0 < NMB; mb0 += MP) {
       f32x16 acc2[MP];
@@ -227,18 +229,35 @@
   }
 }
 
-
+template <int NMB, int K1S>
+__global__ __launch_bounds__(512) void k_filter_fwd(const float* __restrict__ pair_d, const float* __restrict__ pair_c,
+                                                    int P, GeosslFilterWeights w, int G,
+                                                    const float* __restrict__ offset, float coeff,
+                                                    float* __restrict__ Tout, float* __restrict__ Wf,
+                                                    const int32_t* __restrict__ dyn_P) {
+  filter_fwd_body<NMB, K1S, false>(pair_d, pair_c, P, w, G, offset, coeff, Tout, Wf, dyn_P, nullptr);
+}
+template <int NMB, int K1S>
+__global__ __launch_bounds__(512) void k_filter_fwd_rows(const float* __restrict__ pair_d,
+                                                         const float* __restrict__ pair_c, int P, GeosslFilterWeights w,
+                                                         int G, const float* __restrict__ offset, float coeff,
+                                                         float* __restrict__ Tout, float* __restrict__ Wf,
+                                                         const int32_t* __restrict__ dyn_P,
+                                                         const int32_t* __restrict__ row_slot) {
+  filter_fwd_body<NMB, K1S, true>(pair_d, pair_c, P, w, G, offset, coeff, Tout, Wf, dyn_P, row_slot);
+}
 
 #ifndef FFH_THREADS
 #define FFH_THREADS 512
 #endif
-template <int NMB, int K1S>
-__global__ __launch_bounds__(FFH_THREADS) void k_filter_fwd_h(const float* __restrict__ pair_d,
+template <int NMB, int K1S, bool MAP>
+__device__ __forceinline__ void filter_fwd_h_body(const float* __restrict__ pair_d,
                                                       const float* __restrict__ pair_c, int P,
-                                                      GeosslFilterWeights w, int G,
+                                                      const GeosslFilterWeights& w, int G,
                                                       const float* __restrict__ offset, float coeff,
                                                       float* __restrict__ Tout, float* __restrict__ Wf,
-                                                    const int32_t* __restrict__ dyn_P) {
+                                                    const int32_t* __restrict__ dyn_P,
+                                                    const int32_t* __restrict__ row_slot) {
   constexpr int F = 32 * NMB, K2S = F / 16;
   extern __shared__ __attribute__((aligned(16))) uint8_t smem_raw[];
   u32x4* W2f = reinterpret_cast<u32x4*>(smem_raw);
@@ -319,14 +338,17 @@
   };
   int rb = take();
   float d_n = pair_d[min(32 * rb + j, P - 1)], cw_n = pair_c[min(32 * rb + j, P - 1)];
+  int slot_n = MAP ? row_slot[min(32 * rb + j, P - 1)] : 0;
   while (rb < nrb) {
     const int row = 32 * rb + j;
     const bool live = row < P;
     const float d = d_n;
     const float cw = live ? cw_n : 0.0f;
+    const int slot = MAP ? slot_n : row;
     const int rb_next = take();
     d_n = pair_d[min(32 * rb_next + j, P - 1)];
     cw_n = pair_c[min(32 * rb_next + j, P - 1)];
+    if (MAP) slot_n = row_slot[min(32 * rb_next + j, P - 1)];
     int z = 0;
     asm volatile("" : "+v"(z));
     const int lz = lane + z, khz = 4 * kh + z;
@@ -389,7 +411,7 @@
       tb[ks] = split8h_scaled(v, st);
     }
     constexpr int MP = NMB >= 2 ? 2 : 1;
-    float* orow = Wf + (lbase + row) * F + 4 * kh;
+    float* orow = Wf + (lbase + slot) * F + 4 * kh;
 #pragma unroll
     for (int mb0 = 0; mb0 < NMB; mb0 += MP) {
       f32x16 acc2[MP];
@@ -427,6 +449,26 @@
   }
 }
 
+template <int NMB, int K1S>
+__global__ __launch_bounds__(FFH_THREADS) void k_filter_fwd_h(const float* __restrict__ pair_d,
+                                                              const float* __restrict__ pair_c, int P,
+                                                              GeosslFilterWeights w, int G,
+                                                              const float* __restrict__ offset, float coeff,
+                                                              float* __restrict__ Tout, float* __restrict__ Wf,
+                                                              const int32_t* __restrict__ dyn_P) {
+  filter_fwd_h_body<NMB, K1S, false>(pair_d, pair_c, P, w, G, offset, coeff, Tout, Wf, dyn_P, nullptr);
+}
+template <int NMB, int K1S>
+__global__ __launch_bounds__(FFH_THREADS) void k_filter_fwd_rows_h(const float* __restrict__ pair_d,
+                                                                   const float* __restrict__ pair_c, int P,
+                                                                   GeosslFilterWeights w, int G,
+                                                                   const float* __restrict__ offset, float coeff,
+                                                                   float* __restrict__ Tout, float* __restrict__ Wf,
+                                                                   const int32_t* __restrict__ dyn_P,
+                                                                   const int32_t* __restrict__ row_slot) {
+  filter_fwd_h_body<NMB, K1S, true>(pair_d, pair_c, P, w, G, offset, coeff, Tout, Wf, dyn_P, row_slot);
+}
+
 #ifdef FF_TIMING
 }
 extern "C" int geossl_filter_fwd_debug_read(long long* host) {
@@ -447,6 +489,13 @@
                                             const GeosslFilterWeights* w, int L, int F, int G, const float* offset,
                                             float coeff, float* T, float* Wf, const int32_t* dyn_P,
                                             hipStream_t stream) {
+  return geossl_cfconv_filter_fwd_rows(pair_d, pair_c, P, w, L, F, G, offset, coeff, T, Wf, dyn_P, nullptr, stream);
+}
+
+extern "C" int geossl_cfconv_filter_fwd_rows(const float* pair_d, const float* pair_c, int64_t P,
+                                             const GeosslFilterWeights* w, int L, int F, int G, const float* offset,
+                                             float coeff, float* T, float* Wf, const int32_t* dyn_P,
+                                             const int32_t* row_slot, hipStream_t stream) {
   if (P <= 0 || L <= 0) return 0;
   if (L > GEOSSL_MAX_L || (F != 32 && F != 64 && F != 128) || G > 64 || G < 1) return (int)hipErrorInvalidValue;
   const int nrb = (int)((P + 31) / 32);
@@ -457,9 +506,15 @@
 #define LAUNCH(NMB, K1S)                                                                                        \
   do {                                                                                                          \
     const size_t lds = (size_t)(NMB * (2 * NMB) + NMB * K1S) * 3 * 1024 + (2 * 32 * NMB + 16 * K1S) * 4;        \
-    allow_big_lds(&k_filter_fwd<NMB, K1S>);                                                                     \
-    hipLaunchKernelGGL((k_filter_fwd<NMB, K1S>), grid, dim3(512), lds, stream, pair_d, pair_c, (int)P, *w, G,   \
-                       offset, coeff, T, Wf, dyn_P);                                                            \
+    if (row_slot != nullptr) {                                                                                  \
+      allow_big_lds(&k_filter_fwd_rows<NMB, K1S>);                                                              \
+      hipLaunchKernelGGL((k_filter_fwd_rows<NMB, K1S>), grid, dim3(512), lds, stream, pair_d, pair_c, (int)P,   \
+                         *w, G, offset, coeff, T, Wf, dyn_P, row_slot);                                         \
+    } else {                                                                                                    \
+      allow_big_lds(&k_filter_fwd<NMB, K1S>);                                                                   \
+      hipLaunchKernelGGL((k_filter_fwd<NMB, K1S>), grid, dim3(512), lds, stream, pair_d, pair_c, (int)P,        \
+                         *w, G, offset, coeff, T, Wf, dyn_P);                                                   \
+    }                                                                                                           \
   } while (0)
 #define LAUNCH_F(NMB)                   \
   do {                                  \
@@ -472,9 +527,15 @@
 #define LAUNCH_H(NMB, K1S)                                                                                      \
   do {                                                                                                          \
     const size_t lds = (size_t)(NMB * (2 * NMB) + NMB * K1S) * 2 * 1024 + (2 * 32 * NMB + 16 * K1S + 36) * 4;   \
-    allow_big_lds(&k_filter_fwd_h<NMB, K1S>);                                                                   \
-    hipLaunchKernelGGL((k_filter_fwd_h<NMB, K1S>), grid, dim3(FFH_THREADS), lds, stream, pair_d, pair_c, (int)P, *w, G, \
-                       offset, coeff, T, Wf, dyn_P);                                                            \
+    if (row_slot != nullptr) {                                                                                  \
+      allow_big_lds(&k_filter_fwd_rows_h<NMB, K1S>);                                                            \
+      hipLaunchKernelGGL((k_filter_fwd_rows_h<NMB, K1S>), grid, dim3(FFH_THREADS), lds, stream, pair_d, pair_c, \
+                         (int)P, *w, G, offset, coeff, T, Wf, dyn_P, row_slot);                                 \
+    } else {                                                                                                    \
+      allow_big_lds(&k_filter_fwd_h<NMB, K1S>);                                                                 \
+      hipLaunchKernelGGL((k_filter_fwd_h<NMB, K1S>), grid, dim3(FFH_THREADS), lds, stream, pair_d, pair_c,      \
+                         (int)P, *w, G, offset, coeff, T, Wf, dyn_P);                                           \
+    }                                                                                                           \
   } while (0)
 #define LAUNCH_HF(NMB)                    \
   do {                                    \
diff --git a/geossl_amd/csrc/graph.hip b/geossl_amd/csrc/graph.hip
--- a/geossl_amd/csrc/graph.hip
+++ b/geossl_amd/csrc/graph.hip
@@ -114,7 +114,7 @@
                                                int64_t* __restrict__ edge_src, int64_t* __restrict__ edge_dst,
                                                float* __restrict__ edge_weight, float* __restrict__ pair_d,
                                                uint8_t* __restrict__ pair_flag, float cutoff,
-                                               float* __restrict__ pair_c) {
+                                               float* __restrict__ pair_c, int32_t* __restrict__ mol_live) {
   extern __shared__ __attribute__((aligned(16))) unsigned char smem_raw[];
   const int m = blockIdx.x;
   if (m >= B) return;
@@ -144,6 +144,7 @@
   if (MODE == 2) {
     __syncthreads();
     const int base = pair_ptr[m];
+    int cnt = 0;
     for (int a = 0; a + 1 < n; ++a) {
       const int row = base + a * n - a * (a + 1) / 2 - a - 1;
       for (int b = a + 1 + lane; b < n; b += 64) {
@@ -154,15 +155,18 @@
         pair_d[row + b] = d;
         pair_c[row + b] = pair_envelope(d, cutoff);
         pair_flag[row + b] = (uint8_t)(f0 | (f1 << 1));
+        cnt += __popcll(__ballot((f0 | f1) != 0u));
       }
     }
+    if (mol_live != nullptr && lane == 0) mol_live[m] = cnt;
   }
 }
 
 __global__ __launch_bounds__(64) void k_pair_geometry_flat(const float* __restrict__ pos, const int32_t* __restrict__ mol_ptr,
                                                            const int32_t* __restrict__ pair_ptr, int B, float r2,
                                                            float cutoff, float* __restrict__ pair_d,
-                                                           float* __restrict__ pair_c, uint8_t* __restrict__ pair_flag) {
+                                                           float* __restrict__ pair_c, uint8_t* __restrict__ pair_flag,
+                                                           int32_t* __restrict__ mol_live) {
   __shared__ float sp[3 * 64];
   const int m = blockIdx.x, lane = threadIdx.x;
   if (m >= B) return;
@@ -171,6 +175,7 @@
   for (int i = lane; i < 3 * n; i += 64) sp[i] = pos[(size_t)a0 * 3 + i];
   __syncthreads();
   const float tn = (float)(2 * n - 1);
+  int cnt = 0;
   for (int q = lane; q < np; q += 64) {
     int a = (int)((tn - sqrtf(fmaxf(tn * tn - 8.0f * (float)q, 0.0f))) * 0.5f);
     a = min(max(a, 0), n - 2);
@@ -182,7 +187,9 @@
     pair_d[base + q] = d;
     pair_c[base + q] = pair_envelope(d, cutoff);
     pair_flag[base + q] = d2 < r2 ? (uint8_t)3 : (uint8_t)0;
-  }
+    cnt += __popcll(__ballot(d2 < r2));
+  }
+  if (mol_live != nullptr && lane == 0) mol_live[m] = cnt;
 }
 
 __global__ void k_super_edge_ptr(const int64_t* __restrict__ batch, const int64_t* __restrict__ sei0,
@@ -380,7 +387,7 @@
   if (max_n < 1 || max_n > GEOSSL_RADIUS_MAX_N) return (int)hipErrorInvalidValue;
   allow_big_lds(&k_radius<0>);
   hipLaunchKernelGGL((k_radius<0>), dim3((unsigned)B), dim3(64), radius_lds(max_n), stream, pos, mol_ptr, nullptr,
-                     (int)B, max_n, r2, cap, deg, nullptr, nullptr, nullptr, nullptr, nullptr, nullptr, 1.0f, nullptr);
+                     (int)B, max_n, r2, cap, deg, nullptr, nullptr, nullptr, nullptr, nullptr, nullptr, 1.0f, nullptr, nullptr);
   GEOSSL_CHECK_LAUNCH();
   return 0;
 }
@@ -393,7 +400,7 @@
   allow_big_lds(&k_radius<1>);
   hipLaunchKernelGGL((k_radius<1>), dim3((unsigned)B), dim3(64), radius_lds(max_n), stream, pos, mol_ptr, nullptr,
                      (int)B, max_n, r2, cap, nullptr, edge_ptr, edge_src, edge_dst, edge_weight, nullptr, nullptr, 1.0f,
-                     nullptr);
+                     nullptr, nullptr);
   GEOSSL_CHECK_LAUNCH();
   return 0;
 }
@@ -401,17 +408,25 @@
 extern "C" int geossl_pair_geometry(const float* pos, const int32_t* mol_ptr, const int32_t* pair_ptr, int64_t B,
                                     int max_n, float r2, int cap, float cutoff, float* pair_d, float* pair_c,
                                     uint8_t* pair_flag, hipStream_t stream) {
+  return geossl_pair_geometry_live(pos, mol_ptr, pair_ptr, B, max_n, r2, cap, cutoff, pair_d, pair_c, pair_flag, nullptr,
+                                   stream);
+}
+
+extern "C" int geossl_pair_geometry_live(const float* pos, const int32_t* mol_ptr, const int32_t* pair_ptr, int64_t B,
+                                         int max_n, float r2, int cap, float cutoff, float* pair_d, float* pair_c,
+                                         uint8_t* pair_flag, int32_t* mol_live, hipStream_t stream) {
   if (B <= 0) return 0;
   if (max_n <= cap && max_n <= 64) {
     hipLaunchKernelGGL(k_pair_geometry_flat, dim3((unsigned)B), dim3(64), 0, stream, pos, mol_ptr, pair_ptr, (int)B, r2,
-                       cutoff, pair_d, pair_c, pair_flag);
+                       cutoff, pair_d, pair_c, pair_flag, mol_live);
     GEOSSL_CHECK_LAUNCH();
     return 0;
   }
   if (max_n < 1 || max_n > GEOSSL_RADIUS_MAX_N) return (int)hipErrorInvalidValue;
   allow_big_lds(&k_radius<2>);
   hipLaunchKernelGGL((k_radius<2>), dim3((unsigned)B), dim3(64), radius_lds(max_n), stream, pos, mol_ptr, pair_ptr,
-                     (int)B, max_n, r2, cap, nullptr, nullptr, nullptr, nullptr, nullptr, pair_d, pair_flag, cutoff, pair_c);
+                     (int)B, max_n, r2, cap, nullptr, nullptr, nullptr, nullptr, nullptr, pair_d, pair_flag, cutoff, pair_c,
+                     mol_live);
   GEOSSL_CHECK_LAUNCH();
   return 0;
 }
diff --git a/geossl_amd/csrc/sparse_pairs.hip b/geossl_amd/csrc/sparse_pairs.hip
--- a/geossl_amd/csrc/sparse_pairs.hip
+++ b/geossl_amd/csrc/sparse_pairs.hip
@@ -235,6 +235,90 @@
   }
 }
 
+constexpr int LP_THREADS = 256, LP_WAVES = LP_THREADS / 64;
+__global__ __launch_bounds__(LP_THREADS) void k_live_pairs(
+    const float* __restrict__ pair_d, const float* __restrict__ pair_c, const uint8_t* __restrict__ pair_flag,
+    const int32_t* __restrict__ pair_i, const int32_t* __restrict__ pair_j, const int32_t* __restrict__ mol_ptr,
+    const int32_t* __restrict__ pair_ptr, const int32_t* __restrict__ mol_live, int B, int P, float cutoff,
+    const int32_t* __restrict__ dyn_P, float* __restrict__ out_d, float* __restrict__ out_c,
+    uint8_t* __restrict__ out_flag, int32_t* __restrict__ out_i, int32_t* __restrict__ out_j,
+    int32_t* __restrict__ row_slot, int32_t* __restrict__ n_live) {
+  __shared__ int s_before[LP_WAVES], s_all[LP_WAVES];
+  const int tid = threadIdx.x, lane = tid & 63, wave = tid >> 6;
+  const int m0 = blockIdx.x * LP_WAVES;
+  const int Preal = dyn_count(P, dyn_P);
+  {
+    int before = 0, all = 0;
+    for (int k = tid; k < B; k += LP_THREADS) {
+      const int v = mol_live[k];
+      all += v;
+      if (k < m0) before += v;
+    }
+#pragma unroll
+    for (int o = 32; o > 0; o >>= 1) {
+      before += __shfl_xor(before, o, 64);
+      all += __shfl_xor(all, o, 64);
+    }
+    if (lane == 0) {
+      s_before[wave] = before;
+      s_all[wave] = all;
+    }
+    __syncthreads();
+  }
+  int base = 0, total = 0;
+#pragma unroll
+  for (int w = 0; w < LP_WAVES; ++w) {
+    base += s_before[w];
+    total += s_all[w];
+  }
+  total = min(total, P);
+  if (blockIdx.x == 0 && tid == 0) n_live[0] = total;
+  for (int p = total + blockIdx.x * LP_THREADS + tid; p < P; p += gridDim.x * LP_THREADS) {
+    out_i[p] = 0;
+    out_j[p] = 0;
+    out_d[p] = cutoff;
+    out_c[p] = 0.0f;
+    out_flag[p] = 0;
+    row_slot[p] = 0;
+  }
+  const int m = m0 + wave;
+  if (m >= B) return;
+  for (int k = m0; k < m; ++k) base += mol_live[k];
+  const int n = mol_ptr[m + 1] - mol_ptr[m], s0 = pair_ptr[m], np = n * (n - 1) / 2;
+  const unsigned long long lt = (lane == 0) ? 0ull : (~0ull >> (64 - lane));
+  for (int q0 = 0; q0 < np; q0 += 64) {
+    const int slot = s0 + q0 + lane;
+    const bool in = q0 + lane < np && slot < Preal;
+    const unsigned fl = in ? pair_flag[slot] : 0u;
+    const unsigned long long mk = __ballot(fl != 0u);
+    const int r = base + __popcll(mk & lt);
+    if (fl != 0u && r < P) {
+      out_i[r] = pair_i[slot];
+      out_j[r] = pair_j[slot];
+      out_d[r] = pair_d[slot];
+      out_c[r] = pair_c[slot];
+      out_flag[r] = (uint8_t)fl;
+      row_slot[r] = slot;
+    }
+    base += __popcll(mk);
+  }
+}
+
+__global__ __launch_bounds__(256) void k_gather_live_rows(const float* __restrict__ src,
+                                                          const int32_t* __restrict__ row_slot,
+                                                          const int32_t* __restrict__ n_live, int P, int F4,
+                                                          float* __restrict__ dst) {
+  const int n = min(P, n_live[0]);
+  const size_t lbase = (size_t)blockIdx.y * P;
+  const float4* __restrict__ s4 = reinterpret_cast<const float4*>(src);
+  float4* __restrict__ d4 = reinterpret_cast<float4*>(dst);
+  const int64_t total = (int64_t)n * F4;
+  for (int64_t i = (int64_t)blockIdx.x * 256 + threadIdx.x; i < total; i += (int64_t)gridDim.x * 256) {
+    const int r = (int)(i / F4), c = (int)(i - (int64_t)r * F4);
+    d4[(lbase + r) * F4 + c] = s4[(lbase + row_slot[r]) * F4 + c];
+  }
+}
+
 template <int VW>
 __global__ __launch_bounds__(SP_THREADS) void k_aggregate_sparse(const float* __restrict__ x,
                                                                  const float* __restrict__ Wf,
@@ -334,6 +418,31 @@
   return 0;
 }
 
+extern "C" int geossl_live_pairs_build(const float* pair_d, const float* pair_c, const uint8_t* pair_flag,
+                                       const int32_t* pair_i, const int32_t* pair_j, const int32_t* mol_ptr,
+                                       const int32_t* pair_ptr, const int32_t* mol_live, int64_t B, int64_t P,
+                                       float cutoff, const int32_t* dyn_P, float* live_d, float* live_c,
+                                       uint8_t* live_flag, int32_t* live_i, int32_t* live_j, int32_t* row_slot,
+                                       int32_t* n_live, hipStream_t stream) {
+  if (B <= 0 || P < 0 || P > (1ll << 30) || mol_live == nullptr || n_live == nullptr) return (int)hipErrorInvalidValue;
+  hipLaunchKernelGGL(k_live_pairs, dim3((unsigned)((B + LP_WAVES - 1) / LP_WAVES)), dim3(LP_THREADS), 0, stream, pair_d,
+                     pair_c, pair_flag, pair_i, pair_j, mol_ptr, pair_ptr, mol_live, (int)B, (int)P, cutoff, dyn_P, live_d,
+                     live_c, live_flag, live_i, live_j, row_slot, n_live);
+  GEOSSL_CHECK_LAUNCH();
+  return 0;
+}
+
+extern "C" int geossl_gather_live_rows(const float* src, const int32_t* row_slot, const int32_t* n_live, int64_t P, int L,
+                                       int F, float* dst, hipStream_t stream) {
+  if (P <= 0 || L <= 0) return 0;
+  if (F <= 0 || (F & 3) || P > (1ll << 30) || L > 65535 || n_live == nullptr) return (int)hipErrorInvalidValue;
+  const int64_t work = (P * (F / 4) + 255) / 256;
+  hipLaunchKernelGGL(k_gather_live_rows, dim3((unsigned)(work < 2048 ? work : 2048), (unsigned)L), dim3(256), 0, stream,
+                     src, row_slot, n_live, (int)P, F / 4, dst);
+  GEOSSL_CHECK_LAUNCH();
+  return 0;
+}
+
 extern "C" int geossl_cfconv_aggregate_sparse(const float* x, const float* Wf, const int32_t* inc_ptr,
                                               const int32_t* inc_pair, const uint32_t* inc_src, int64_t N, int F,
                                               int swap, float* out, hipStream_t stream) {
diff --git a/geossl_amd/ops.py b/geossl_amd/ops.py
--- a/geossl_amd/ops.py
+++ b/geossl_amd/ops.py
@@ -55,7 +55,7 @@
     return (edge_index, weight) if return_weight else edge_index
 
 
-def pair_geometry(pos, layout, cutoff, max_num_neighbors=32):
+def pair_geometry(pos, layout, cutoff, max_num_neighbors=32, mol_live=None):
     if getattr(layout, "sparse", False):
         raise _lib.GeosslHipError("a sparse layout (a structure above 255 atoms, or GEOSSL_SPARSE_PAIRS=1) has no dense "
                                   "pair slots: ops.sparse_pair_geometry builds its pair list")
@@ -68,9 +68,51 @@
     pair_flag = torch.empty(P, dtype=torch.uint8, device=dev)
     r2 = float(torch.tensor(float(cutoff) * float(cutoff), dtype=torch.float32))
     if P > 0:
-        call("geossl_pair_geometry", ptr(pos), ptr(layout.mol_ptr), ptr(layout.pair_ptr), layout.B, layout.max_n, r2,
-             radius_cap(max_num_neighbors), float(cutoff), ptr(pair_d), ptr(pair_c), ptr(pair_flag), stream())
+        if mol_live is not None:
+            call("geossl_pair_geometry_live", ptr(pos), ptr(layout.mol_ptr), ptr(layout.pair_ptr), layout.B, layout.max_n,
+                 r2, radius_cap(max_num_neighbors), float(cutoff), ptr(pair_d), ptr(pair_c), ptr(pair_flag),
+                 ptr(mol_live), stream())
+        else:
+            call("geossl_pair_geometry", ptr(pos), ptr(layout.mol_ptr), ptr(layout.pair_ptr), layout.B, layout.max_n, r2,
+                 radius_cap(max_num_neighbors), float(cutoff), ptr(pair_d), ptr(pair_c), ptr(pair_flag), stream())
     return pair_d, pair_c, pair_flag
+
+
+def live_pairs_enabled():
+    return _env("GEOSSL_LIVE_PAIRS", "1") != "0"
+
+
+class LivePairs:
+
+    __slots__ = ("P", "pair_d", "pair_c", "pair_flag", "pair_i", "pair_j", "row_slot", "n_live")
+
+    @property
+    def dyn_P(self):
+        return self.n_live.data_ptr()
+
+
+def live_pairs(pair_d, pair_c, pair_flag, layout, mol_live, cutoff, out=None):
+    P = layout.P
+    dev = pair_d.device
+    lp = out
+    if lp is None:
+        lp = LivePairs()
+        lp.P = P
+        i32 = dict(dtype=torch.int32, device=dev)
+        lp.pair_d = torch.empty(max(P, 1), dtype=torch.float32, device=dev)
+        lp.pair_c = torch.empty(max(P, 1), dtype=torch.float32, device=dev)
+        lp.pair_flag = torch.empty(max(P, 1), dtype=torch.uint8, device=dev)
+        lp.pair_i, lp.pair_j = torch.empty(max(P, 1), **i32), torch.empty(max(P, 1), **i32)
+        lp.row_slot = torch.empty(max(P, 1), **i32)
+        lp.n_live = torch.empty(1, **i32)
+    elif lp.P != P:
+        raise ValueError("the LivePairs given as `out` was made for another capacity")
+    dyn = getattr(layout, "dyn", None)
+    call("geossl_live_pairs_build", ptr(pair_d), ptr(pair_c), ptr(pair_flag), ptr(layout.pair_i), ptr(layout.pair_j),
+         ptr(layout.mol_ptr), ptr(layout.pair_ptr), ptr(mol_live), layout.B, P, float(cutoff),
+         dyn.n_pairs2 if dyn is not None else None, ptr(lp.pair_d), ptr(lp.pair_c), ptr(lp.pair_flag), ptr(lp.pair_i),
+         ptr(lp.pair_j), ptr(lp.row_slot), ptr(lp.n_live), stream())
+    return lp
 
 
 class SparsePairs:
diff --git a/include/geossl_hip.h b/include/geossl_hip.h
--- a/include/geossl_hip.h
+++ b/include/geossl_hip.h
@@ -596,6 +596,21 @@
                               int32_t* lo_cnt, int32_t* pair_i, int32_t* pair_j, float* pair_d, float* pair_c,
                               uint8_t* pair_flag, int32_t* inc_ptr, int32_t* inc_pair, uint32_t* inc_src,
                               int32_t* n_pairs, hipStream_t stream);
+
+int geossl_pair_geometry_live(const float* pos, const int32_t* mol_ptr, const int32_t* pair_ptr, int64_t B, int max_n,
+                              float r2, int cap, float cutoff, float* pair_d, float* pair_c, uint8_t* pair_flag,
+                              int32_t* mol_live, hipStream_t stream);
+int geossl_live_pairs_build(const float* pair_d, const float* pair_c, const uint8_t* pair_flag, const int32_t* pair_i,
+                            const int32_t* pair_j, const int32_t* mol_ptr, const int32_t* pair_ptr,
+                            const int32_t* mol_live, int64_t B, int64_t P, float cutoff, const int32_t* dyn_P,
+                            float* live_d, float* live_c, uint8_t* live_flag, int32_t* live_i, int32_t* live_j,
+                            int32_t* row_slot, int32_t* n_live, hipStream_t stream);
+int geossl_cfconv_filter_fwd_rows(const float* pair_d, const float* pair_c, int64_t P, const GeosslFilterWeights* w, int L,
+                                  int F, int G, const float* offset, float coeff, float* T, float* Wf,
+                                  const int32_t* dyn_P, const int32_t* row_slot, hipStream_t stream);
+int geossl_gather_live_rows(const float* src, const int32_t* row_slot, const int32_t* n_live, int64_t P, int L, int F,
+                            float* dst, hipStream_t stream);
+
 int geossl_cfconv_aggregate_sparse(const float* x, const float* Wf, const int32_t* inc_ptr, const int32_t* inc_pair,
                                    const uint32_t* inc_src, int64_t N, int F, int swap, float* out,
                                    hipStream_t stream);
```

Measured after the change: 400,900 (median of 6 runs). 2.3% higher.
